# probcomp/PClean

Hardware: AMD Instinct MI355X
Metric: rows/sec per Gibbs sweep on 1M-row synthetic hospital; F1 vs ground truth (higher is better)
Workload: dtype f64

## Files before the change

include/pclean_hip.h:

```cpp
#ifndef PCLEAN_HIP_H
#define PCLEAN_HIP_H

#include <stddef.h>
#include <stdint.h>

#ifdef __cplusplus
extern "C" {
#endif

typedef struct pclean_ctx pclean_ctx;

typedef enum {
  PCLEAN_OK = 0,
  PCLEAN_ERR_ARG = -1,
  PCLEAN_ERR_HIP = -2,
  PCLEAN_ERR_NO_DEVICE = -3,
  PCLEAN_ERR_STATE = -4,
  PCLEAN_ERR_CAPACITY = -5
} pclean_status;

#define PCLEAN_DIST_OSA 0
#define PCLEAN_DIST_DL 1

#define PCLEAN_DENS_ADD_TYPOS 0
// ... 176 lines not shown
int pclean_get_moved(pclean_ctx* ctx, int32_t block_id, int32_t* n_out, int32_t* rows_out, int32_t* choice_out);
int pclean_set_active_rows(pclean_ctx* ctx, int32_t begin, int32_t count);
int pclean_set_cur_stride(pclean_ctx* ctx, int64_t stride);
int pclean_pin_host(pclean_ctx* ctx, void* ptr, size_t bytes);
int pclean_unpin_host(pclean_ctx* ctx, void* ptr);
int pclean_sweep_latent(pclean_ctx* ctx, const pclean_infer_config* cfg, uint64_t seed, uint32_t sweep_idx,
                        int32_t block_id, int32_t n_roots, const int32_t* roots, int32_t n_items,
                        const int32_t* keys, const int32_t* ev_off, const int32_t* ev_rows, const int32_t* ev_ctx,
                        const int32_t* excl, int32_t* chosen, int32_t* vals);
#define PCLEAN_EV_MAX_STEPS 4
int pclean_build_evidence(pclean_ctx* ctx, int32_t cur_block, int32_t n_steps, const int32_t* step_table,
                          const int32_t* step_col, int32_t n_target_rows, int32_t n_src, const int32_t* src_block,
                          const int32_t* src_table, const int32_t* src_col, int32_t* off_out);
int pclean_get_evidence(pclean_ctx* ctx, int32_t begin, int32_t n, int32_t* rows_out, int32_t* ctx_out);
int pclean_sweep_latent_resident(pclean_ctx* ctx, const pclean_infer_config* cfg, uint64_t seed, uint32_t sweep_idx,
                                 int32_t block_id, int32_t n_roots, const int32_t* roots, int32_t n_items,
                                 const int32_t* keys, const int32_t* ev_off, int32_t ev_begin, const int32_t* excl,
                                 int32_t* chosen, int32_t* vals);
int pclean_stats_device_ptr(pclean_ctx* ctx, int32_t table_id, void** dptr, int64_t* n);
int pclean_get_stats(pclean_ctx* ctx, int32_t table_id, int64_t* out);
int pclean_get_timing(pclean_ctx* ctx, pclean_timing* out);
int pclean_get_root_stats(pclean_ctx* ctx, pclean_root_stats* out);
int pclean_set_timed_block(pclean_ctx* ctx, int32_t block_id);
int pclean_set_profiling(pclean_ctx* ctx, int32_t on);
int pclean_get_profile(pclean_ctx* ctx, int32_t cap, char* names, float* ms, int32_t* launches, int32_t* n_out);

int pclean_argsort_ids(pclean_ctx* ctx, int32_t n, const int32_t* ids, int32_t id_max, int32_t* order_out);

int pclean_comm_unique_id(pclean_ctx* ctx, unsigned char id_out[128]);
int pclean_comm_init(pclean_ctx* ctx, int32_t n_ranks, int32_t rank, const unsigned char id[128]);
int pclean_allreduce_stats(pclean_ctx* ctx, int32_t table_id, int64_t* out);
int pclean_allreduce_stats_fused(pclean_ctx* ctx, int32_t n_tables, const int32_t* table_ids, int32_t local_is_zero,
                                 int64_t* out);
int pclean_comm_destroy(pclean_ctx* ctx);
int pclean_comm_get_stats(pclean_ctx* ctx, int64_t out[8]);

#define PCLEAN_COMMIT_FB_RECORDS 1
#define PCLEAN_COMMIT_FB_DUMMY 2
#define PCLEAN_COMMIT_FB_CAPACITY 4
typedef struct {
  int32_t table_id;
  int32_t n_hw;
  int32_t n_free;
  int32_t cols_changed;
  int32_t created, deleted;
  int64_t total, live, max_count;
} pclean_commit_slot;
typedef struct {
  int32_t fallback;
  int32_t n_changed;
  int32_t n_slots;
  int32_t stats_reduced;
  int32_t n_records[16];
  int32_t n_distinct[16];
  pclean_commit_slot slot[16];
} pclean_commit_summary;
int pclean_prepare(pclean_ctx* ctx, uint32_t ev_blocks);
int pclean_commit_enable(pclean_ctx* ctx, int32_t n_blocks, int32_t* supported);
int pclean_commit_n_slots(pclean_ctx* ctx, int32_t* n_slots, int32_t* table_ids);
int pclean_commit_set_table_state(pclean_ctx* ctx, int32_t table_id, int32_t n_hw, int32_t n_free,
                                  const int32_t* free_stack);
int pclean_commit_device(pclean_ctx* ctx, int32_t n_blocks, uint32_t sweep_idx, pclean_commit_summary* out);
int pclean_commit_device_dist(pclean_ctx* ctx, int32_t n_blocks, uint32_t sweep_idx, int32_t local_empty,
                              int32_t max_local_rows, pclean_commit_summary* out);
int pclean_commit_pull_table(pclean_ctx* ctx, int32_t table_id, int32_t* state8, int32_t* cols, int64_t* counts,
                             uint8_t* live, int32_t* free_stack, int32_t* origin);
int pclean_set_cur(pclean_ctx* ctx, int32_t n_blocks, const int32_t* cur);
int pclean_get_cur(pclean_ctx* ctx, int32_t n_blocks, int32_t* cur);
int pclean_drop_cur(pclean_ctx* ctx);
int pclean_set_sweep_mode(pclean_ctx* ctx, int32_t flags);
int pclean_sweep_fetch(pclean_ctx* ctx);
int pclean_table_shape(pclean_ctx* ctx, int32_t table_id, int32_t* n_rows, int32_t* n_cols);

int pclean_maybe_resample(pclean_ctx* ctx, int32_t n_rows, int32_t n_particles, const double* logw,
                          int32_t retain_first, uint64_t seed, uint32_t sweep, uint32_t block,
                          int32_t* ancestors, double* logml_inc, double* ess);
int pclean_final_choice(pclean_ctx* ctx, int32_t n_rows, int32_t n_particles, const double* logw,
                        int32_t use_mh, int32_t is_csmc, uint64_t seed, uint32_t sweep, int32_t* chosen,
                        double* log_total);

int pclean_debug_force_generic(pclean_ctx* ctx, int32_t on);
int pclean_debug_global_evidence_sort(pclean_ctx* ctx, int32_t on);
int pclean_debug_root_flags(pclean_ctx* ctx, int32_t n_rows, int32_t* out);

int pclean_random_add_typos(pclean_ctx* ctx, int32_t n, const uint32_t* cp, const int64_t* off, int32_t max_typos,
                            uint64_t seed, uint32_t stream, int32_t out_stride, uint32_t* out_cp, int32_t* out_len);
int pclean_random_string_prior(pclean_ctx* ctx, int32_t n, int32_t min_len, int32_t max_len, const double* init_p,
                               const double* trans_p, uint64_t seed, uint32_t stream, int32_t out_stride,
                               uint8_t* out_letters, int32_t* out_len);
int pclean_random_string_prior_at(pclean_ctx* ctx, int32_t n, const uint64_t* seeds, const uint32_t* elems, int32_t min_len,
                                  int32_t max_len, const double* init_p, const double* trans_p, uint32_t stream,
                                  int32_t out_stride, uint8_t* out_letters, int32_t* out_len);
int pclean_random_categorical(pclean_ctx* ctx, int32_t n, int32_t n_options, const double* logp, uint64_t seed,
                              uint32_t stream, int32_t* out);
int pclean_random_normal(pclean_ctx* ctx, int32_t n, const double* mean, double std, double fwd_scale, uint64_t seed,
                         uint32_t stream, double* out);
int pclean_random_maybe_swap(pclean_ctx* ctx, int32_t n, const double* prob, const int32_t* n_options, uint64_t seed,
                             uint32_t stream, int32_t* out);
int pclean_random_time_prior(pclean_ctx* ctx, int32_t n, uint64_t seed, uint32_t stream, int32_t* out);

int pclean_debug_detmath(pclean_ctx* ctx, int32_t n, const double* x, double* exp_out, double* log_out,
                         uint64_t* fixw_out);
int pclean_debug_rand64(pclean_ctx* ctx, int32_t n, uint64_t seed, const uint32_t* rows, uint32_t site,
                        uint32_t particle, uint32_t sweep, uint64_t* out);

#ifdef __cplusplus
}
#endif
#endif
```

pclean_amd/_lib.py:

```python
import ctypes as C
import os

import numpy as np

HERE = os.path.dirname(os.path.abspath(__file__))
LIB_PATH = os.environ.get("PCLEAN_HIP_LIB") or os.path.join(HERE, "libpclean_hip.so")

MAX_CTX = 4
EV_MAX_STEPS = 4
CHOICE_NEW = -1
DIST_OSA, DIST_DL = 0, 1
DENS_ADD_TYPOS, DENS_EQUAL, DENS_MAYBE_SWAP = 0, 1, 2
NODE_FK, NODE_LEAF = 0, 1
DUMMY_STRING_PRIOR, DUMMY_TIME_PRIOR = 1, 2


class PCleanHipError(RuntimeError):
    pass


class Term(C.Structure):
    _fields_ = [("obs_col", C.c_int32), ("cand_col", C.c_int32), ("pair_table", C.c_int32),
                ("dens_kind", C.c_int32), ("max_typos", C.c_int32), ("ctx_slot", C.c_int32),
                ("fn_table", C.c_int32), ("ctx_mode", C.c_int32)]
# ... 119 lines not shown
            if self._io.get("cur_pinned"):
                self.lib.pclean_unpin_host(self.h, C.c_void_p(self._io["cur_pinned"][0]))
            self._pinned, self._io = [], {}
            self.lib.pclean_ctx_destroy(self.h)
            self.h = C.c_void_p()

    def __del__(self):
        try:
            self.close()
        except Exception:
            pass

    def load_strings(self, sym, off):
        sym = np.ascontiguousarray(sym, dtype=np.uint16)
        off = np.ascontiguousarray(off, dtype=np.int64)
        check(self.h, self.lib.pclean_load_strings(self.h, C.c_int32(len(off) - 1), _p(sym, C.c_uint16),
                                                   _p(off, C.c_int64)), "pclean_load_strings")

    def load_columns(self, obs):
        obs = np.ascontiguousarray(obs, dtype=np.int32)
        n_cols, n_rows = obs.shape
        check(self.h, self.lib.pclean_load_columns(self.h, C.c_int32(n_rows), C.c_int32(n_cols), _p(obs, C.c_int32)),
              "pclean_load_columns")

    def build_pair_table(self, table_id, obs_ids, lat_ids, mode=DIST_OSA):
        obs_ids = np.ascontiguousarray(obs_ids, dtype=np.int32)
        lat_ids = np.ascontiguousarray(lat_ids, dtype=np.int32)
        check(self.h, self.lib.pclean_build_pair_table(self.h, C.c_int32(table_id), C.c_int32(len(obs_ids)),
                                                       _p(obs_ids, C.c_int32), C.c_int32(len(lat_ids)),
                                                       _p(lat_ids, C.c_int32), C.c_int32(mode)),
              "pclean_build_pair_table")

    def set_pair_table(self, table_id, table):
        table = np.ascontiguousarray(table, dtype=np.uint8)
        check(self.h, self.lib.pclean_set_pair_table(self.h, C.c_int32(table_id), C.c_int32(table.shape[0]),
                                                     C.c_int32(table.shape[1]), _p(table, C.c_uint8)),
              "pclean_set_pair_table")

    def get_pair_table(self, table_id, n_obs, n_lat):
        out = np.empty((n_obs, n_lat), dtype=np.uint16)
        check(self.h, self.lib.pclean_get_pair_table(self.h, C.c_int32(table_id), _p(out, C.c_uint16)),
              "pclean_get_pair_table")
        return out

    def get_pair_rows(self, table_id, obs_rows, n_lat):
        obs_rows = np.ascontiguousarray(obs_rows, dtype=np.int32)
        out = np.empty((len(obs_rows), n_lat), dtype=np.uint16)
        check(self.h, self.lib.pclean_get_pair_rows(self.h, C.c_int32(table_id), C.c_int32(len(obs_rows)),
                                                    _p(obs_rows, C.c_int32), _p(out, C.c_uint16)),
              "pclean_get_pair_rows")
        return out

    def set_row_offset(self, row_offset):
        check(self.h, self.lib.pclean_set_row_offset(self.h, C.c_int64(row_offset)), "pclean_set_row_offset")

    def get_density_tables(self):
        mr, md, ml = C.c_int32(), C.c_int32(), C.c_int32()
        check(self.h, self.lib.pclean_get_density_tables(self.h, C.byref(mr), C.byref(md), C.byref(ml), None, None),
              "pclean_get_density_tables")
        nb = np.empty((mr.value + 1, md.value + 1), dtype=np.float64)
        logl = np.empty(ml.value + 1, dtype=np.float64)
        check(self.h, self.lib.pclean_get_density_tables(self.h, C.byref(mr), C.byref(md), C.byref(ml),
                                                         _p(nb, C.c_double), _p(logl, C.c_double)),
              "pclean_get_density_tables")
        return mr.value, md.value, ml.value, nb, logl

    def string_prior_scores(self, lm, off, min_len, max_len, init_logp, trans_logp):
        lm = np.ascontiguousarray(lm, dtype=np.uint8)
        off = np.ascontiguousarray(off, dtype=np.int64)
        init_logp = np.ascontiguousarray(init_logp, dtype=np.float64)
        trans_logp = np.ascontiguousarray(trans_logp, dtype=np.float64)
        n = len(off) - 1
        out = np.empty(n, dtype=np.float64)
        check(self.h, self.lib.pclean_string_prior_scores(self.h, C.c_int32(n), _p(lm, C.c_uint8), _p(off, C.c_int64),
                                                          C.c_int32(min_len), C.c_int32(max_len),
                                                          _p(init_logp, C.c_double), _p(trans_logp, C.c_double),
                                                          _p(out, C.c_double)), "pclean_string_prior_scores")
        return out

    def root_flags(self, n_rows):
        out = np.empty(n_rows, dtype=np.int32)
        check(self.h, self.lib.pclean_debug_root_flags(self.h, C.c_int32(n_rows), _p(out, C.c_int32)), "pclean_debug_root_flags")
        return out

    def global_evidence_sort(self, on):
        check(self.h, self.lib.pclean_debug_global_evidence_sort(self.h, C.c_int32(int(on))), "pclean_debug_global_evidence_sort")

    def force_generic(self, on):
        check(self.h, self.lib.pclean_debug_force_generic(self.h, C.c_int32(int(on))), "pclean_debug_force_generic")

    def set_table(self, table_id, cols, counts, strength, discount, n_cols=None):
        counts = np.ascontiguousarray(counts, dtype=np.int64)
        if cols is None:
            n_rows = len(counts)
        else:
            cols = np.ascontiguousarray(cols, dtype=np.int32)
            n_cols, n_rows = cols.shape if cols.ndim == 2 else (0, len(counts))
        check(self.h, self.lib.pclean_set_table(self.h, C.c_int32(table_id), C.c_int32(n_rows), C.c_int32(n_cols),
                                                _p(cols, C.c_int32), _p(counts, C.c_int64), C.c_double(strength),
                                                C.c_double(discount)), "pclean_set_table")

    def set_block_group(self, block_id, group):
        check(self.h, self.lib.pclean_set_block_group(self.h, C.c_int32(block_id), C.c_int32(group)), "pclean_set_block_group")

    def set_lm_tables(self, init_p, trans_p, letter_sym):
        init_p = np.ascontiguousarray(init_p, dtype=np.float64)
        trans_p = np.ascontiguousarray(trans_p, dtype=np.float64)
        letter_sym = np.ascontiguousarray(letter_sym, dtype=np.uint16)
        assert init_p.size == 28 and trans_p.size == 28 * 28 and letter_sym.size == 28
        check(self.h, self.lib.pclean_set_lm_tables(self.h, _p(init_p, C.c_double), _p(trans_p, C.c_double),
                                                    _p(letter_sym, C.c_uint16)), "pclean_set_lm_tables")

    def set_options(self, table_id, values, logp):
        values = np.ascontiguousarray(values, dtype=np.int32)
        logp = np.ascontiguousarray(logp, dtype=np.float64)
        check(self.h, self.lib.pclean_set_options(self.h, C.c_int32(table_id), C.c_int32(len(values)),
                                                  _p(values, C.c_int32), _p(logp, C.c_double)), "pclean_set_options")

    def set_options_cols(self, table_id, cols, logp):
        cols = np.ascontiguousarray(cols, dtype=np.int32)
        logp = np.ascontiguousarray(logp, dtype=np.float64)
        check(self.h, self.lib.pclean_set_options_cols(self.h, C.c_int32(table_id), C.c_int32(cols.shape[1]),
                                                       C.c_int32(cols.shape[0]), _p(cols, C.c_int32),
                                                       _p(logp, C.c_double)), "pclean_set_options_cols")

    def load_numeric_columns(self, x):
        x = np.ascontiguousarray(x, dtype=np.float64)
        check(self.h, self.lib.pclean_load_numeric_columns(self.h, C.c_int32(x.shape[1]), C.c_int32(x.shape[0]),
                                                           _p(x, C.c_double)), "pclean_load_numeric_columns")

    def set_mean_table(self, table_id, mean):
        mean = np.ascontiguousarray(mean, dtype=np.float64).reshape(-1)
        check(self.h, self.lib.pclean_set_mean_table(self.h, C.c_int32(table_id), C.c_int32(len(mean)),
                                                     _p(mean, C.c_double)), "pclean_set_mean_table")

    def set_node_gauss(self, block_id, node_id, g):
        check(self.h, self.lib.pclean_set_node_gauss(self.h, C.c_int32(block_id), C.c_int32(node_id), C.byref(g)),
              "pclean_set_node_gauss")

    def set_cur_locals(self, block_id, locals_):
        if locals_ is None:
            check(self.h, self.lib.pclean_set_cur_locals(self.h, C.c_int32(block_id), None, C.c_int32(0)), "pclean_set_cur_locals")
            return
        a = np.ascontiguousarray(locals_, dtype=np.int32).reshape(-1, 2)
        check(self.h, self.lib.pclean_set_cur_locals(self.h, C.c_int32(block_id), _p(a, C.c_int32), C.c_int32(len(a))),
              "pclean_set_cur_locals")

    def get_locals(self, block_id, n_rows):
        out = np.empty((n_rows, 2), dtype=np.int32)
        check(self.h, self.lib.pclean_get_locals(self.h, C.c_int32(block_id), _p(out, C.c_int32)), "pclean_get_locals")
        return out

    def set_fn_table(self, fn_id, fn):
        fn = np.ascontiguousarray(fn, dtype=np.int32)
        check(self.h, self.lib.pclean_set_fn_table(self.h, C.c_int32(fn_id), C.c_int32(fn.shape[0]),
                                                   C.c_int32(fn.shape[1]), _p(fn, C.c_int32)), "pclean_set_fn_table")

    def set_prob_table(self, p):
        p = np.ascontiguousarray(p, dtype=np.float64)
        check(self.h, self.lib.pclean_set_prob_table(self.h, C.c_int32(len(p)), _p(p, C.c_double)),
              "pclean_set_prob_table")

    def load_score_block(self, block_id, obs_col, pair_table, val_src, key_src, nopt_fn, other_val, prob_fn,
                         prob_a_src, prob_b_src):
        a = [np.ascontiguousarray(x, dtype=np.int32).reshape(-1) for x in
             (obs_col, pair_table, val_src, key_src, nopt_fn, other_val, prob_a_src, prob_b_src)]
# ... 454 lines not shown
```

pclean_amd/csrc/enum.h:

```cpp
#pragma once
#include "ctx.h"

#define PCLEAN_MAX_CHILDREN 16
#define PCLEAN_MAX_TERMS 16

struct TermDev {
  const int32_t* obs_col;
  const int32_t* cand_col;
  const uint8_t* pair;
  const uint16_t* lat_len;
  const int32_t* fn;
  int32_t n_lat, elem_bytes, dens_kind, max_typos, ctx_slot, fn_nb;
  int32_t ctx_mode, pad;
  const int32_t* aux_col;
  int32_t other_val, pad2;
};

struct GaussDev {
  int32_t on, n_dims, n_locals, t_kind;
  const double* x;
  const double* mu;
  int32_t src_kind[4];
  const int32_t* src_ptr[4];
  int32_t src_slot[4], stride[4];
// ... 23 lines not shown
  int32_t nb_stride, pad;
  const double* prob_same;
  const double* prob_diff;
  const double* logn;
};

struct AggDev {
  const uint64_t* key;
  const int32_t* cnt;
  const int32_t* off;
  const int32_t* end;
};

struct ItemsDev {
  int32_t n, pad;
  const int32_t* row;
  const int32_t* ctx;
  const int32_t* excl;
  const int32_t* particle;
  int64_t row_offset;
  const int32_t* out_pos;
  const int32_t* ev_lo;
  const int32_t* ev_hi;
  const int32_t* ev_rows;
  const int32_t* ev_ctx;
  const int32_t* rng_row;
  const int32_t* grp_off;
  const int32_t* members;
  int32_t draw_is, draw_ds;
  const AggDev* agg;
  const int32_t* ev_item;
  const int32_t* sel;
  const unsigned int* sel_n;
  const int32_t* grp_uid;
};

struct ChildrenDev {
  int32_t n, pad;
  const double* arr[PCLEAN_MAX_CHILDREN];
  const int32_t* obs_col[PCLEAN_MAX_CHILDREN];
  int32_t n_obs[PCLEAN_MAX_CHILDREN];
};

struct GateDev {
  int32_t n, pad;
  const double* cache[PCLEAN_MAX_CHILDREN];
  const int32_t* obs_col[PCLEAN_MAX_CHILDREN];
  int32_t n_obs[PCLEAN_MAX_CHILDREN];
  double ub[PCLEAN_MAX_CHILDREN];
};
int pclean_launch_gate(pclean_ctx* ctx, const NodeDev& nd, const ItemsDev& it, const GateDev& gt, int32_t* flag);

struct FastTermDev {
  const uint8_t* comp;
  const uint8_t* clen;
  const uint8_t* cmin;
  const int32_t* obs_col;
  int32_t max_typos, ctx_slot;
  const uint8_t* pair;
  const uint16_t* lat_len;
  const int32_t* cand_col;
  const int32_t* fn;
  int32_t n_lat, fn_nb;
};
struct FastRootDev {
  int32_t n_cand, kpad, n_terms, lmax, dstride;
  int32_t kscan;
  int32_t is_leaf;
  const uint16_t* alive;
  const double* prior_e;
  const double* prior_n;
  const double* logc_m1;
  const int64_t* counts;
  double scal[4];
  int32_t n_pre, pre[3];
  int32_t cstride, atd_stride;
  double inv_c, prior_max_e, prior_max_n;
  const double* atd;
  const uint8_t* zero_row;
  const int32_t* obs_rm;
  FastTermDev terms[PCLEAN_MAX_TERMS];
};

#define ROOT_LZ_CAP 256
struct RootExtra {
  int32_t* lz_k;
  uint64_t* lz_p;
  int32_t* lz_ns;
  const int32_t* eager_rows;
  const uint64_t* g_U;
};
int pclean_launch_root_fast(pclean_ctx* ctx, const FastRootDev& fr, const ItemsDev& it, const ChildrenDev& ch,
                            uint64_t seed, uint32_t sweep, uint32_t site, int n_draws, double* lse_out,
                            int32_t* draws_out, int32_t* overflow_flag, unsigned int* overflow_count,
                            int32_t* desc_scratch, int32_t* overflow_list,
                            unsigned int* scan_stats = nullptr, int n_items = 0, const double* pre_score = nullptr,
                            bool want_worklist = true, unsigned int* wl_stat = nullptr, const int32_t* pre_obs = nullptr,
                            RootExtra* extra = nullptr);
struct LazyDrawArgs {
  int32_t n_pos, n_rows, n_particles, pad;
  const int32_t* members;
  const int32_t* uid;
  const int32_t* item_row;
  const int32_t* slot_item;
  const int32_t* chosen;
  const int32_t* cur_b;
  const int32_t* eager_rows;
  const int32_t* draws_item;
  const int32_t* lz_k;
  const uint64_t* lz_p;
  const int32_t* lz_ns;
  const uint64_t* g_U;
  int32_t* pchoice;
  int64_t row_offset;
  int32_t res_new, pad2;
};
int pclean_launch_lazy_draws(pclean_ctx* ctx, const LazyDrawArgs& a, uint64_t seed, uint32_t sweep, uint32_t site);
int pclean_launch_group_gate(pclean_ctx* ctx, const FastRootDev& fr, const ItemsDev& it, const GateDev& gt, int32_t* flag,
                             double* score_out, int32_t* obs_out);
int pclean_launch_overflow_fast(pclean_ctx* ctx, const FastRootDev& fr, const ItemsDev& it, const ChildrenDev& ch,
                                uint64_t seed, uint32_t sweep, uint32_t site, int n_draws, double* lse_out,
                                int32_t* draws_out, const int32_t* over_list, const unsigned int* over_count);
int pclean_overflow_fast_ok(const FastRootDev& fr, const ItemsDev& it);
int pclean_launch_root_flags(pclean_ctx* ctx, int n_groups, const int32_t* gd, const int32_t* grp_off,
                             const int32_t* members, const int32_t* oflag, int32_t* out);
size_t pclean_fast_desc_words(int n_groups);
int pclean_debug_gauss_ev_probe(pclean_ctx* ctx, int n_items, int P, int n_nodes, const NodeDev* nds, int node, const ItemsDev& it,
                                const int32_t* vals, int n_mean, int n_ev);
int pclean_build_obs_rowmajor(pclean_ctx* ctx, const int32_t* const* obs_cols, int n_terms, int n_rows, int32_t* out);
int pclean_build_compact(pclean_ctx* ctx, const uint8_t* pair, int n_obs, int n_lat, const int32_t* cand_col,
                         const uint16_t* lat_len, int n_cand, int kpad, uint8_t* comp, uint8_t* clen);
int pclean_build_compact_min(pclean_ctx* ctx, const uint8_t* comp, int n_obs, int kpad, int cstride, uint8_t* cmin);
int pclean_update_compact_min(pclean_ctx* ctx, const uint8_t* comp, int n_obs, int kpad, int cstride, const int32_t* rows,
                              int n_rows, uint8_t* cmin);
int pclean_update_compact(pclean_ctx* ctx, const uint8_t* pair, int n_obs, int n_lat, const int32_t* cand_col,
                          const uint16_t* lat_len, const int32_t* rows, int n_rows, int kpad, uint8_t* comp, uint8_t* clen);
int pclean_build_priors(pclean_ctx* ctx, const int64_t* counts, const double* logc_full, int n_cand, int kpad,
                        double logden_e, double logden_n, double* prior_e, double* prior_n, uint16_t* alive);

int pclean_launch_enum(pclean_ctx* ctx, const NodeDev& nd, const ItemsDev& it, const ChildrenDev& ch, uint64_t seed,
                       uint32_t sweep, uint32_t site, int n_draws, double* lse_out, double* scores_out,
                       int32_t* draws_out, double* scores_tmp = nullptr);
size_t pclean_enum_split_scores(const NodeDev& nd, const ItemsDev& it);
int pclean_leaf_coarse_blocks(int n_options);
int pclean_launch_leaf_coarse_build(pclean_ctx* ctx, const NodeDev& nd, const ItemsDev& it, int n_blocks, double* lse_out,
                                    double* m_out, uint64_t* U_out, uint64_t* coarse, int dummy_k, uint64_t* udummy_out);
int pclean_launch_leaf_coarse_draw(pclean_ctx* ctx, const NodeDev& nd, const ItemsDev& it, const int32_t* obs_col, int n_obs,
                                   int n_blocks, const double* lse_c, const double* m_c, const uint64_t* U_c,
                                   const uint64_t* coarse, uint64_t seed, uint32_t sweep, uint32_t site, int n_draws,
                                   double* lse_out, int32_t* draws_out);
int pclean_launch_prior_terms(pclean_ctx* ctx, size_t n_slots, int N, int n_nodes, const NodeDev* nds,
                              const int32_t* n_children, const int32_t* child_begin, const int32_t* children,
                              const int32_t* pchoice, const int32_t* pnewpos, const int32_t* vals, const int32_t* it_ctx,
                              double* w);
int pclean_launch_prior_terms_ev(pclean_ctx* ctx, int n_items, int P, int n_nodes, const NodeDev* nds, const AggDev* const* aggs,
                                 const int32_t* n_children, const int32_t* child_begin, const int32_t* children, int n_roots,
                                 const int32_t* roots, const ItemsDev& it, const int32_t* vals, double* w);
int pclean_launch_ev_leaf(pclean_ctx* ctx, const NodeDev& nd, const ItemsDev& it, const FastRootDev& fr, uint64_t seed,
                          uint32_t sweep, uint32_t site, int n_draws, double* lse_out, int32_t* draws_out,
                          int32_t* overflow_flag, unsigned int* overflow_count, int32_t* overflow_list = nullptr,
                          const ChildrenDev* ch = nullptr, uint32_t* dsum = nullptr);
```

pclean_amd/csrc/eval.hip:

```cpp
#include "sweep_internal.h"

int build_gauss_dev(pclean_ctx* ctx, const pclean_gauss& g, const CandTable* t, GaussDev& d) {
  memset(&d, 0, sizeof d);
  if (g.x_col < 0 || g.x_col >= ctx->n_xcols) return pclean_fail(ctx, PCLEAN_ERR_ARG, "gauss: numeric column out of range");
  const MeanTable& m = ctx->mean[g.mean_table];
  if (!m.valid) return pclean_fail(ctx, PCLEAN_ERR_STATE, "gauss: mean table %d not set", g.mean_table);
  d.on = 1;
  d.n_dims = g.n_dims;
  d.n_locals = g.n_locals;
  d.x = ctx->xnum.p + (size_t)g.x_col * ctx->n_rows + ctx->active_begin;
  d.mu = m.v.p;
  for (int i = 0; i < g.n_dims; ++i) {
    d.src_kind[i] = g.src_kind[i];
    d.src_slot[i] = g.src[i];
    d.stride[i] = g.stride[i];
    d.src_ptr[i] = nullptr;
    if (g.src_kind[i] == PCLEAN_GSRC_CAND) {
      if (!t || g.src[i] < 0 || g.src[i] >= t->n_cols) return pclean_fail(ctx, PCLEAN_ERR_ARG, "gauss: candidate column out of range");
      d.src_ptr[i] = t->cols.p + (size_t)g.src[i] * t->n_rows;
    } else if (g.src_kind[i] == PCLEAN_GSRC_OBS) {
      if (g.src[i] < 0 || g.src[i] >= ctx->n_cols) return pclean_fail(ctx, PCLEAN_ERR_ARG, "gauss: observed column out of range");
      d.src_ptr[i] = ctx->obs.p + (size_t)g.src[i] * ctx->n_rows + ctx->active_begin;
    }
  }
// ... 155 lines not shown
      b.leaf_drawable[node_id] = any ? 1 : 0;
      if (getenv("PCLEAN_DEBUG_DUMMY"))
        fprintf(stderr, "[pclean] block %d node %d: dummy option %d, drawable %d (first observed value %d, weight %llu; missing-value weight %llu)\n",
                block_id, node_id, dummy_k, any ? 1 : 0, first_o, first_o >= 0 ? (unsigned long long)hu[first_o] : 0ull,
                (unsigned long long)hu[U]);
    }
    s->leaf_version[key] = ver;
  }
  *out = cache.p;
  *obs_col = ctx->obs.p + (size_t)tm.obs_col * ctx->n_rows + ctx->active_begin;
  *n_obs = U;
  return PCLEAN_OK;
}

static int prefilter_terms(pclean_ctx* ctx, const Block& b, const pclean_node& n, int32_t pre[3]) {
  int order[PCLEAN_MAX_TERMS];
  const int nt = std::min(n.n_terms, PCLEAN_MAX_TERMS);
  for (int i = 0; i < nt; ++i) order[i] = i;
  auto plain = [&](const pclean_term& tm) {
    return tm.ctx_slot < 0 && tm.dens_kind == PCLEAN_DENS_ADD_TYPOS && tm.pair_table >= 0 && tm.pair_table < PCLEAN_MAX_TABLES &&
           ctx->pair[tm.pair_table].valid;
  };
  std::stable_sort(order, order + nt, [&](int a, int c) {
    const pclean_term& ta = b.terms[n.term_begin + a];
    const pclean_term& tc = b.terms[n.term_begin + c];
    if (plain(ta) != plain(tc)) return plain(ta);
    if (!plain(ta)) return false;
    return ctx->pair[ta.pair_table].max_lat_len > ctx->pair[tc.pair_table].max_lat_len;
  });
  int n_compact = 0;
  for (int i = 0; i < nt; ++i) n_compact += plain(b.terms[n.term_begin + i]) ? 1 : 0;
  const int n_pre = std::min(3, n_compact);
  for (int p = 0; p < 3; ++p) pre[p] = p < n_pre ? order[p] : 0;
  return n_pre;
}

static int cols_union(pclean_ctx* ctx, CandTable& t, uint64_t base, uint64_t col_mask, int* n_out) {
  *n_out = 0;
  if (t.union_n >= 0 && t.union_base == base && t.union_head == t.cols_version && t.union_mask == col_mask) {
    *n_out = t.union_n;
    return 1;
  }
  size_t first = t.delta_log.size();
  for (size_t i = 0; i < t.delta_log.size(); ++i)
    if (t.delta_log[i].base == base) {
      first = i;
      break;
    }
  if (first == t.delta_log.size() || t.delta_log.back().next != t.cols_version) return 0;
  std::vector<uint8_t> mark((size_t)std::max(t.n_rows, 1), 0);
  std::vector<int32_t> rows;
  for (size_t i = first; i < t.delta_log.size(); ++i) {
    if (i > first && t.delta_log[i].base != t.delta_log[i - 1].next) return 0;
    const CandTable::DeltaEntry& e = t.delta_log[i];
    for (size_t q = 0; q < e.rows.size(); ++q) {
      const int32_t r = e.rows[q];
      if ((e.masks[q] & col_mask) && r >= 0 && r < t.n_rows && !mark[r]) {
        mark[r] = 1;
        rows.push_back(r);
      }
    }
    if (rows.size() * 8 > (size_t)t.n_rows) return 0;
  }
  std::sort(rows.begin(), rows.end());
  if (!rows.empty()) {
    const size_t bytes = rows.size() * sizeof(int32_t);
    if (t.union_rows.alloc(rows.size() + rows.size() / 4 + 64)) return pclean_fail(ctx, PCLEAN_ERR_HIP, "device alloc failed");
    if (ctx->ustage.grow(bytes + 256)) return pclean_fail(ctx, PCLEAN_ERR_HIP, "page-locked staging alloc failed");
    ctx->ustage.rewind();
    void* h = ctx->ustage.take(bytes);
    if (!h) return pclean_fail(ctx, PCLEAN_ERR_HIP, "page-locked staging alloc failed");
    memcpy(h, rows.data(), bytes);
    HIPCHK(ctx, hipMemcpyAsync(t.union_rows.p, h, bytes, hipMemcpyHostToDevice, ctx->stream));
    HIPCHK(ctx, hipStreamSynchronize(ctx->stream));
  }
  t.union_base = base;
  t.union_mask = col_mask;
  t.union_head = t.cols_version;
  t.union_n = (int32_t)rows.size();
  *n_out = t.union_n;
  return 1;
}

static int try_fast_root(pclean_ctx* ctx, int block_id, int node_id, FastRootDev& fr, bool ev_mode = false) {
  Block& b = ctx->block[block_id];
  if (node_id >= 64) return 0;
  const pclean_node& n = b.nodes[node_id];
  const CandTable& t = ctx->cand[n.table];
  const bool leaf = n.kind == PCLEAN_NODE_LEAF;
  static const bool no_leaf = getenv("PCLEAN_NO_FAST_LEAF") != nullptr;
  if (!t.valid || t.n_rows < 1024 || n.n_terms < 1 || n.n_terms > PCLEAN_MAX_TERMS || (leaf && no_leaf)) return 0;
  if (leaf != t.is_options) return 0;
  int lmax = 0, dmax = 0;
  for (int i = 0; i < n.n_terms; ++i) {
    const pclean_term& tm = b.terms[n.term_begin + i];
    const PairTable& pt = ctx->pair[tm.pair_table];
    if (!pt.valid || tm.dens_kind != PCLEAN_DENS_ADD_TYPOS || pt.elem_bytes != 1) return 0;
    if (tm.ctx_slot >= 0 && ((!ev_mode && tm.ctx_mode != 0) || !ctx->fn[tm.fn_table].valid)) return 0;
    if (tm.ctx_slot >= 2) return 0;
    lmax = std::max(lmax, pt.max_lat_len);
    dmax = std::max(dmax, std::max(pt.max_lat_len, pt.max_obs_len));
  }
  if (lmax > 255 || dmax > 255) return 0;
  if (leaf && !ev_mode) {
    double best = 0.0;
    for (int i = 0; i < n.n_terms; ++i) {
      const pclean_term& tm = b.terms[n.term_begin + i];
      if (tm.ctx_slot < 0) best = std::max(best, ctx->pair[tm.pair_table].mean_lat_len);
    }
    if (best < 16.0) return 0;
  }
  const int kpad = (t.n_rows + 15) & ~15;
  FastRoot& f = st(ctx)->fast[block_id * 64 + node_id];
  if (f.disabled > 0) {
    --f.disabled;
    return 0;
  }
  if ((int)f.comp.size() != n.n_terms) {
    for (auto& c : f.comp) c.release();
    for (auto& c : f.clen) c.release();
    for (auto& c : f.cblk) c.release();
    f.cblk.assign(n.n_terms, DevBuf<uint8_t>());
    f.comp.assign(n.n_terms, DevBuf<uint8_t>());
    f.clen.assign(n.n_terms, DevBuf<uint8_t>());
    f.ver.assign(n.n_terms, 0);
    f.kpad = kpad;
    f.prior_ver = 0;
  } else if (f.kpad != kpad) {
    f.ver.assign(n.n_terms, 0);
    f.kpad = kpad;
    f.prior_ver = 0;
  }
  auto grow = [](DevBuf<uint8_t>& b, size_t need) -> int {
    need = std::max<size_t>(need, 16);
    return need <= b.n && b.p ? 0 : b.alloc(need + need / 8);
  };
  const int cstride = ((((kpad + 63) >> 6) + 15) & ~15);
  for (int i = 0; i < n.n_terms; ++i) {
    const pclean_term& tm = b.terms[n.term_begin + i];
    const PairTable& pt = ctx->pair[tm.pair_table];
    fr.terms[i] = FastTermDev{};
    fr.terms[i].obs_col = ctx->obs_override ? ctx->obs_override : ctx->obs.p + (size_t)tm.obs_col * ctx->n_rows + ctx->active_begin;
    fr.terms[i].max_typos = tm.max_typos;
    fr.terms[i].ctx_slot = tm.ctx_slot;
    fr.terms[i].pair = (const uint8_t*)pt.d.p;
    fr.terms[i].lat_len = pt.lat_len.p;
    fr.terms[i].cand_col = t.cols.p + (size_t)tm.cand_col * t.n_rows;
    fr.terms[i].n_lat = pt.n_lat;
    if (tm.ctx_slot >= 0) {
      const FnTable& fnt = ctx->fn[tm.fn_table];
      fr.terms[i].fn = fnt.fn.p;
      fr.terms[i].fn_nb = fnt.n_b;
      continue;
    }
    const uint64_t ver = t.cols_version * 1000003ull + pt.version;
    static const bool no_delta = getenv("PCLEAN_NO_COMPACT_DELTA") != nullptr;
    if (f.ver[i] != ver && f.comp[i].p && f.cblk[i].p && !no_delta && t.cols_delta_n >= 0 && t.cols_delta_n * 8 <= t.n_rows &&
        f.ver[i] == t.cols_delta_base * 1000003ull + pt.version) {
      ProfScope psd(ctx, "compact_table_update");
      int rc = PCLEAN_OK;
      if (t.cols_delta_n > 0)
        rc = pclean_update_compact(ctx, pt.d.p, pt.n_obs, pt.n_lat, t.cols.p + (size_t)tm.cand_col * t.n_rows, pt.lat_len.p,
                                     t.cols_delta_rows, t.cols_delta_n, kpad, f.comp[i].p, f.clen[i].p);
      if (rc) return rc;
      if (t.cols_delta_n > 0)
        rc = pclean_update_compact_min(ctx, f.comp[i].p, pt.n_obs, kpad, cstride, t.cols_delta_rows, t.cols_delta_n, f.cblk[i].p);
      if (rc) return rc;
      f.ver[i] = ver;
    }
    static const bool no_chain = getenv("PCLEAN_NO_DELTA_CHAIN") != nullptr;
    if (f.ver[i] != ver && f.comp[i].p && f.cblk[i].p && !no_delta && !no_chain) {
      CandTable& tw = ctx->cand[n.table];
      uint64_t at = 0;
      bool have = false, via_commit = false;
      if (tw.commit_delta_n >= 0 && f.ver[i] == tw.commit_delta_base * 1000003ull + pt.version) {
        at = tw.commit_delta_next;
        have = via_commit = true;
      } else {
        for (const auto& e : tw.delta_log)
          if (f.ver[i] == e.base * 1000003ull + pt.version) {
            at = e.base;
            have = true;
            break;
          }
      }
      int un = 0;
      bool ok = have;
      if (ok && at != tw.cols_version) {
        uint64_t node_mask = 0;
        for (int q = 0; q < n.n_terms; ++q)
          if (b.terms[n.term_begin + q].ctx_slot < 0) node_mask |= 1ull << std::min(b.terms[n.term_begin + q].cand_col, 63);
        const int rcu = cols_union(ctx, tw, at, node_mask, &un);
        if (rcu < 0) return rcu;
        ok = rcu == 1;
      }
      const int64_t total = (int64_t)(via_commit ? tw.commit_delta_n : 0) + un;
      static const bool dbg_chain = getenv("PCLEAN_DEBUG_CHAIN") != nullptr;
      if (dbg_chain && i == 0)
        fprintf(stderr, "[chain] block %d node %d table %d (%d rows): have %d via_commit %d (commit rows %d) log %zu entries, union %s %d rows\n",
                block_id, node_id, (int)n.table, tw.n_rows, (int)have, (int)via_commit, tw.commit_delta_n, tw.delta_log.size(),
                ok ? "ok" : "none", un);
      if (ok && total * 8 <= tw.n_rows) {
        ProfScope psd(ctx, "compact_table_update");
        int rc = PCLEAN_OK;
        const int32_t* colp = tw.cols.p + (size_t)tm.cand_col * tw.n_rows;
        if (via_commit && tw.commit_delta_n > 0) {
          rc = pclean_update_compact(ctx, pt.d.p, pt.n_obs, pt.n_lat, colp, pt.lat_len.p, tw.commit_delta_rows, tw.commit_delta_n, kpad,
                                     f.comp[i].p, f.clen[i].p);
          if (!rc) rc = pclean_update_compact_min(ctx, f.comp[i].p, pt.n_obs, kpad, cstride, tw.commit_delta_rows, tw.commit_delta_n, f.cblk[i].p);
          if (rc) return rc;
        }
        if (un > 0) {
          rc = pclean_update_compact(ctx, pt.d.p, pt.n_obs, pt.n_lat, colp, pt.lat_len.p, tw.union_rows.p, un, kpad, f.comp[i].p, f.clen[i].p);
          if (!rc) rc = pclean_update_compact_min(ctx, f.comp[i].p, pt.n_obs, kpad, cstride, tw.union_rows.p, un, f.cblk[i].p);
          if (rc) return rc;
        }
        f.ver[i] = ver;
      }
    }
    if (f.ver[i] != ver || !f.comp[i].p) {
      ProfScope psd(ctx, "compact_table_rebuild");
      if (grow(f.comp[i], (size_t)pt.n_obs * kpad) || grow(f.clen[i], (size_t)kpad))
        return pclean_fail(ctx, PCLEAN_ERR_HIP, "device alloc failed (compact tables)");
      int rc = pclean_build_compact(ctx, pt.d.p, pt.n_obs, pt.n_lat, t.cols.p + (size_t)tm.cand_col * t.n_rows,
                                    pt.lat_len.p, t.n_rows, kpad, f.comp[i].p, f.clen[i].p);
      if (rc) return rc;
      if (grow(f.cblk[i], (size_t)pt.n_obs * cstride))
        return pclean_fail(ctx, PCLEAN_ERR_HIP, "device alloc failed (compact tables)");
      rc = pclean_build_compact_min(ctx, f.comp[i].p, pt.n_obs, kpad, cstride, f.cblk[i].p);
      if (rc) return rc;
      f.ver[i] = ver;
    }
    fr.terms[i].comp = f.comp[i].p;
    fr.terms[i].clen = f.clen[i].p;
    fr.terms[i].cmin = f.cblk[i].p;
  }
  if ((int)f.zero_row.n < kpad || !f.zero_row.p) {
    if (f.zero_row.alloc((size_t)kpad + 4096)) return pclean_fail(ctx, PCLEAN_ERR_HIP, "device alloc failed");
    HIPCHK(ctx, hipMemsetAsync(f.zero_row.p, 0, f.zero_row.n, ctx->stream));
  }
  if (f.prior_ver != t.version || !f.prior_n.p) {
    if ((!leaf && f.prior_e.alloc(kpad)) || f.prior_n.alloc(kpad) || f.alive.alloc(std::max(kpad >> 4, 1)))
      return pclean_fail(ctx, PCLEAN_ERR_HIP, "device alloc failed");
    int rc = pclean_build_priors(ctx, leaf ? nullptr : t.counts.p, t.logc_full.p, t.n_rows, kpad, t.scal[1], t.scal[0],
                                 leaf ? nullptr : f.prior_e.p, f.prior_n.p, f.alive.p);
    if (rc) return rc;
    f.prior_ver = t.version;
    f.logc_max = t.logc_max;
  }
  {
    fr.n_pre = prefilter_terms(ctx, b, n, fr.pre);
    const int stride = ctx->max_d + 1;
    const uint64_t ckey = ((uint64_t)lmax << 40) | ((uint64_t)dmax << 20) | (uint64_t)stride;
    if (f.cmin_key != ckey) {
      double cm = INFINITY;
      for (int L = 1; L <= lmax; ++L)
        for (int d = 1; d <= dmax; ++d) {
          const int r = (L + 4) / 5;
          double l = ctx->h_nb[(size_t)r * stride + d];
          l -= ctx->h_logl[L] * (double)d;
          l -= 1.629048269010741 * (double)d;
          if (l == l) cm = std::min(cm, -l / (double)d);
        }
      f.cmin = cm;
      f.cmin_key = ckey;
    }
    const double cmin = f.cmin;
    if (!(cmin > 1e-6) || !std::isfinite(cmin)) {
      fr.n_pre = 0;
      fr.inv_c = 0.0;
    } else {
      fr.inv_c = 1.0 / (cmin * (1.0 - 1e-9));
    }
    fr.cstride = cstride;
    fr.prior_max_e = f.logc_max - t.scal[1];
    fr.prior_max_n = f.logc_max - t.scal[0];
  }
  fr.obs_rm = nullptr;
  static const bool no_obs_rm = getenv("PCLEAN_NO_OBS_ROWMAJOR") != nullptr;
  if (!leaf && !ev_mode && !ctx->obs_override && !no_obs_rm && ctx->n_rows >= 4096) {
    const uint64_t key = ctx->obs_version * 1000003ull + (uint64_t)ctx->n_rows + 1ull;
    if (f.obs_rm_key != key || !f.obs_rm.p) {
      if (f.obs_rm.alloc((size_t)ctx->n_rows * PCLEAN_MAX_TERMS)) return pclean_fail(ctx, PCLEAN_ERR_HIP, "device alloc failed");
      const int32_t* cols[PCLEAN_MAX_TERMS] = {};
      for (int i = 0; i < n.n_terms; ++i) cols[i] = ctx->obs.p + (size_t)b.terms[n.term_begin + i].obs_col * ctx->n_rows;
      int rc = pclean_build_obs_rowmajor(ctx, cols, n.n_terms, ctx->n_rows, f.obs_rm.p);
      if (rc) return rc;
      f.obs_rm_key = key;
    }
    fr.obs_rm = f.obs_rm.p + (size_t)ctx->active_begin * PCLEAN_MAX_TERMS;
  }
  fr.n_cand = t.n_rows;
  fr.kpad = kpad;
  {
    static const bool no_kscan = getenv("PCLEAN_NO_KSCAN") != nullptr;
    const int n_used = (t.n_used > 0 && t.n_used <= t.n_rows && !no_kscan) ? t.n_used : t.n_rows;
    fr.kscan = std::min(kpad, (n_used + 63) & ~63);
  }
  fr.n_terms = n.n_terms;
  fr.lmax = lmax;
  fr.dstride = dmax + 1;
  fr.is_leaf = leaf ? 1 : 0;
  fr.atd = ctx->atd.p;
  fr.atd_stride = ctx->max_d + 1;
// ... 30 lines not shown
  double sum = 0.0;
  for (int c = 0; c < n.n_children; ++c) sum += subtree_ub(ctx, b, b.children[n.child_begin + c]);
  return std::max(0.0, sum);
}

__global__ void scatter_f64_kernel(int n, const int32_t* list, const double* src, double* dst) {
  const int j = blockIdx.x * blockDim.x + threadIdx.x;
  if (j < n) dst[list[j]] = src[j];
}
__global__ void sub_items_kernel(int n, const int32_t* list, const int32_t* p_row, const int32_t* p_ctx,
                                 const int32_t* p_excl, const int32_t* p_ev_lo, const int32_t* p_ev_hi,
                                 const int32_t* p_rng, const int32_t* p_origin, int32_t* row, int32_t* ctxv,
                                 int32_t* excl, int32_t* ev_lo, int32_t* ev_hi, int32_t* rng, int32_t* origin) {
  const int j = blockIdx.x * blockDim.x + threadIdx.x;
  if (j >= n) return;
  const int s = list[j];
  row[j] = p_row ? p_row[s] : s;
  excl[j] = p_excl ? p_excl[s] : -1;
  for (int c = 0; c < PCLEAN_MAX_CTX; ++c) ctxv[j * PCLEAN_MAX_CTX + c] = p_ctx ? p_ctx[(size_t)s * PCLEAN_MAX_CTX + c] : 0;
  if (p_ev_lo) {
    ev_lo[j] = p_ev_lo[s];
    ev_hi[j] = p_ev_hi[s];
  }
  if (p_rng) rng[j] = p_rng[s];
  if (origin) origin[j] = p_origin ? p_origin[s] : s;
}

__global__ void group_rep_items_kernel(int n, const int32_t* list, const int32_t* grp_off, const int32_t* members,
                                       const int32_t* p_row, const int32_t* p_ctx, const int32_t* p_excl, int32_t* row,
                                       int32_t* ctxv, int32_t* excl) {
  const int j = blockIdx.x * blockDim.x + threadIdx.x;
  if (j >= n) return;
  const int g = list ? list[j] : j;
  const int s = members[grp_off[g]];
  row[j] = p_row ? p_row[s] : s;
  excl[j] = p_excl ? p_excl[s] : -1;
  for (int c = 0; c < PCLEAN_MAX_CTX; ++c) ctxv[j * PCLEAN_MAX_CTX + c] = p_ctx ? p_ctx[(size_t)s * PCLEAN_MAX_CTX + c] : 0;
}
__global__ void group_scatter_f64_kernel(int n, const int32_t* list, const int32_t* grp_off, const int32_t* members,
                                         const double* src, double* dst) {
  const int j = blockIdx.x * blockDim.x + threadIdx.x;
  if (j >= n) return;
  const int g = list ? list[j] : j;
  const double v = src[j];
  const int hi = grp_off[g + 1];
  for (int mi = grp_off[g]; mi < hi; ++mi) dst[members[mi]] = v;
}

__global__ void member_scatter_f64_kernel(int n_pos, const int32_t* uid, const int32_t* members, const double* src, double* dst) {
  const int mi = blockIdx.x * blockDim.x + threadIdx.x;
  if (mi < n_pos) dst[members[mi]] = src[uid[mi] - 1];
}

int eval_node(pclean_ctx* ctx, int block_id, int node_id, const ItemList& il, const int32_t* excl,
                     uint64_t seed, uint32_t sweep, int n_draws, double* lse_out, int32_t* draws_out,
                     double* scores_out, const double* snew_override, bool time_it) {
  Block& b = ctx->block[block_id];
  const pclean_node& n = b.nodes[node_id];
  SweepState* s = st(ctx);
  const SweepState::LazyReq lazy_req = s->lazy_req;
  s->lazy_req = SweepState::LazyReq();
  s->lazy_out.valid = false;
  static const bool no_lazy = getenv("PCLEAN_NO_LAZY_DRAWS") != nullptr;
  const bool lazy_ok = lazy_req.on && !no_lazy && n_draws > 1 && !il.rng_row && !il.ev_lo;
  static const bool lazy_split = getenv("PCLEAN_LAZY_SPLIT") != nullptr;
  const bool lazy_sure = lazy_ok && (size_t)il.n * ROOT_LZ_CAP * 12 <= ((size_t)4 << 30);
  const int fast_split_m = (lazy_sure && !lazy_split) ? 0 : std::max(4, 256 / std::max(n_draws, 1));
  NodeDev nd;
  int rc = build_node_dev(ctx, b, node_id, nd);
  if (rc) return rc;
  ChildrenDev ch{};
  ItemsDev it{il.n, 0, il.row, il.ctx, excl, n_draws == 1 ? il.particle : nullptr, s->row_offset + ctx->active_begin,
              nullptr, il.ev_lo, il.ev_hi, il.ev_rows, il.ev_ctx, il.rng_row, nullptr, nullptr, il.draw_is, il.draw_ds,
              nullptr, nullptr};
  if (il.ev_lo) {
    rc = ensure_agg(ctx, block_id, node_id, il, &it.agg);
    if (rc) return rc;
    it.ev_item = il.origin;
  }
  FastRootDev fr;
  int fast = 0, fast_ev = 0;
  ItemGroups g_pre;
  bool fast_tried = false, groups_tried = false;
  const double* pre_score = nullptr;
  const int32_t* pre_obs = nullptr;
  if (n.kind == PCLEAN_NODE_FK && ctx->prior_mode) {
    ch.n = 0;
  } else if (n.kind == PCLEAN_NODE_FK) {
    if (snew_override) {
      ch.n = 1;
      ch.arr[0] = snew_override;
      ch.obs_col[0] = nullptr;
    } else {
      if (n.n_children > PCLEAN_MAX_CHILDREN) return pclean_fail(ctx, PCLEAN_ERR_CAPACITY, "too many children");
      ch.n = n.n_children;
      const CandTable& t = ctx->cand[n.table];
      GateDev gt{};
      gt.n = n.n_children;
      int n_open = 0;
      const char* gm = getenv("PCLEAN_GATE_MIN");
      const int gate_min = gm ? atoi(gm) : 2048;
      bool gate = excl && !scores_out && il.n >= gate_min && !getenv("PCLEAN_NO_GATE");
      SweepState::GateStat* gstat = (gate && node_id < 64 && sweep < 0x7ffffff0u && !il.ev_lo && !getenv("PCLEAN_GATE_ALWAYS"))
                                        ? &s->gate_stat[block_id * 64 + node_id] : nullptr;
      if (gstat && gstat->skip > 0) {
        --gstat->skip;
        gate = false;
        gstat = nullptr;
      }
      for (int c = 0; c < n.n_children; ++c) {
        const int cid = b.children[n.child_begin + c];
        const pclean_node& cn = b.nodes[cid];
        if (cn.kind == PCLEAN_NODE_LEAF && cn.cacheable) {
          rc = ensure_leaf_cache(ctx, block_id, cid, &ch.arr[c], &ch.obs_col[c], &ch.n_obs[c]);
          if (rc) return rc;
          gt.cache[c] = ch.arr[c];
          gt.obs_col[c] = ch.obs_col[c];
          gt.n_obs[c] = ch.n_obs[c];
          gt.ub[c] = 0.0;
          if (il.ev_lo) gt.ub[c] = subtree_ub(ctx, b, cid);
        } else {
          ++n_open;
          gt.cache[c] = nullptr;
          gt.ub[c] = subtree_ub(ctx, b, cid);
          if (!(gt.ub[c] < INFINITY)) gate = false;
        }
        if (il.ev_lo && !(gt.ub[c] < INFINITY)) gate = false;
      }
      static const bool no_group_gate = getenv("PCLEAN_NO_GROUP_GATE") != nullptr;
      bool pre_grouped = false;
      if (n_open > 0 && n_draws > 0 && excl && !scores_out && !ctx->force_generic && !nd.g.on && !il.rng_row && !il.ev_lo &&
          !no_group_gate) {
        fast = try_fast_root(ctx, block_id, node_id, fr);
        if (fast < 0) return fast;
        fast_tried = true;
        if (fast) {
          rc = make_item_groups(ctx, block_id, node_id, il, excl, g_pre, fast_split_m);
          if (rc) return rc;
          groups_tried = true;
          pre_grouped = g_pre.n_groups > 0;
        }
      }
      if (pre_grouped) {
        const int ng = g_pre.n_groups;
        ItemsDev itg = it;
        itg.n = ng;
        itg.grp_off = g_pre.grp_off;
        itg.members = g_pre.members;
        int32_t* list_g = nullptr;
        unsigned int n_need = (unsigned int)ng;
        if (gate) {
          ProfScope ps(ctx, "gate_new_branch");
          int32_t* flag = scratch<int32_t>(ctx, ng);
          list_g = scratch<int32_t>(ctx, ng);
          double* sc = scratch<double>(ctx, ng);
          int32_t* ow = scratch<int32_t>(ctx, (size_t)ng * PCLEAN_MAX_TERMS);
          if (!flag || !list_g || !sc || !ow) return pclean_fail(ctx, PCLEAN_ERR_HIP, "scratch alloc failed");
          if (time_it && s->evg0) (void)hipEventRecord(s->evg0, ctx->stream);
          rc = pclean_launch_group_gate(ctx, fr, itg, gt, flag, sc, ow);
          if (rc) return rc;
          if (time_it && s->evg0) {
            (void)hipEventRecord(s->evg1, ctx->stream);
            s->gate_timed = true;
          }
          unsigned int* need_ctr = fresh_counter(ctx);
          if (!need_ctr) return pclean_fail(ctx, PCLEAN_ERR_HIP, "counter bank: device alloc failed");
          hipLaunchKernelGGL(compact_new_kernel, grid1(ng), dim3(256), 0, ctx->stream, (size_t)ng, flag, 1, need_ctr, list_g,
                             nullptr);
          PCLEAN_READ_COUNT(ctx, need_ctr, &n_need);
          pre_score = sc;
          pre_obs = ow;
          if (gstat) {
            gstat->all_need_run = n_need == (unsigned int)ng ? gstat->all_need_run + 1 : 0;
            if (gstat->all_need_run >= 3) {
              gstat->skip = 16;
              gstat->all_need_run = 2;
            }
          }
          if (n_need == (unsigned int)ng) list_g = nullptr;
        }
        ItemList sil;
        const int32_t* sexcl = nullptr;
        if (n_need > 0) {
          int32_t* row2 = scratch<int32_t>(ctx, n_need);
          int32_t* ctx2 = scratch<int32_t>(ctx, (size_t)n_need * PCLEAN_MAX_CTX);
          int32_t* excl2 = scratch<int32_t>(ctx, n_need);
          if (!row2 || !ctx2 || !excl2) return pclean_fail(ctx, PCLEAN_ERR_HIP, "scratch alloc failed");
          hipLaunchKernelGGL(group_rep_items_kernel, grid1(n_need), dim3(256), 0, ctx->stream, (int)n_need, list_g, g_pre.grp_off,
                             g_pre.members, il.row, il.ctx, excl, row2, ctx2, excl2);
          sil = ItemList{(int)n_need, row2, il.ctx ? ctx2 : nullptr, nullptr, nullptr};
          sexcl = excl2;
        }
        for (int c = 0; c < n.n_children; ++c) {
          const int cid = b.children[n.child_begin + c];
          const pclean_node& cn = b.nodes[cid];
          if (cn.kind == PCLEAN_NODE_LEAF && cn.cacheable) continue;
          double* child_lse = scratch<double>(ctx, il.n);
          if (!child_lse) return pclean_fail(ctx, PCLEAN_ERR_HIP, "scratch alloc failed");
          ch.arr[c] = child_lse;
          ch.obs_col[c] = nullptr;
          if (n_need < (unsigned int)ng)
            hipLaunchKernelGGL(fill_f64_kernel, grid1(il.n), dim3(256), 0, ctx->stream, child_lse, (size_t)il.n, -__builtin_inf());
          if (n_need == 0) continue;
          const int32_t* child_excl = nullptr;
          if (cn.kind == PCLEAN_NODE_FK) {
            if (cn.parent_fk_col < 0 || cn.parent_fk_col >= t.n_cols)
              return pclean_fail(ctx, PCLEAN_ERR_ARG, "node %d: parent_fk_col out of range", cid);
            int32_t* ce = scratch<int32_t>(ctx, sil.n);
            if (!ce) return pclean_fail(ctx, PCLEAN_ERR_HIP, "scratch alloc failed");
            hipLaunchKernelGGL(derive_excl_kernel, grid1(sil.n), dim3(256), 0, ctx->stream, sil.n, sexcl, t.counts.p,
                               t.cols.p + (size_t)cn.parent_fk_col * t.n_rows, ce);
            child_excl = ce;
          }
          double* dst = scratch<double>(ctx, sil.n);
          if (!dst) return pclean_fail(ctx, PCLEAN_ERR_HIP, "scratch alloc failed");
          rc = eval_node_lse(ctx, block_id, cid, sil, child_excl, seed, sweep, dst);
          if (rc) return rc;
          if (!list_g && g_pre.uid && fast_split_m == 0)
            hipLaunchKernelGGL(member_scatter_f64_kernel, grid1(il.n), dim3(256), 0, ctx->stream, il.n, g_pre.uid, g_pre.members, dst,
                               child_lse);
          else
            hipLaunchKernelGGL(group_scatter_f64_kernel, grid1(sil.n), dim3(256), 0, ctx->stream, sil.n, list_g, g_pre.grp_off,
                               g_pre.members, dst, child_lse);
        }
      } else {
      int32_t* list = nullptr;
      unsigned int n_need = (unsigned int)il.n;
      if (gate && n_open > 0) {
        ProfScope ps(ctx, "gate_new_branch");
        int32_t* flag = scratch<int32_t>(ctx, il.n);
        list = scratch<int32_t>(ctx, il.n);
        if (!flag || !list) return pclean_fail(ctx, PCLEAN_ERR_HIP, "scratch alloc failed");
        if (s->counter.alloc(4)) return pclean_fail(ctx, PCLEAN_ERR_HIP, "device alloc failed");
        rc = pclean_launch_gate(ctx, nd, it, gt, flag);
        if (rc) return rc;
        unsigned int* need_ctr = fresh_counter(ctx);
        if (!need_ctr) return pclean_fail(ctx, PCLEAN_ERR_HIP, "counter bank: device alloc failed");
        hipLaunchKernelGGL(compact_new_kernel, grid1(il.n), dim3(256), 0, ctx->stream, (size_t)il.n, flag, 1, need_ctr, list,
                           nullptr);
        PCLEAN_READ_COUNT(ctx, need_ctr, &n_need);
        if (gstat) {
          gstat->all_need_run = n_need == (unsigned int)il.n ? gstat->all_need_run + 1 : 0;
// ... 106 lines not shown
        it.grp_off = g.grp_off;
        it.members = g.members;
        if (fast && fast_split_m == 0) it.grp_uid = g.uid;
        ggrp = g;
      }
    }
  }
  const uint32_t site = PCLEAN_SITE_NODE(block_id, node_id);
  if (time_it) {
    pclean_root_stats& rs = ctx->root_stats;
    rs = pclean_root_stats{};
    rs.fast = fast;
    rs.n_items = il.n;
    rs.n_groups = it.n;
    rs.n_cand = nd.n_cand;
    rs.n_terms = n.n_terms;
    rs.n_draws = n_draws;
    rs.pre_scored = pre_score ? 1 : 0;
    if (fast) {
      rs.kpad = fr.kscan;
      rs.cstride = std::min(fr.cstride, (((fr.kscan + 63) >> 6) + 15) & ~15);
      rs.n_pre = fr.n_pre;
      for (int p = 0; p < 3; ++p) rs.pre_obs_col[p] = p < fr.n_pre ? b.terms[n.term_begin + fr.pre[p]].obs_col : -1;
    }
  }
  if (!fast && !fast_ev) {
    ProfScope ps(ctx, n.kind == PCLEAN_NODE_FK ? "enum_fk_generic" : "enum_leaf_generic");
    if (time_it) (void)hipEventRecord(s->ev0, ctx->stream);
    double* sc_tmp = nullptr;
    if (!scores_out) {
      const size_t sc_n = pclean_enum_split_scores(nd, it);
      if (sc_n && !(sc_tmp = scratch<double>(ctx, sc_n))) return pclean_fail(ctx, PCLEAN_ERR_HIP, "scratch alloc failed");
    }
    rc = pclean_launch_enum(ctx, nd, it, ch, seed, sweep, site, n_draws, lse_out, scores_out, draws_out, sc_tmp);
    if (time_it) (void)hipEventRecord(s->ev1, ctx->stream);
    return rc;
  }
  int32_t* oflag = scratch<int32_t>(ctx, il.n);
  if (!oflag || s->counter.alloc(4)) return pclean_fail(ctx, PCLEAN_ERR_HIP, "scratch alloc failed");
  static const bool no_fast_over = getenv("PCLEAN_NO_FAST_OVERFLOW") != nullptr;
  const bool list_mode = fast && !no_fast_over && pclean_overflow_fast_ok(fr, it) && s->over_rec.size() < OVER_SLOTS &&
                         s->over_ctr.p != nullptr;
  static const bool no_ev_list = getenv("PCLEAN_NO_EV_LIST") != nullptr;
  const bool ev_list_mode = fast_ev && !no_ev_list && s->over_rec.size() < OVER_SLOTS && s->over_ctr.p != nullptr;
  unsigned int* over_count = (list_mode || ev_list_mode) ? s->over_ctr.p + s->over_rec.size() : s->counter.p + 1;
  int32_t* over_list = nullptr;
  if (list_mode || ev_list_mode) {
    over_list = scratch<int32_t>(ctx, il.n);
    if (!over_list) return pclean_fail(ctx, PCLEAN_ERR_HIP, "scratch alloc failed");
    s->over_rec.push_back(SweepState::OverRec{block_id, node_id, il.n, time_it, n.kind == PCLEAN_NODE_LEAF, fast_ev ? 64 : 1024});
  } else {
    { const int rcz = dev_zero(ctx, s->counter.p + 1, sizeof(unsigned int)); if (rcz) return rcz; }
  }
  if (!ev_list_mode)
    { const int rcz = dev_zero(ctx, oflag, (size_t)il.n * sizeof(int32_t)); if (rcz) return rcz; }
  if (fast) {
    int32_t* desc = scratch<int32_t>(ctx, pclean_fast_desc_words(it.n));
    if (!desc) return pclean_fail(ctx, PCLEAN_ERR_HIP, "scratch alloc failed");
    ProfScope ps(ctx, (time_it && block_id == 0) ? "root_scan_block0" : (n.kind == PCLEAN_NODE_FK ? "slot_scan" : "option_scan"));
    if (time_it) (void)hipEventRecord(s->ev0, ctx->stream);
    unsigned int* scan_stats = nullptr;
    if (time_it && s->over_ctr.p) {
      scan_stats = s->over_ctr.p + OVER_SLOTS;
      s->scan_stats_used = true;
    }
    FastRoot& fwl = s->fast[block_id * 64 + node_id];
    unsigned int* wl_stat = nullptr;
    if (!fwl.wl_off && node_id < 64 && s->over_rec.size() < OVER_SLOTS && s->over_ctr.p) {
      wl_stat = s->over_ctr.p + s->over_rec.size();
      s->over_rec.push_back(SweepState::OverRec{block_id, node_id, it.n, false, false, -1});
    }
    if (fwl.wl_off > 0) --fwl.wl_off;
    RootExtra ex{};
    bool use_ex = false;
    if (lazy_ok && !it.particle && !it.out_pos &&
        (size_t)it.n * ROOT_LZ_CAP * 12 <= ((size_t)4 << 30)) {
      ex.lz_k = scratch<int32_t>(ctx, (size_t)it.n * ROOT_LZ_CAP);
      ex.lz_p = scratch<uint64_t>(ctx, (size_t)it.n * ROOT_LZ_CAP);
      ex.lz_ns = scratch<int32_t>(ctx, (size_t)it.n);
      if (!ex.lz_k || !ex.lz_p || !ex.lz_ns) return pclean_fail(ctx, PCLEAN_ERR_HIP, "scratch alloc failed");
      ex.eager_rows = lazy_req.eager_rows;
      use_ex = true;
    }
    rc = pclean_launch_root_fast(ctx, fr, it, ch, seed, sweep, site, n_draws, lse_out, draws_out, oflag, over_count, desc,
                                 over_list, scan_stats, il.n, pre_score, wl_stat != nullptr, wl_stat, pre_obs, use_ex ? &ex : nullptr);
    if (!rc && ex.lz_ns) {
      SweepState::LazyOut& lo = s->lazy_out;
      lo.valid = true;
      lo.site = site;
      lo.args = LazyDrawArgs{};
      lo.args.n_pos = il.n;
      lo.args.members = it.grp_off ? it.members : nullptr;
      lo.args.uid = it.grp_off ? ggrp.uid : nullptr;
      lo.args.item_row = il.row;
      lo.args.eager_rows = lazy_req.eager_rows;
      lo.args.draws_item = draws_out;
      lo.args.lz_k = ex.lz_k;
      lo.args.lz_p = ex.lz_p;
      lo.args.lz_ns = ex.lz_ns;
      lo.args.g_U = ex.g_U;
      lo.args.row_offset = it.row_offset;
      lo.args.res_new = fr.is_leaf ? fr.n_cand - 1 : PCLEAN_CHOICE_NEW;
    }
    if (time_it) {
      (void)hipEventRecord(s->ev1, ctx->stream);
      s->dbg_desc = desc;
      s->dbg_grp_off = it.grp_off;
      s->dbg_members = it.members;
      s->dbg_oflag = oflag;
      s->dbg_groups = it.n;
      s->dbg_items = il.n;
    }
    if (!rc && list_mode) {
      ProfScope ps2(ctx, "overflow_rerun");
      ItemsDev itf = it;
      itf.n = il.n;
      itf.grp_off = nullptr;
      itf.members = nullptr;
      const int done = pclean_launch_overflow_fast(ctx, fr, itf, ch, seed, sweep, site, n_draws, lse_out, draws_out, over_list,
                                                   over_count);
      return done < 0 ? done : PCLEAN_OK;
    }
  } else {
    {
      ProfScope ps(ctx, "evidence_option_scan");
      uint32_t* dsum = nullptr;
      static const bool no_split = getenv("PCLEAN_NO_EV_SPLIT") != nullptr;
      if (!no_split && il.n <= 64 && s->lat_max_ev >= 16384 && fr.kpad >= 256 && (size_t)il.n * fr.kpad * 4 <= ((size_t)1 << 28)) {
        dsum = scratch<uint32_t>(ctx, (size_t)il.n * fr.kpad);
        if (!dsum) return pclean_fail(ctx, PCLEAN_ERR_HIP, "scratch alloc failed");
        const int rcz = dev_zero(ctx, dsum, (size_t)il.n * fr.kpad * sizeof(uint32_t));
        if (rcz) return rcz;
      }
      rc = pclean_launch_ev_leaf(ctx, nd, it, fr, seed, sweep, site, n_draws, lse_out, draws_out, oflag, over_count, over_list,
                                 n.kind == PCLEAN_NODE_FK ? &ch : nullptr, dsum);
    }
    if (!rc && ev_list_mode) {
      ProfScope ps2(ctx, "overflow_rerun");
      ItemsDev itr = it;
      itr.sel = over_list;
      itr.sel_n = over_count;
      double* sc_tmp = nullptr;
      const size_t sc_n = pclean_enum_split_scores(nd, itr);
      if (sc_n && !(sc_tmp = scratch<double>(ctx, sc_n))) return pclean_fail(ctx, PCLEAN_ERR_HIP, "scratch alloc failed");
      return pclean_launch_enum(ctx, nd, itr, ch, seed, sweep, site, n_draws, lse_out, nullptr, draws_out, sc_tmp);
    }
  }
  if (rc) return rc;
  unsigned int n_over = 0;
  PCLEAN_READ_COUNT(ctx, s->counter.p + 1, &n_over);
  ctx->timing.reserved += (int32_t)n_over;
  if (time_it) ctx->root_stats.overflow_items = (int32_t)n_over;
  if (n.kind == PCLEAN_NODE_LEAF && il.n >= (il.ev_lo ? 64 : 1024) &&
      (il.ev_lo ? n_over >= (unsigned int)il.n : (size_t)n_over * 4 > (size_t)il.n)) {
    FastRoot& f = s->fast[block_id * 64 + node_id];
    f.disabled = f.backoff;
    f.backoff = std::min(f.backoff * 2, 1 << 20);
  }
  if (n_over && getenv("PCLEAN_DEBUG_OVERFLOW"))
    fprintf(stderr, "[pclean] block %d node %d: %u of %d items re-run by the generic kernel\n", block_id, node_id, n_over,
            il.n);
  if (n_over) {
    ProfScope ps(ctx, "overflow_rerun");
    int32_t* list = scratch<int32_t>(ctx, n_over);
    int32_t* row2 = scratch<int32_t>(ctx, n_over);
    int32_t* excl2 = scratch<int32_t>(ctx, n_over);
    int32_t* ctx2 = scratch<int32_t>(ctx, (size_t)n_over * PCLEAN_MAX_CTX);
    int32_t* part2 = scratch<int32_t>(ctx, n_over);
// ... 334 lines not shown
  const bool first = split_m > 0 ? pos == piece * split_m : pos == 0;
  const int at = off0 + pos;
  members[at] = i;
  uid[at] = g0 + piece + 1;
  if (head) head[at] = first ? 1 : 0;
  if (first) grp_off[g0 + piece] = at;
}
__global__ void hg_unique_kernel(int n, const uint64_t* __restrict__ incl, const int32_t* __restrict__ rep,
                                 const int32_t* __restrict__ slot_of, const int32_t* __restrict__ row,
                                 const int32_t* __restrict__ ctxv, const int32_t* __restrict__ excl,
                                 int32_t* __restrict__ uid_of_item, int32_t* __restrict__ row2, int32_t* __restrict__ ctx2,
                                 int32_t* __restrict__ excl2) {
  const int i = blockIdx.x * blockDim.x + threadIdx.x;
  if (i >= n) return;
  const int sl = slot_of[i];
  const int u = (int)incl[sl] - 1;
  uid_of_item[i] = u;
  if (rep[sl] - 1 == i) {
    row2[u] = row ? row[i] : i;
    if (ctxv)
      for (int s = 0; s < PCLEAN_MAX_CTX; ++s) ctx2[(size_t)u * PCLEAN_MAX_CTX + s] = ctxv[(size_t)i * PCLEAN_MAX_CTX + s];
    if (excl) excl2[u] = excl[i];
  }
}
static int make_item_groups_hash(pclean_ctx* ctx, const ItemList& il, const int32_t* excl, const KeyColsDev& kc, int split_m,
                                 bool want_members, ItemGroups& g) {
  const int n = il.n;
  uint32_t cap = 1024;
  while (cap < 2u * (uint32_t)n) cap <<= 1;
  int32_t* rep = scratch<int32_t>(ctx, (size_t)cap * 2);
  uint64_t* incl = scratch<uint64_t>(ctx, cap);
  int32_t* slot_of = scratch<int32_t>(ctx, n);
  int32_t* pos_of = want_members ? scratch<int32_t>(ctx, n) : nullptr;
  size_t tmp_scan = 0, tmp_scan2 = 0;
  hipcub::TransformInputIterator<uint64_t, HgClaimed, const int32_t*> in_claimed(rep, HgClaimed());
  hipcub::TransformInputIterator<uint64_t, HgPacked, const unsigned int*> in_packed((const unsigned int*)(rep + cap), HgPacked{split_m});
  HIPCHK(ctx, hipcub::DeviceScan::InclusiveSum(nullptr, tmp_scan, in_claimed, incl, (int)cap, ctx->stream));
  HIPCHK(ctx, hipcub::DeviceScan::InclusiveSum(nullptr, tmp_scan2, in_packed, incl, (int)cap, ctx->stream));
  unsigned char* tmp = scratch<unsigned char>(ctx, std::max<size_t>(std::max(tmp_scan, tmp_scan2), 16));
  if (!rep || !incl || !slot_of || (want_members && !pos_of) || !tmp) return pclean_fail(ctx, PCLEAN_ERR_HIP, "scratch alloc failed");
  uint32_t wbits = HG_WBITS;
  while ((1u << wbits) > cap) --wbits;
  HashGroupDev hg{rep, want_members ? (unsigned int*)(rep + cap) : nullptr, cap - 1, split_m, wbits};
  { const int rcz = dev_zero(ctx, rep, (size_t)cap * (want_members ? 2 : 1) * sizeof(int32_t)); if (rcz) return rcz; }
  hipLaunchKernelGGL(hg_insert_kernel, grid1(n), dim3(256), 0, ctx->stream, n, kc, il.row, il.ctx, excl, hg, slot_of, pos_of);
  int32_t n_unique = 0;
  if (want_members) {
    HIPCHK(ctx, hipcub::DeviceScan::InclusiveSum(tmp, tmp_scan2, in_packed, incl, (int)cap, ctx->stream));
    PCLEAN_READ_COUNT(ctx, reinterpret_cast<const uint32_t*>(incl + (cap - 1)) + 1, &n_unique);
  } else {
    HIPCHK(ctx, hipcub::DeviceScan::InclusiveSum(tmp, tmp_scan, in_claimed, incl, (int)cap, ctx->stream));
    PCLEAN_READ_COUNT(ctx, reinterpret_cast<const uint32_t*>(incl + (cap - 1)), &n_unique);
  }
  if (n_unique <= 0 || (double)n_unique > 0.75 * n) return PCLEAN_OK;
  g.n_groups = n_unique;
  g.hg_incl = incl;
  g.hg_rep = rep;
  g.hg_slot_of = slot_of;
  if (!want_members) return PCLEAN_OK;
  int32_t* members = scratch<int32_t>(ctx, n);
  int32_t* uid = scratch<int32_t>(ctx, n);
  int32_t* grp_off = scratch<int32_t>(ctx, (size_t)n_unique + 1);
  if (!members || !uid || !grp_off) return pclean_fail(ctx, PCLEAN_ERR_HIP, "scratch alloc failed");
  hipLaunchKernelGGL(hg_fill_kernel, grid1(n), dim3(256), 0, ctx->stream, n, cap, incl, hg.cnt, slot_of, pos_of, split_m, members,
                     (int32_t*)nullptr, uid, grp_off);
  g.grp_off = grp_off;
  g.members = members;
  g.head = nullptr;
  g.uid = uid;
  return PCLEAN_OK;
}

#define STATIC_ORDER_WINDOWS 8
__global__ void static_key_kernel(int n, const int32_t* __restrict__ tuple_id, const uint32_t* __restrict__ pre_hash,
                                  uint64_t* __restrict__ key, int32_t* __restrict__ idx) {
  const int i = blockIdx.x * blockDim.x + threadIdx.x;
  if (i >= n) return;
  key[i] = ((uint64_t)pre_hash[i] << 32) | (uint32_t)tuple_id[i];
  idx[i] = i;
}
__global__ void static_tid_kernel(int n, const uint64_t* __restrict__ key_s, int32_t* __restrict__ tid) {
  const int j = blockIdx.x * blockDim.x + threadIdx.x;
  if (j < n) tid[j] = (int32_t)(uint32_t)key_s[j];
}
static int ensure_static_order(pclean_ctx* ctx, int block_id, int node_id, int n, const SweepState::TupleIds::StaticOrder** out) {
  typedef SweepState::TupleIds::StaticOrder StaticOrder;
  *out = nullptr;
  SweepState::TupleIds& t = st(ctx)->tuple_ids[block_id * 64 + node_id];
  const int begin = ctx->active_begin;
  if (!t.id.p || !t.pre.p || n <= 0 || (size_t)begin + (size_t)n > t.id.n) return PCLEAN_OK;
  for (const StaticOrder& w : t.windows)
    if (w.begin == begin && w.n == n) {
      *out = &w;
      return PCLEAN_OK;
    }
  for (;;) {
    size_t held = 0, smallest = 0;
    for (size_t k = 0; k < t.windows.size(); ++k) {
      held += (size_t)t.windows[k].n;
      if (t.windows[k].n < t.windows[smallest].n) smallest = k;
    }
    if (t.windows.size() < STATIC_ORDER_WINDOWS && held + (size_t)n <= 2 * (size_t)ctx->n_rows) break;
    if (t.windows.empty() || t.windows[smallest].n >= n) {
      static const bool trace = getenv("PCLEAN_TRACE_SYNC") != nullptr;
      if (trace) fprintf(stderr, "[pclean static groups] block %d node %d rows %d+%d: window not cached, hash table\n", block_id, node_id, begin, n);
      return PCLEAN_OK;
    }
    t.windows[smallest].release();
    t.windows.erase(t.windows.begin() + smallest);
  }
  StaticOrder w;
  w.begin = begin;
  w.n = n;
  DevBuf<uint64_t> key, key_s;
  DevBuf<int32_t> idx;
  DevBuf<unsigned char> tmp;
  int32_t* h_tid = nullptr;
  int32_t* h_off = nullptr;
  auto cleanup = [&]() {
    key.release(); key_s.release(); idx.release(); tmp.release();
    if (h_tid) (void)hipHostFree(h_tid);
    if (h_off) (void)hipHostFree(h_off);
  };
  auto fail = [&](const char* what) {
    cleanup();
    w.release();
    return pclean_fail(ctx, PCLEAN_ERR_HIP, "%s", what);
  };
  if (key.alloc(n) || key_s.alloc(n) || idx.alloc(n) || w.order.alloc(n) || w.tid.alloc(n)) return fail("device alloc failed");
  hipLaunchKernelGGL(static_key_kernel, grid1(n), dim3(256), 0, ctx->stream, n, t.id.p + begin, t.pre.p + begin, key.p, idx.p);
  size_t tmp_sort = 0;
  if (hipcub::DeviceRadixSort::SortPairs(nullptr, tmp_sort, key.p, key_s.p, idx.p, w.order.p, n, 0, 64, ctx->stream) != hipSuccess ||
      tmp.alloc(std::max<size_t>(tmp_sort, 16)) ||
      hipcub::DeviceRadixSort::SortPairs(tmp.p, tmp_sort, key.p, key_s.p, idx.p, w.order.p, n, 0, 64, ctx->stream) != hipSuccess)
    return fail("static order: sort failed");
  hipLaunchKernelGGL(static_tid_kernel, grid1(n), dim3(256), 0, ctx->stream, n, key_s.p, w.tid.p);
  if (hipHostMalloc((void**)&h_tid, (size_t)n * sizeof(int32_t)) != hipSuccess) { h_tid = nullptr; return fail("host alloc failed"); }
  if (hipHostMalloc((void**)&h_off, ((size_t)n + 1) * sizeof(int32_t)) != hipSuccess) { h_off = nullptr; return fail("host alloc failed"); }
  if (hipMemcpyAsync(h_tid, w.tid.p, (size_t)n * sizeof(int32_t), hipMemcpyDeviceToHost, ctx->stream) != hipSuccess ||
      hipStreamSynchronize(ctx->stream) != hipSuccess)
    return fail("static order: read-back failed");
  int n_off = 0, start = 0;
  h_off[n_off++] = 0;
  for (int sb = 0; sb < n;) {
    int se = sb + 1;
    while (se < n && h_tid[se] == h_tid[sb]) ++se;
    if (se - start > 64) {
      if (sb > start) h_off[n_off++] = start = sb;
      while (se - start > 64) h_off[n_off++] = start = start + 64;
    }
    sb = se;
  }
  h_off[n_off++] = n;
  w.n_tiles = n_off - 1;
  if (w.tile_off.alloc(n_off)) return fail("device alloc failed");
  if (hipMemcpyAsync(w.tile_off.p, h_off, (size_t)n_off * sizeof(int32_t), hipMemcpyHostToDevice, ctx->stream) != hipSuccess ||
      hipStreamSynchronize(ctx->stream) != hipSuccess)
    return fail("static order: upload failed");
  cleanup();
  t.windows.push_back(w);
  *out = &t.windows.back();
  return PCLEAN_OK;
}
__global__ __launch_bounds__(256) void sg_class_kernel(int n_tiles, const int32_t* __restrict__ tile_off,
                                                       const int32_t* __restrict__ order, const int32_t* __restrict__ tid_sorted,
                                                       const int32_t* __restrict__ excl, int split_m,
                                                       int32_t* __restrict__ members, int32_t* __restrict__ loc,
                                                       int32_t* __restrict__ tile_cnt) {
  const int tile = blockIdx.x * 4 + (threadIdx.x >> 6);
  const int lane = threadIdx.x & 63;
  if (tile >= n_tiles) return;
  const int t0 = tile_off[tile], len = tile_off[tile + 1] - t0;
  const bool on = lane < len;
  int i = 0, kt = 0, ke = 0;
  if (on) {
    i = order[t0 + lane];
    kt = tid_sorted[t0 + lane];
    ke = excl[i];
  }
  int pos_acc = 0, piece_acc = 0, my_at = 0, my_loc = 0;
  for (unsigned long long pend = __ballot(on); pend;) {
    const int ld = __builtin_ctzll(pend);
    const int lt = __builtin_amdgcn_readlane(kt, ld), le = __builtin_amdgcn_readlane(ke, ld);
    const unsigned long long cls = __ballot(on && kt == lt && ke == le) & pend;
    const int c = __popcll(cls);
    const int pieces = split_m > 0 ? max(c / split_m, 1) : 1;
    if ((cls >> lane) & 1ull) {
      const int r = __popcll(cls & ((1ull << lane) - 1ull));
      const int piece = split_m > 0 ? min(r / split_m, pieces - 1) : 0;
      const bool first = split_m > 0 ? r == piece * split_m : r == 0;
      my_at = pos_acc + r;
      my_loc = ((piece_acc + piece) << 1) | (first ? 1 : 0);
    }
    pos_acc += c;
    piece_acc += pieces;
    pend &= ~cls;
  }
  if (on) {
    members[t0 + my_at] = i;
    loc[t0 + my_at] = my_loc;
  }
  if (lane == 0) tile_cnt[tile] = piece_acc;
}
__global__ __launch_bounds__(256) void sg_fill_kernel(int n, int n_tiles, const int32_t* __restrict__ tile_off,
                                                      const int32_t* __restrict__ loc, const int32_t* __restrict__ tile_cnt,
                                                      const int32_t* __restrict__ incl, int32_t* __restrict__ uid,
                                                      int32_t* __restrict__ grp_off) {
  const int tile = blockIdx.x * 4 + (threadIdx.x >> 6);
  const int lane = threadIdx.x & 63;
  if (tile >= n_tiles) return;
  const int t0 = tile_off[tile], len = tile_off[tile + 1] - t0;
  const int base = incl[tile] - tile_cnt[tile];
  if (lane < len) {
    const int v = loc[t0 + lane], grp = base + (v >> 1);
    uid[t0 + lane] = grp + 1;
    if (v & 1) grp_off[grp] = t0 + lane;
  }
  if (tile == 0 && lane == 0) grp_off[incl[n_tiles - 1]] = n;
}
static int make_item_groups_static(pclean_ctx* ctx, const SweepState::TupleIds::StaticOrder& so, const ItemList& il,
                                   const int32_t* excl, int split_m, ItemGroups& g) {
  const int n = il.n, nt = so.n_tiles;
  int32_t* members = scratch<int32_t>(ctx, n);
  int32_t* loc = scratch<int32_t>(ctx, n);
  int32_t* tile_cnt = scratch<int32_t>(ctx, nt);
  int32_t* incl = scratch<int32_t>(ctx, nt);
  size_t tmp_scan = 0;
  HIPCHK(ctx, hipcub::DeviceScan::InclusiveSum(nullptr, tmp_scan, tile_cnt, incl, nt, ctx->stream));
  unsigned char* tmp = scratch<unsigned char>(ctx, std::max<size_t>(tmp_scan, 16));
  if (!members || !loc || !tile_cnt || !incl || !tmp) return pclean_fail(ctx, PCLEAN_ERR_HIP, "scratch alloc failed");
  hipLaunchKernelGGL(sg_class_kernel, grid1(nt, 4), dim3(256), 0, ctx->stream, nt, so.tile_off.p, so.order.p, so.tid.p, excl,
                     split_m, members, loc, tile_cnt);
  HIPCHK(ctx, hipcub::DeviceScan::InclusiveSum(tmp, tmp_scan, tile_cnt, incl, nt, ctx->stream));
  int32_t n_unique = 0;
  PCLEAN_READ_COUNT(ctx, incl + (nt - 1), &n_unique);
  if (n_unique <= 0 || (double)n_unique > 0.75 * n) return PCLEAN_OK;
  int32_t* uid = scratch<int32_t>(ctx, n);
  int32_t* grp_off = scratch<int32_t>(ctx, (size_t)n_unique + 1);
  if (!uid || !grp_off) return pclean_fail(ctx, PCLEAN_ERR_HIP, "scratch alloc failed");
  hipLaunchKernelGGL(sg_fill_kernel, grid1(nt, 4), dim3(256), 0, ctx->stream, n, nt, so.tile_off.p, loc, tile_cnt, incl, uid, grp_off);
  g.n_groups = n_unique;
  g.grp_off = grp_off;
  g.members = members;
  g.head = nullptr;
  g.uid = uid;
  return PCLEAN_OK;
}

static int make_item_groups(pclean_ctx* ctx, int block_id, int node_id, const ItemList& il, const int32_t* excl,
                            ItemGroups& g, int split_m, bool want_members) {
  Block& b = ctx->block[block_id];
  std::set<int> cols;
  bool use_ctx = false;
  static const bool disabled = getenv("PCLEAN_NO_DEDUP") != nullptr;
  g = ItemGroups();
  if (ctx->prior_mode) {
    if (disabled || il.n < 4096 || il.ev_lo) return PCLEAN_OK;
  } else if (disabled || il.n < 4096 || il.ev_lo || !subtree_key(ctx, b, node_id, cols, use_ctx) || cols.size() > 32) {
    return PCLEAN_OK;
  }
  const int n = il.n;
  KeyColsDev kc{};
  kc.use_ctx = use_ctx ? 1 : 0;
  for (int c : cols) {
    if (c < 0 || c >= ctx->n_cols) return pclean_fail(ctx, PCLEAN_ERR_ARG, "term column out of range");
    kc.col[kc.n_cols++] = ctx->obs.p + (size_t)c * ctx->n_rows + ctx->active_begin;
  }
  {
    const pclean_node& nn = b.nodes[node_id];
    int32_t pre[3];
    kc.n_pre = (nn.n_terms <= PCLEAN_MAX_TERMS && !ctx->prior_mode) ? prefilter_terms(ctx, b, nn, pre) : 0;
    for (int q = 0; q < kc.n_pre; ++q) {
      const int c = b.terms[nn.term_begin + pre[q]].obs_col;
      kc.pre_col[q] = ctx->obs.p + (size_t)c * ctx->n_rows + ctx->active_begin;
    }
  }
  static const bool no_tuple_ids = getenv("PCLEAN_NO_TUPLE_IDS") != nullptr;
  if (!ctx->prior_mode && !ctx->obs_override && !cols.empty() && node_id < 64 && !no_tuple_ids) {
    int32_t pre_cols[3] = {-1, -1, -1};
    const pclean_node& nn2 = b.nodes[node_id];
    int32_t pre2[3];
    const int np2 = kc.n_pre > 0 ? prefilter_terms(ctx, b, nn2, pre2) : 0;
    for (int q = 0; q < np2; ++q) pre_cols[q] = b.terms[nn2.term_begin + pre2[q]].obs_col;
    int rc = ensure_tuple_ids(ctx, block_id, node_id, cols, pre_cols, np2, &kc.tuple_id, &kc.pre_hash);
    if (rc) return rc;
    if (np2 == 0) kc.pre_hash = nullptr;
  }
  static const bool sort_groups = getenv("PCLEAN_SORT_GROUPS") != nullptr;
  static const bool no_static = getenv("PCLEAN_NO_STATIC_GROUPS") != nullptr;
  if (want_members && excl && !il.row && (!kc.use_ctx || !il.ctx) && kc.tuple_id && !sort_groups && !no_static) {
    const SweepState::TupleIds::StaticOrder* so = nullptr;
    int rc = ensure_static_order(ctx, block_id, node_id, n, &so);
    if (rc) return rc;
    if (so) return make_item_groups_static(ctx, *so, il, excl, split_m, g);
  }
  if (!sort_groups) return make_item_groups_hash(ctx, il, excl, kc, split_m, want_members, g);
  uint64_t* key = scratch<uint64_t>(ctx, n);
  uint64_t* key_s = scratch<uint64_t>(ctx, n);
  int32_t* idx = scratch<int32_t>(ctx, n);
  int32_t* idx_s = scratch<int32_t>(ctx, n);
  int32_t* head = scratch<int32_t>(ctx, n);
  int32_t* uid = scratch<int32_t>(ctx, n);
  if (!key || !key_s || !idx || !idx_s || !head || !uid) return pclean_fail(ctx, PCLEAN_ERR_HIP, "scratch alloc failed");
  size_t tmp_sort = 0, tmp_scan = 0;
  int key_bits = 32, low_bits = 24;
  bool k32 = true;
  if (excl) {
    const int kmax = ctx->cand[b.nodes[node_id].table].n_rows + 2;
    int rb = 1;
    while ((1ll << rb) < kmax) ++rb;
    static const bool force64 = getenv("PCLEAN_SORT_KEY64") != nullptr;
    k32 = rb <= 16 && !force64;
    low_bits = k32 ? 32 - rb : 24;
    key_bits = low_bits + rb;
  }
  uint32_t* key32 = (uint32_t*)key;
  uint32_t* key32_s = (uint32_t*)key_s;
  if (k32) {
    hipLaunchKernelGGL(item_key_kernel<uint32_t>, grid1(n), dim3(256), 0, ctx->stream, n, kc, il.row, il.ctx, excl, low_bits,
                       key32, idx);
    HIPCHK(ctx, pclean_sort_pairs<uint32_t>(nullptr, tmp_sort, key32, key32_s, idx, idx_s, n, key_bits, ctx->stream));
  } else {
    hipLaunchKernelGGL(item_key_kernel<uint64_t>, grid1(n), dim3(256), 0, ctx->stream, n, kc, il.row, il.ctx, excl, low_bits,
// ... 341 lines not shown
```

pclean_amd/csrc/root_wave.hip:

```cpp
#include <algorithm>
#include <cstdlib>
#include <cstring>
#include <cstdio>

#include "../../include/pclean_detmath.h"
#include "../../include/pclean_philox.h"
#include "enum.h"

#define ADD_TYPOS_IMPOSSIBLE (-1e5)
#define FIX_CUTOFF 28.5
#define PRE_CLAMP 42
#define CUT_ALL 126u
#define WAVE_SURV_CAP 256
#ifndef WAVE_RB
#define WAVE_RB 1
#endif
#ifndef WAVE_TC
#define WAVE_TC 6
#endif
#ifndef WAVE_CHUNK
#define WAVE_CHUNK 4
#endif
#ifndef WAVE_MIN_WAVES
#define WAVE_MIN_WAVES 5
// ... 107 lines not shown
  return PCLEAN_OK;
}
int pclean_build_compact_min(pclean_ctx* ctx, const uint8_t* comp, int n_obs, int kpad, int cstride, uint8_t* cmin) {
  for (int o0 = 0; o0 < n_obs; o0 += 65535) {
    const int no = std::min(65535, n_obs - o0);
    hipLaunchKernelGGL(compact_min_kernel, dim3((cstride + 63) / 64, no), dim3(64), 0, ctx->stream,
                       comp + (size_t)o0 * kpad, no, kpad, cstride, cmin + (size_t)o0 * cstride);
  }
  HIPCHK(ctx, hipGetLastError());
  return PCLEAN_OK;
}
__global__ void compact_min_rows_kernel(const uint8_t* __restrict__ comp, int kpad, int cstride, const int32_t* __restrict__ rows,
                                        int n_rows, uint8_t* __restrict__ cmin) {
  const int j = blockIdx.x * blockDim.x + threadIdx.x;
  const int o = blockIdx.y;
  if (j >= n_rows) return;
  const int kb = rows[j] >> 6;
  uint32_t m = 255u;
  const int q0 = kb * 4, nq = kpad >> 4;
  for (int q = q0; q < q0 + 4 && q < nq; ++q) {
    const uint4 c = reinterpret_cast<const uint4*>(comp + (size_t)o * kpad)[q];
    const uint32_t cw[4] = {c.x, c.y, c.z, c.w};
#pragma unroll
    for (int w = 0; w < 4; ++w)
#pragma unroll
      for (int e = 0; e < 4; ++e) m = min(m, (cw[w] >> (8 * e)) & 0xffu);
  }
  cmin[(size_t)o * cstride + kb] = (uint8_t)m;
}
int pclean_update_compact_min(pclean_ctx* ctx, const uint8_t* comp, int n_obs, int kpad, int cstride, const int32_t* rows,
                              int n_rows, uint8_t* cmin) {
  if (n_rows <= 0) return PCLEAN_OK;
  static const bool no_rows = getenv("PCLEAN_NO_COMPACT_MIN_ROWS") != nullptr;
  if (no_rows || (size_t)n_rows * 64 * 2 > (size_t)kpad) return pclean_build_compact_min(ctx, comp, n_obs, kpad, cstride, cmin);
  for (int o0 = 0; o0 < n_obs; o0 += 65535) {
    const int no = std::min(65535, n_obs - o0);
    hipLaunchKernelGGL(compact_min_rows_kernel, dim3((n_rows + 63) / 64, no), dim3(64), 0, ctx->stream, comp + (size_t)o0 * kpad,
                       kpad, cstride, rows, n_rows, cmin + (size_t)o0 * cstride);
  }
  HIPCHK(ctx, hipGetLastError());
  return PCLEAN_OK;
}
int pclean_build_priors(pclean_ctx* ctx, const int64_t* counts, const double* logc_full, int n_cand, int kpad,
                        double logden_e, double logden_n, double* prior_e, double* prior_n, uint16_t* alive) {
  static const bool unfused = getenv("PCLEAN_NO_FUSED_PRIORS") != nullptr;
  hipLaunchKernelGGL(priors_kernel, dim3((kpad + 255) / 256), dim3(256), 0, ctx->stream, counts, logc_full, n_cand,
                     kpad, logden_e, logden_n, prior_e, prior_n, unfused ? (uint16_t*)nullptr : alive);
  if (unfused) hipLaunchKernelGGL(alive_kernel, dim3(((kpad >> 4) + 255) / 256), dim3(256), 0, ctx->stream, prior_n, kpad, alive);
  HIPCHK(ctx, hipGetLastError());
  return PCLEAN_OK;
}

__device__ __forceinline__ double wave_max64(double v) {
  for (int o = 32; o > 0; o >>= 1) v = fmax(v, __shfl_xor(v, o, 64));
  return v;
}

__device__ __forceinline__ double wave_term_dens(const FastRootDev& fr, const FastTermDev& tm, int of, int ctx0, int ctx1,
                                                 int k) {
  int d, L;
  if (tm.ctx_slot < 0) {
    d = tm.comp[(size_t)of * fr.kpad + k];
    L = tm.clen[k];
    if (d == PRE_CLAMP) d = tm.pair[(size_t)of * tm.n_lat + tm.cand_col[k]];
  } else {
    const int c = tm.ctx_slot == 0 ? ctx0 : ctx1;
    const int val = tm.fn[(size_t)c * tm.fn_nb + tm.cand_col[k]];
    d = tm.pair[(size_t)of * tm.n_lat + val];
    L = tm.lat_len[val];
  }
  return (tm.max_typos >= 0 && d > tm.max_typos) ? ADD_TYPOS_IMPOSSIBLE : fr.atd[(size_t)L * fr.atd_stride + d];
}

__device__ __forceinline__ double fast_exact_score(const FastRootDev& fr, const int* o, int ctx0, int ctx1, int k,
                                                   double pr) {
  double b = pr;
  for (int f = 0; f < fr.n_terms; ++f) {
    if (o[f] < 0) continue;
    b += wave_term_dens(fr, fr.terms[f], o[f], ctx0, ctx1, k);
  }
  return b;
}

__device__ __forceinline__ double fast_exact_score_mlp(const FastRootDev& fr, const int* o, int ctx0, int ctx1, int k, double pr) {
  int d[PCLEAN_MAX_TERMS], L[PCLEAN_MAX_TERMS];
  bool sat = false;
#pragma unroll
  for (int f = 0; f < PCLEAN_MAX_TERMS; ++f) {
    const bool plain = f < fr.n_terms && fr.terms[f].ctx_slot < 0;
    const uint8_t* crow = (plain && o[f] >= 0) ? fr.terms[f].comp + (size_t)o[f] * fr.kpad : fr.zero_row;
    const uint8_t* cl = plain ? fr.terms[f].clen : fr.zero_row;
    d[f] = crow[k];
    L[f] = cl[k];
  }
#pragma unroll
  for (int f = 0; f < PCLEAN_MAX_TERMS; ++f) sat |= d[f] == PRE_CLAMP;
  if (sat) {
#pragma unroll
    for (int f = 0; f < PCLEAN_MAX_TERMS; ++f)
      if (d[f] == PRE_CLAMP) d[f] = fr.terms[f].pair[(size_t)o[f] * fr.terms[f].n_lat + fr.terms[f].cand_col[k]];
  }
  double l[PCLEAN_MAX_TERMS];
#pragma unroll
  for (int f = 0; f < PCLEAN_MAX_TERMS; ++f) {
    const int mt = f < fr.n_terms ? fr.terms[f].max_typos : -1;
    l[f] = fr.atd[(size_t)L[f] * fr.atd_stride + ((mt >= 0 && d[f] > mt) ? 0 : d[f])];
  }
  double b = pr;
#pragma unroll
  for (int f = 0; f < PCLEAN_MAX_TERMS; ++f) {
    if (f < fr.n_terms) {
      if (fr.terms[f].ctx_slot >= 0) {
        if (o[f] >= 0) b += wave_term_dens(fr, fr.terms[f], o[f], ctx0, ctx1, k);
      } else {
        const int mt = fr.terms[f].max_typos;
        const double lf = (mt >= 0 && d[f] > mt) ? ADD_TYPOS_IMPOSSIBLE : l[f];
        if (o[f] >= 0) b += lf;
      }
    }
  }
  return b;
}

__device__ __forceinline__ void load_row_obs(const FastRootDev& fr, int row, int* o) {
  static_assert(PCLEAN_MAX_TERMS == 16, "four 16-byte loads");
  if (fr.obs_rm) {
    const int4* po = reinterpret_cast<const int4*>(fr.obs_rm + (size_t)row * PCLEAN_MAX_TERMS);
#pragma unroll
    for (int q = 0; q < 4; ++q) {
      const int4 v = po[q];
      o[4 * q] = v.x;
      o[4 * q + 1] = v.y;
      o[4 * q + 2] = v.z;
      o[4 * q + 3] = v.w;
    }
  } else {
    for (int f = 0; f < PCLEAN_MAX_TERMS; ++f) o[f] = f < fr.n_terms ? fr.terms[f].obs_col[row] : -1;
  }
}
struct ObsColsDev {
  const int32_t* col[PCLEAN_MAX_TERMS];
};
__global__ void obs_rowmajor_kernel(ObsColsDev oc, int n_terms, int n_rows, int32_t* __restrict__ out) {
  const size_t i = (size_t)blockIdx.x * blockDim.x + threadIdx.x;
  if (i >= (size_t)n_rows * PCLEAN_MAX_TERMS) return;
  const int row = (int)(i / PCLEAN_MAX_TERMS), f = (int)(i % PCLEAN_MAX_TERMS);
  out[i] = f < n_terms ? oc.col[f][row] : -1;
}
int pclean_build_obs_rowmajor(pclean_ctx* ctx, const int32_t* const* obs_cols, int n_terms, int n_rows, int32_t* out) {
  if (n_rows <= 0) return PCLEAN_OK;
  ObsColsDev oc{};
  for (int f = 0; f < n_terms && f < PCLEAN_MAX_TERMS; ++f) oc.col[f] = obs_cols[f];
  const size_t n = (size_t)n_rows * PCLEAN_MAX_TERMS;
  hipLaunchKernelGGL(obs_rowmajor_kernel, dim3((unsigned)((n + 255) / 256)), dim3(256), 0, ctx->stream, oc, n_terms, n_rows, out);
  HIPCHK(ctx, hipGetLastError());
  return PCLEAN_OK;
}

__global__ void group_desc_kernel(const FastRootDev fr, const ItemsDev it, const ChildrenDev ch, int n_groups,
                                  int32_t* __restrict__ gd, unsigned int* __restrict__ chunk_ctr, double* __restrict__ g_m,
                                  uint64_t* __restrict__ g_U, int32_t* __restrict__ g_res,
                                  unsigned int* __restrict__ scan_stats, const double* __restrict__ pre_score,
                                  const int32_t* __restrict__ pre_obs) {
  const int g = blockIdx.x * blockDim.x + threadIdx.x;
  if (g < 8) chunk_ctr[g * WAVE_CTR_STRIDE] = 0u;
  if (g >= 8 && g < 8 + WL_SEGS) chunk_ctr[WL_SEG_CTR(g - 8)] = 0u;
  if (g == 8 + WL_SEGS) chunk_ctr[WAVE_WORK_CTR] = 0u;
  unsigned int st_blocks = 0, st_resolved = 0;
  if (g < n_groups) {
  const int m_lo = it.grp_off ? it.grp_off[g] : g, m_hi = it.grp_off ? it.grp_off[g + 1] : g + 1;
  const int t = it.grp_off ? it.members[m_lo] : g;
  const int row = it.row ? it.row[t] : t;
  const int excl = it.excl ? it.excl[t] : -1;
  const int ctx0 = it.ctx ? it.ctx[(size_t)t * PCLEAN_MAX_CTX] : 0;
  const int ctx1 = it.ctx ? it.ctx[(size_t)t * PCLEAN_MAX_CTX + 1] : 0;
  int o[PCLEAN_MAX_TERMS];
  if (pre_obs) {
    static_assert(PCLEAN_MAX_TERMS == 16, "four 16-byte loads");
    const int4* po = reinterpret_cast<const int4*>(pre_obs + (size_t)g * PCLEAN_MAX_TERMS);
#pragma unroll
    for (int q = 0; q < 4; ++q) {
      const int4 v = po[q];
      o[4 * q] = v.x;
      o[4 * q + 1] = v.y;
      o[4 * q + 2] = v.z;
      o[4 * q + 3] = v.w;
    }
  } else {
    load_row_obs(fr, row, o);
  }
  const bool deleted = excl >= 0 && fr.counts && fr.counts[excl] <= 1;
  double bound = -__builtin_inf(), score_cur = 0.0;
  bool have_cur = false;
  if (excl >= 0 && !deleted && fr.logc_m1) {
    score_cur = pre_score ? pre_score[g] : fast_exact_score_mlp(fr, o, ctx0, ctx1, excl, fr.logc_m1[excl] - fr.scal[1]);
    have_cur = true;
    bound = score_cur - 1.0;
  }
  double sn = -__builtin_inf();
  if (!fr.is_leaf) {
    const double logden = excl >= 0 ? fr.scal[1] : fr.scal[0];
    double snew = 0.0;
    for (int c = 0; c < ch.n; ++c) {
      size_t idx = (size_t)(it.out_pos ? it.out_pos[t] : t);
      if (ch.obs_col[c]) {
        const int oc = ch.obs_col[c][row];
        idx = oc < 0 ? (size_t)ch.n_obs[c] : (size_t)oc;
      }
      snew += ch.arr[c][idx];
    }
    sn = ((deleted ? fr.scal[3] : fr.scal[2]) - logden) + snew;
  }
  bound = fmax(bound, sn);
  uint32_t cut = CUT_ALL, cut_max = CUT_ALL, refine = 0;
  if (fr.n_pre > 0) {
    const double pmax = excl >= 0 ? fr.prior_max_e : fr.prior_max_n;
    if (bound > -__builtin_inf()) {
      const double x = (pmax - bound + FIX_CUTOFF) * fr.inv_c;
      if (x >= 0.0 && x < (double)(CUT_ALL - 2u)) cut_max = (uint32_t)x + 2u;
    }
    if (cut_max < WAVE_DCUT_OK) {
      cut = cut_max;
    } else {
      cut = WAVE_GUESS;
      refine = 1;
    }
  }
  bool resolved = false;
  int res_val = 0;
  double res_m = 0.0;
  if (g_res && have_cur && !refine && fr.n_pre == 3 && fr.cstride > 0 && !fr.is_leaf) {
    const double hi = fmax(score_cur, sn), lo = fmin(score_cur, sn);
    if (hi > -__builtin_inf() && score_cur != sn && !(lo - hi >= -28.5)) {
      const uint8_t *r[3], *mn[3];
      for (int p = 0; p < 3; ++p) {
        const int op = o[fr.pre[p]];
        r[p] = op >= 0 ? fr.terms[fr.pre[p]].comp + (size_t)op * fr.kpad : fr.zero_row;
        mn[p] = op >= 0 ? fr.terms[fr.pre[p]].cmin + (size_t)op * fr.cstride : fr.zero_row;
      }
      const int nquads = fr.kscan >> 4, kblk = (fr.kscan + 63) >> 6;
      bool has_excl = false, other = false;
      for (int kb0 = 0; kb0 < kblk && !other; kb0 += 16) {
        const uint4 a = *reinterpret_cast<const uint4*>(mn[0] + kb0), b = *reinterpret_cast<const uint4*>(mn[1] + kb0),
                    c = *reinterpret_cast<const uint4*>(mn[2] + kb0);
        const uint32_t aw[4] = {a.x, a.y, a.z, a.w}, bw[4] = {b.x, b.y, b.z, b.w}, cw[4] = {c.x, c.y, c.z, c.w};
        for (int e = 0; e < 16 && !other; ++e) {
          const int kb = kb0 + e;
          if (kb >= kblk) break;
          const uint32_t sh = 8u * (e & 3);
          if (((aw[e >> 2] >> sh) & 0xffu) + ((bw[e >> 2] >> sh) & 0xffu) + ((cw[e >> 2] >> sh) & 0xffu) > cut) continue;
          ++st_blocks;
          for (int q = kb * 4; q < kb * 4 + 4 && q < nquads && !other; ++q) {
            const uint4 fa = reinterpret_cast<const uint4*>(r[0])[q], fb = reinterpret_cast<const uint4*>(r[1])[q],
                        fc = reinterpret_cast<const uint4*>(r[2])[q];
            const uint32_t al = fr.alive[q];
            const uint32_t xa[4] = {fa.x, fa.y, fa.z, fa.w}, xb[4] = {fb.x, fb.y, fb.z, fb.w}, xc[4] = {fc.x, fc.y, fc.z, fc.w};
            for (int i = 0; i < 16; ++i) {
              const uint32_t s2 = 8u * (i & 3);
              const uint32_t dsum = ((xa[i >> 2] >> s2) & 0xffu) + ((xb[i >> 2] >> s2) & 0xffu) + ((xc[i >> 2] >> s2) & 0xffu);
              if (dsum <= cut && ((al >> i) & 1u)) {
                if (q * 16 + i == excl)
                  has_excl = true;
                else
                  other = true;
              }
            }
          }
        }
      }
      if (has_excl && !other) {
        resolved = true;
        res_m = hi;
        res_val = sn > score_cur ? PCLEAN_CHOICE_NEW : excl;
      }
    }
  }
  int32_t* d = gd + (size_t)g * GD_STRIDE;
  d[0] = m_lo;
  d[1] = m_hi;
  d[2] = t;
  d[3] = row;
  d[4] = excl;
  d[5] = ctx0;
  d[6] = ctx1;
  d[7] = (deleted ? 1 : 0) | (refine ? 2 : 0) | (have_cur ? 4 : 0) | (resolved ? 8 : 0);
  d[8] = __double2loint(bound);
  d[9] = __double2hiint(bound);
  for (int f = 0; f < PCLEAN_MAX_TERMS; ++f) d[10 + f] = o[f];
  d[26] = __double2loint(sn);
  d[27] = __double2hiint(sn);
  d[28] = (int32_t)cut;
  d[29] = (int32_t)cut_max;
  d[30] = __double2loint(score_cur);
  d[31] = __double2hiint(score_cur);
  if (g_res) g_res[g] = resolved ? res_val : WAVE_RES_UNRESOLVED;
  if (resolved) {
    g_m[g] = res_m;
    g_U[g] = PCLEAN_FIX_ONE;
    st_resolved = 1u;
  }
  }
  if (scan_stats) {
    for (int sh = 32; sh > 0; sh >>= 1) {
      st_blocks += __shfl_xor(st_blocks, sh, 64);
      st_resolved += __shfl_xor(st_resolved, sh, 64);
    }
    if ((threadIdx.x & 63) == 0 && (st_blocks | st_resolved)) {
      unsigned int* sl = scan_stats + (size_t)(((blockIdx.x * blockDim.x + threadIdx.x) >> 6) & 63) * 32;
      atomicAdd(&sl[1], st_blocks);
      atomicAdd(&sl[3], st_resolved);
    }
  }
}

__global__ void group_gate_kernel(const FastRootDev fr, const ItemsDev it, const GateDev gt, int n_groups,
                                  int32_t* __restrict__ flag, double* __restrict__ score_out,
                                  int32_t* __restrict__ obs_out) {
  const int g = blockIdx.x * blockDim.x + threadIdx.x;
  if (g >= n_groups) return;
  const int t = it.grp_off ? it.members[it.grp_off[g]] : g;
  const int row = it.row ? it.row[t] : t;
  const int excl = it.excl ? it.excl[t] : -1;
  const int ctx0 = it.ctx ? it.ctx[(size_t)t * PCLEAN_MAX_CTX] : 0;
  const int ctx1 = it.ctx ? it.ctx[(size_t)t * PCLEAN_MAX_CTX + 1] : 0;
  const bool deleted = excl >= 0 && fr.counts && fr.counts[excl] <= 1;
  bool need = true;
  double sc = 0.0;
  int o[PCLEAN_MAX_TERMS];
  load_row_obs(fr, row, o);
  {
    int4* po = reinterpret_cast<int4*>(obs_out + (size_t)g * PCLEAN_MAX_TERMS);
#pragma unroll
    for (int q = 0; q < 4; ++q) po[q] = make_int4(o[4 * q], o[4 * q + 1], o[4 * q + 2], o[4 * q + 3]);
  }
  if (excl >= 0 && !deleted && fr.logc_m1) {
    sc = fast_exact_score_mlp(fr, o, ctx0, ctx1, excl, fr.logc_m1[excl] - fr.scal[1]);
    double ub = fr.scal[2] - fr.scal[1];
    for (int c = 0; c < gt.n; ++c) {
      if (gt.cache[c]) {
        const int oc = gt.obs_col[c][row];
        ub += gt.cache[c][oc < 0 ? gt.n_obs[c] : oc];
      } else {
        ub += gt.ub[c];
      }
    }
    need = !(ub + 1e-6 < sc - FIX_CUTOFF);
  }
  flag[g] = need ? PCLEAN_CHOICE_NEW : 0;
  score_out[g] = sc;
}
int pclean_launch_group_gate(pclean_ctx* ctx, const FastRootDev& fr, const ItemsDev& it, const GateDev& gt, int32_t* flag,
                             double* score_out, int32_t* obs_out) {
  if (it.n <= 0) return PCLEAN_OK;
  hipLaunchKernelGGL(group_gate_kernel, dim3((it.n + 255) / 256), dim3(256), 0, ctx->stream, fr, it, gt, it.n, flag, score_out,
                     obs_out);
  HIPCHK(ctx, hipGetLastError());
  return PCLEAN_OK;
}

__global__ void resolved_draws_kernel(int n_items, int n_groups, const int32_t* __restrict__ grp_off,
                                      const int32_t* __restrict__ members, const int32_t* __restrict__ out_pos,
                                      const int32_t* __restrict__ g_res, int n_draws, int draw_is, int draw_ds,
                                      int32_t* __restrict__ draws_out) {
  const int mi = blockIdx.x * blockDim.x + threadIdx.x;
  if (mi >= n_items) return;
  int g = mi, tm = mi;
  if (grp_off) {
    int lo = 0, hi = n_groups - 1;
    while (lo < hi) {
      const int mid = (lo + hi + 1) >> 1;
      if (grp_off[mid] <= mi)
        lo = mid;
      else
        hi = mid - 1;
    }
    g = lo;
    tm = members[mi];
  }
  const int r = g_res[g];
  if (r == WAVE_RES_UNRESOLVED) return;
  int32_t* dst = draws_out + (size_t)(out_pos ? out_pos[tm] : tm) * draw_is;
  for (int j = 0; j < n_draws; ++j) dst[(size_t)j * draw_ds] = r;
}

struct WaveItems {
  const int32_t* members;
  const int32_t* row;
  const int32_t* rng_row;
  const int32_t* particle;
  const int32_t* out_pos;
  int64_t row_offset;
  int32_t draw_is, draw_ds;
};

#define SETTLE_L 16
#define SETTLE_MAX_BLOCKS 4
struct SettleArgs {
  const uint8_t* comp[3];
  const uint8_t* cmin[3];
  int32_t pre[3];
  int32_t kpad, kscan, cstride;
  const uint16_t* alive;
  const uint8_t* zero_row;
};
__global__ __launch_bounds__(256) void group_settle_kernel(const SettleArgs sa, const WaveItems wi, int n_groups, int n_draws,
                                                           int32_t* __restrict__ gd, double* __restrict__ g_m,
                                                           uint64_t* __restrict__ g_U, int32_t* __restrict__ draws_out,
                                                           unsigned int* __restrict__ scan_stats,
                                                           int32_t* __restrict__ worklist, unsigned int* __restrict__ work_n,
                                                           int seg_cap, int32_t* __restrict__ lz_ns, int32_t* __restrict__ lz_k,
                                                           uint64_t* __restrict__ lz_p, const int32_t* __restrict__ eager_rows) {
  const int tid = blockIdx.x * blockDim.x + threadIdx.x;
  const int g = tid / SETTLE_L, l = tid % SETTLE_L;
  const int lane = threadIdx.x & 63, base = lane & ~(SETTLE_L - 1);
  const unsigned long long gmask = ((1ull << SETTLE_L) - 1ull) << base;
  int32_t* d = gd + (size_t)(g < n_groups ? g : 0) * GD_STRIDE;
  const int w0 = g < n_groups ? d[l] : 0, w1 = g < n_groups ? d[16 + l] : 0;
  auto word = [&](int w) { return __shfl(w < 16 ? w0 : w1, base + (w & 15), 64); };
  const int flags = word(7), excl = word(4);
  const double sn = __hiloint2double(word(27), word(26)), score_cur = __hiloint2double(word(31), word(30));
  const double hi = fmax(score_cur, sn), lo = fmin(score_cur, sn);
  const uint32_t cut = (uint32_t)word(28);
  int op[3];
#pragma unroll
  for (int p = 0; p < 3; ++p) op[p] = sa.pre[p] >= 0 ? word(sa.pre[p] >= 0 ? sa.pre[p] : 0) : -1;
  const bool eligible = g < n_groups && (flags & 4) && !(flags & 2) && !(flags & 8) && hi > -__builtin_inf() &&
                        score_cur != sn && !(lo - hi >= -28.5);
  const uint8_t *r[3], *mn[3];
#pragma unroll
  for (int p = 0; p < 3; ++p) {
    r[p] = op[p] >= 0 ? sa.comp[p] + (size_t)op[p] * sa.kpad : sa.zero_row;
    mn[p] = op[p] >= 0 ? sa.cmin[p] + (size_t)op[p] * sa.cstride : sa.zero_row;
  }
  const int kblk = (sa.kscan + 63) >> 6;
  unsigned int st_blocks = 0;
  bool has_excl = false, other = false;
  uint32_t pass = 0;
  int kb_base = 0;
// ... 977 lines not shown
      const uint64_t x = pclean_mulhi64(pclean_rand64(seed, rng_row, site, pid, sweep), U);
      int a = 0, b = nc - 1;
      while (a < b) {
        const int mid = (a + b) >> 1;
        if (u[mid] > x)
          b = mid;
        else
          a = mid + 1;
      }
      res = (fk && a == n) ? PCLEAN_CHOICE_NEW : a;
    }
    draws_out[(size_t)to * draw_is + (size_t)j * draw_ds] = res;
  }
  }
}

static size_t overflow_lds_bytes(const FastRootDev& fr) {
  const int nc = fr.n_cand + (fr.is_leaf ? 0 : 1);
  return (size_t)((nc + 1) & ~1) * 8 + (32 + 64) * 8;
}
int pclean_overflow_fast_ok(const FastRootDev& fr, const ItemsDev& it) {
  return overflow_lds_bytes(fr) <= 160 * 1024 && !it.ev_lo;
}
int pclean_launch_overflow_fast(pclean_ctx* ctx, const FastRootDev& fr, const ItemsDev& it, const ChildrenDev& ch,
                                uint64_t seed, uint32_t sweep, uint32_t site, int n_draws, double* lse_out,
                                int32_t* draws_out, const int32_t* over_list, const unsigned int* over_count) {
  if (it.n <= 0) return 1;
  const size_t lds = overflow_lds_bytes(fr);
  if (lds > 160 * 1024 || it.grp_off || it.ev_lo) return 0;
  static bool attr_set = false;
  if (!attr_set) {
    HIPCHK(ctx, hipFuncSetAttribute((const void*)overflow_lds_kernel, hipFuncAttributeMaxDynamicSharedMemorySize, 160 * 1024));
    attr_set = true;
  }
  const int grid = over_list ? std::min(it.n, 256) : it.n;
  hipLaunchKernelGGL(overflow_lds_kernel, dim3(grid), dim3(OVF_T), lds, ctx->stream, fr, it, ch, seed, sweep, site, n_draws,
                     lse_out, draws_out, over_list, over_count);
  HIPCHK(ctx, hipGetLastError());
  return 1;
}

__global__ void root_flags_kernel(int n_groups, const int32_t* __restrict__ gd, const int32_t* __restrict__ grp_off,
                                  const int32_t* __restrict__ members, const int32_t* __restrict__ oflag,
                                  int32_t* __restrict__ out) {
  const int g = blockIdx.x * blockDim.x + threadIdx.x;
  if (g >= n_groups) return;
  const int refine = (gd[(size_t)g * GD_STRIDE + 7] & 2) ? 2 : 0;
  const int lo = grp_off ? grp_off[g] : g, hi = grp_off ? grp_off[g + 1] : g + 1;
  for (int mi = lo; mi < hi; ++mi) {
    const int t = grp_off ? members[mi] : g;
    out[t] = refine | (oflag[t] != 0 ? 1 : 0);
  }
}
int pclean_launch_root_flags(pclean_ctx* ctx, int n_groups, const int32_t* gd, const int32_t* grp_off,
                             const int32_t* members, const int32_t* oflag, int32_t* out) {
  hipLaunchKernelGGL(root_flags_kernel, dim3((n_groups + 255) / 256), dim3(256), 0, ctx->stream, n_groups, gd, grp_off,
                     members, oflag, out);
  HIPCHK(ctx, hipGetLastError());
  return PCLEAN_OK;
}

typedef void (*wave_kernel_t)(const FastRootDev, const WaveItems, uint64_t, uint32_t, uint32_t, int, int, int, const int32_t*,
                              unsigned int*, double*, uint64_t*, int32_t*, int32_t*, unsigned int*, int32_t*, unsigned int*,
                              const int32_t*, int32_t*, uint64_t*, int32_t*, const int32_t*, int);

static wave_kernel_t pick_kernel(int n_terms) {
  if (n_terms <= 2) return fk_root_wave_kernel<2, WAVE_SURV_CAP, 4>;
  if (n_terms <= 4) return fk_root_wave_kernel<4, WAVE_SURV_CAP, 4>;
  if (n_terms <= 8) return fk_root_wave_kernel<8, WAVE_SURV_CAP, 4>;
  if (n_terms <= 12) return fk_root_wave_kernel<12, WAVE_SURV_CAP, 4>;
  return fk_root_wave_kernel<16, WAVE_SURV_CAP, 4>;
}

size_t pclean_fast_desc_words(int n_groups) {
  const size_t ng = (size_t)std::max(n_groups, 1);
  return ng * GD_STRIDE + 8 * WAVE_CTR_STRIDE + ng * 4 + ng + ng + (ng + 16 * (WL_SEGS + 1) + 64);
}

int pclean_launch_root_fast(pclean_ctx* ctx, const FastRootDev& fr, const ItemsDev& it, const ChildrenDev& ch,
                            uint64_t seed, uint32_t sweep, uint32_t site, int n_draws, double* lse_out,
                            int32_t* draws_out, int32_t* overflow_flag, unsigned int* overflow_count,
                            int32_t* desc_scratch, int32_t* overflow_list, unsigned int* scan_stats, int n_items,
                            const double* pre_score, bool want_worklist, unsigned int* wl_stat, const int32_t* pre_obs,
                            RootExtra* extra) {
  if (it.n <= 0) return PCLEAN_OK;
  const size_t ng = (size_t)it.n;
  unsigned int* chunk_ctr = reinterpret_cast<unsigned int*>(desc_scratch + ng * GD_STRIDE);
  double* g_m = reinterpret_cast<double*>(desc_scratch + ng * GD_STRIDE + 8 * WAVE_CTR_STRIDE);
  uint64_t* g_U = reinterpret_cast<uint64_t*>(g_m + ng);
  int32_t* g_res = reinterpret_cast<int32_t*>(g_U + ng);
  int32_t* worklist = g_res + ng;
  static const bool want_resolve = getenv("PCLEAN_RESOLVE_GROUPS") != nullptr;
  const bool resolve = n_draws > 0 && want_resolve && (!it.grp_off || n_items > 0);
  const bool lazy = extra && extra->lz_ns && n_draws > 0 && !resolve;
  hipLaunchKernelGGL(group_desc_kernel, dim3((it.n + 255) / 256), dim3(256), 0, ctx->stream, fr, it, ch, it.n,
                     desc_scratch, chunk_ctr, g_m, g_U, resolve ? g_res : nullptr, scan_stats, pre_score, pre_obs);
  if (extra) extra->g_U = g_U;
  static const bool no_settle = getenv("PCLEAN_NO_SETTLE") != nullptr;
  const bool settle = !no_settle && !resolve && n_draws > 0 && !fr.is_leaf && fr.n_pre >= 1 && fr.n_pre <= 3 && fr.cstride > 0 &&
                      it.excl != nullptr && it.n >= 4096;
  const int wpg = 4;
  wave_kernel_t kern = pick_kernel(fr.n_terms);
  static const bool no_dense = getenv("PCLEAN_NO_DENSE_SCAN") != nullptr;
  static int resident[17] = {0};
  const int variant = fr.n_terms <= 2 ? 2 : fr.n_terms <= 4 ? 4 : fr.n_terms <= 8 ? 8 : fr.n_terms <= 12 ? 12 : 16;
  int& res = resident[variant];
  if (!res) {
    int per_cu = 0, n_cu = 256;
    if (hipOccupancyMaxActiveBlocksPerMultiprocessor(&per_cu, (const void*)kern, 64 * wpg, 0) != hipSuccess || per_cu <= 0) per_cu = 4;
    hipDeviceProp_t prop;
    if (hipGetDeviceProperties(&prop, ctx->device) == hipSuccess && prop.multiProcessorCount > 0) n_cu = prop.multiProcessorCount;
    per_cu = std::min(per_cu, 8);
    res = n_cu * per_cu;
  }
  int wgs = res;
  if (const char* e = getenv("PCLEAN_WAVE_WGS")) wgs = std::max(1, atoi(e));
  int chunk = std::max(1, std::min(WAVE_CHUNK, it.n / std::max(res * wpg, 1)));
  if (const char* e = getenv("PCLEAN_WAVE_CHUNK")) chunk = std::max(1, atoi(e));
  wgs = std::min(wgs, (it.n + wpg * chunk - 1) / (wpg * chunk));
  wgs = (wgs + 7) & ~7;
  WaveItems wi{it.grp_off ? it.members : nullptr, it.row, it.rng_row, it.particle, it.out_pos, it.row_offset, it.draw_is,
               it.draw_ds};
  bool use_worklist = false;
  if (settle) {
    WaveItems ws = wi;
    ws.draw_is = it.draw_is ? it.draw_is : n_draws;
    ws.draw_ds = it.draw_ds ? it.draw_ds : 1;
    SettleArgs sa{};
    for (int p = 0; p < 3; ++p) {
      const bool on = p < fr.n_pre && fr.terms[fr.pre[p]].comp && fr.terms[fr.pre[p]].cmin;
      sa.comp[p] = on ? fr.terms[fr.pre[p]].comp : fr.zero_row;
      sa.cmin[p] = on ? fr.terms[fr.pre[p]].cmin : fr.zero_row;
      sa.pre[p] = on ? 10 + fr.pre[p] : -1;
    }
    sa.kpad = fr.kpad;
    sa.kscan = fr.kscan;
    sa.cstride = fr.cstride;
    sa.alive = fr.alive;
    sa.zero_row = fr.zero_row;
    const size_t n_thr = (size_t)it.n * SETTLE_L;
    static const bool no_worklist = getenv("PCLEAN_NO_WORKLIST") != nullptr;
    use_worklist = !no_worklist && want_worklist;
    const unsigned int n_wg = (unsigned int)((n_thr + 255) / 256);
    const int seg_cap = (int)((n_wg / WL_SEGS + 1) * 16);
    int32_t* seg_list = worklist + ng;
    hipLaunchKernelGGL(group_settle_kernel, dim3(n_wg), dim3(256), 0, ctx->stream, sa, ws, it.n, n_draws, desc_scratch, g_m, g_U,
                       draws_out, scan_stats, use_worklist ? seg_list : nullptr, chunk_ctr, seg_cap, lazy ? extra->lz_ns : nullptr,
                       lazy ? extra->lz_k : nullptr, lazy ? extra->lz_p : nullptr, lazy ? extra->eager_rows : nullptr);
    if (use_worklist)
      hipLaunchKernelGGL(worklist_pack_kernel, dim3(1), dim3(1024), 0, ctx->stream, seg_list, seg_cap, chunk_ctr, worklist, wl_stat);
  }
  hipLaunchKernelGGL(kern, dim3(wgs), dim3(64 * wpg), 0, ctx->stream, fr, wi, seed, sweep, site, n_draws, it.n, chunk, desc_scratch,
                     chunk_ctr, g_m, g_U, draws_out, overflow_flag, overflow_count, overflow_list, scan_stats,
                     use_worklist ? worklist : nullptr, lazy ? extra->lz_k : nullptr, lazy ? extra->lz_p : nullptr,
                     lazy ? extra->lz_ns : nullptr, lazy ? extra->eager_rows : nullptr, no_dense ? 0 : 1);
#ifdef WAVE_PHASE_CLOCK
  if (it.n > 100000) {
    unsigned long long h[16];
    (void)hipStreamSynchronize(ctx->stream);
    (void)hipMemcpyFromSymbol(h, HIP_SYMBOL(g_wave_clk), sizeof h);
    const char* nm[7] = {"handout+desc", "decode", "scan", "exact", "weights", "draws+out", "tail"};
    double tot = 0;
    for (int i = 0; i < 6; ++i) tot += (double)h[i];
    fprintf(stderr, "[wave clk] groups %d terms %d waves %llu (grid %d WGs): ", it.n, fr.n_terms, h[8], wgs);
    for (int i = 0; i < 6; ++i) fprintf(stderr, "%s %.1f%% ", nm[i], 100.0 * (double)h[i] / tot);
    fprintf(stderr, "| cycles/group %.0f, groups seen %llu; full scans %llu, cached scans %llu, decided groups %llu, survivors scored %llu; two-level scans %llu, passing blocks %llu; chunk %d, lazy %d\n",
            tot / (double)h[7], h[7], h[9], h[10], h[12], h[11], h[13], h[14], chunk, lazy ? 1 : 0);
    memset(h, 0, sizeof h);
    (void)hipMemcpyToSymbol(HIP_SYMBOL(g_wave_clk), h, sizeof h);
  }
#endif
  if (resolve) {
    const int n_mem_all = it.grp_off ? n_items : it.n;
    hipLaunchKernelGGL(resolved_draws_kernel, dim3((n_mem_all + 255) / 256), dim3(256), 0, ctx->stream, n_mem_all, it.n,
                       it.grp_off, it.members, it.out_pos, g_res, n_draws, it.draw_is ? it.draw_is : n_draws,
                       it.draw_ds ? it.draw_ds : 1, draws_out);
  }
  if (lse_out && it.grp_off && it.grp_uid && n_items > 0)
    hipLaunchKernelGGL(member_lse_kernel, dim3((n_items + 255) / 256), dim3(256), 0, ctx->stream, n_items, it.grp_uid, it.members,
// ... 48 lines not shown
```

pclean_amd/csrc/sweep.hip:

```cpp
#include "sweep_internal.h"

int g_pclean_sync_count = 0;

__global__ void publish_count_kernel(const unsigned int* __restrict__ src, volatile unsigned int* __restrict__ dst, unsigned int seq) {
  dst[0] = *src;
  __threadfence_system();
  dst[1] = seq;
}
int read_count(pclean_ctx* ctx, const void* dev, void* out, const char* func, int line) {
  SweepState* s = st(ctx);
  static const bool no_poll = getenv("PCLEAN_NO_POLL") != nullptr;
  static const bool trace = getenv("PCLEAN_TRACE_SYNC") != nullptr;
  if (trace) fprintf(stderr, "[pclean sync %d] %s:%d (count)\n", ++g_pclean_sync_count, func, line);
  if (!no_poll && !s->h_poll) {
    if (hipHostMalloc((void**)&s->h_poll, 64, hipHostMallocMapped | hipHostMallocCoherent) != hipSuccess) s->h_poll = nullptr;
    if (s->h_poll) {
      s->h_poll[0] = s->h_poll[1] = 0;
      if (hipHostGetDevicePointer((void**)&s->d_poll, (void*)s->h_poll, 0) != hipSuccess) {
        (void)hipHostFree((void*)s->h_poll);
        s->h_poll = nullptr;
      }
    }
  }
  if (no_poll || !s->h_poll) {
// ... 837 lines not shown
  const int slot = new_slots[j];
  const int row = slot % N, particle = slot / N;
  const int32_t* v = vals + (size_t)j * n_nodes;
  double corr = 0.0;
  bool any = false;
  for (int li = 0; li < dp.n_leaves; ++li) {
    const DummyLeafDev& lf = dp.leaf[li];
    const int k = v[lf.node];
    if (k < 0 || lf.opt_vals[k] != lf.dummy_val) continue;
    any = true;
    double c = -lf.opt_logp[k];
    if (lf.kind == PCLEAN_DUMMY_STRING_PRIOR) {
      uint16_t drawn[DUMMY_MAX_LEN + 1];
      int L = -1;
      for (int ti = 0; ti < lf.n_terms; ++ti) {
        const DummyTermDev& tm = lf.t[ti];
        const int o = tm.obs_col[row];
        if (o < 0) continue;
        if (L < 0) {
          const uint64_t key = pclean_dummy_seed(seed, PCLEAN_SITE_NODE(dp.site_block, lf.node), (uint32_t)particle, sweep);
          L = dummy_draw_string(key, (uint32_t)((int64_t)row + row_offset), lf.min_len, lf.max_len, dp.lm_init, dp.lm_trans,
                                dp.letter_sym, drawn);
        }
        const int sid = tm.obs_ids[o];
        const uint16_t* os = dp.sym + dp.off[sid];
        const int ol = (int)(dp.off[sid + 1] - dp.off[sid]);
        if (ol > DUMMY_MAX_LEN) {
          dp.dp_ctr[1] = 1u;
          continue;
        }
        int16_t* H = dp.dp + (size_t)jl * dp.slot_cells + tm.dp_off;
        const int d = dummy_distance(tm.dist_mode, os, ol, drawn, L, H);
        double l;
        if (tm.max_typos >= 0 && d > tm.max_typos) {
          l = -1e5;
        } else {
          l = dp.nb[(size_t)((L + 4) / 5) * dp.nb_stride + d];
          l -= dp.logl[L] * (double)d;
          l -= 1.629048269010741 * (double)d;
        }
        const size_t pi = (size_t)o * tm.n_lat + lf.dummy_val;
        const int dph = tm.elem_bytes == 1 ? (int)tm.pair[pi] : (int)((const uint16_t*)tm.pair)[pi];
        double lph;
        if (tm.max_typos >= 0 && dph > tm.max_typos) {
          lph = -1e5;
        } else {
          const int Lp = tm.lat_len[lf.dummy_val];
          lph = dp.nb[(size_t)((Lp + 4) / 5) * dp.nb_stride + dph];
          lph -= dp.logl[Lp] * (double)dph;
          lph -= 1.629048269010741 * (double)dph;
        }
        c += l - lph;
      }
    }
    corr += c;
  }
  if (any) w[slot] += corr;
}


void pclean_sweep_state_free(pclean_ctx* ctx) {
  if (!ctx->sweep_state) return;
  SweepState* s = (SweepState*)ctx->sweep_state;
  for (auto& b : s->pool) b.release();
  for (auto& r : s->run) {
    r.pchoice.release(); r.pnewpos.release(); r.draws.release(); r.moved_flag.release(); r.new_flag.release();
    r.moved_list.release(); r.new_list.release(); r.new_slots.release();
    r.locals.release(); r.it_ctx.release(); r.choice.release(); r.chosen_newpos.release(); r.vals.release();
    r.lse.release(); r.plan_kind.release(); r.plan_nrows.release(); r.plan_cmb.release(); r.plan_colmap.release();
    r.plan_cols.release();
  }
  s->did.release(); s->cur.release(); s->chosen.release(); s->ancestors.release(); s->csmc_flag.release(); s->w.release();
  s->log_total.release(); s->logml_inc.release(); s->logml_acc.release(); s->logml.release(); s->counter.release();
  s->arr_ptrs.release();
  for (auto& kv : s->leaf_iota) kv.second.release();
  for (auto& f : s->fast) {
    for (auto& c : f.comp) c.release();
    for (auto& c : f.clen) c.release();
    for (auto& c : f.cblk) c.release();
    f.prior_e.release();
    f.prior_n.release();
    f.alive.release();
    f.zero_row.release();
  }
  s->tail_counts.release();
  for (auto& kv : s->tuple_ids) kv.second.release();
  for (auto& kv : s->memo) {
    kv.second.keys.release();
    kv.second.vals.release();
    kv.second.count.release();
  }
  if (s->h_counts) (void)hipHostFree(s->h_counts);
  if (s->h_over) (void)hipHostFree(s->h_over);
  for (int k = 0; k < SweepState::MAX_SIDE; ++k) {
    if (s->side[k]) (void)hipStreamDestroy(s->side[k]);
    if (s->side_join[k]) (void)hipEventDestroy(s->side_join[k]);
    if (s->side_mid[k]) (void)hipEventDestroy(s->side_mid[k]);
  }
  if (s->side_fork) (void)hipEventDestroy(s->side_fork);
  if (s->h_poll) (void)hipHostFree((void*)s->h_poll);
  s->dummy_dp.release();
  s->dummy_ctr.release();
  s->over_ctr.release();
  for (auto& b : s->more_banks) b.release();
  for (auto e : s->prof_ev) (void)hipEventDestroy(e);
  if (s->ev0) (void)hipEventDestroy(s->ev0);
  if (s->ev1) (void)hipEventDestroy(s->ev1);
  if (s->pre_stream) (void)hipStreamDestroy(s->pre_stream);
  if (s->pre_fork) (void)hipEventDestroy(s->pre_fork);
  if (s->pre_join) (void)hipEventDestroy(s->pre_join);
  if (s->evg0) (void)hipEventDestroy(s->evg0);
  if (s->evg1) (void)hipEventDestroy(s->evg1);
  if (s->evs) (void)hipEventDestroy(s->evs);
  if (s->eve) (void)hipEventDestroy(s->eve);
  delete s;
  ctx->sweep_state = nullptr;
}

int begin_call(pclean_ctx* ctx) {
  SweepState* s = st(ctx);
  s->pool_used = 0;
  s->dbg_desc = nullptr;
  s->dummy_used = false;
  ctx->prior_mode = false;
  s->over_rec.clear();
  if (s->over_ctr.alloc(OVER_SLOTS + STAT_WORDS + CTR_BANK)) return pclean_fail(ctx, PCLEAN_ERR_HIP, "device alloc failed");
  { const int rcz = dev_zero(ctx, s->over_ctr.p, (OVER_SLOTS + STAT_WORDS + CTR_BANK) * sizeof(unsigned int)); if (rcz) return rcz; }
  s->bank_used = 0;
  s->scan_stats_used = false;
  return PCLEAN_OK;
}
__global__ void dev_zero_kernel(uint4* __restrict__ p16, size_t n16, unsigned char* __restrict__ tail, int n_tail) {
  const size_t stride = (size_t)gridDim.x * blockDim.x;
  for (size_t i = (size_t)blockIdx.x * blockDim.x + threadIdx.x; i < n16; i += stride) p16[i] = make_uint4(0u, 0u, 0u, 0u);
  if (blockIdx.x == 0 && (int)threadIdx.x < n_tail) tail[threadIdx.x] = 0;
}
int dev_zero(pclean_ctx* ctx, void* p, size_t bytes) {
  static const bool off = getenv("PCLEAN_NO_ZERO_KERNEL") != nullptr;
  if (bytes == 0) return PCLEAN_OK;
  unsigned char* b = static_cast<unsigned char*>(p);
  const size_t head = (16 - ((uintptr_t)b & 15)) & 15;
  if (!off && bytes <= 256) {
    hipLaunchKernelGGL(dev_zero_kernel, dim3(1), dim3(256), 0, ctx->stream, (uint4*)nullptr, (size_t)0, b, (int)bytes);
    return PCLEAN_OK;
  }
  if (off || head > 0) {
    HIPCHK(ctx, hipMemsetAsync(p, 0, bytes, ctx->stream));
    return PCLEAN_OK;
  }
  const size_t n16 = bytes >> 4;
  const int n_tail = (int)(bytes & 15);
  const unsigned int blocks = (unsigned int)std::min<size_t>(std::max<size_t>((n16 + 255) / 256, 1), 4096);
  hipLaunchKernelGGL(dev_zero_kernel, dim3(blocks), dim3(256), 0, ctx->stream, reinterpret_cast<uint4*>(b), n16, b + (n16 << 4), n_tail);
  return PCLEAN_OK;
}
__global__ void publish_regions_kernel(const SweepState::PubRegions pr) {
  const int r = blockIdx.x;
  const uint32_t* __restrict__ src = pr.src[r];
  uint32_t* __restrict__ dst = pr.dst[r];
  for (uint32_t i = threadIdx.x; i < pr.words[r]; i += blockDim.x) dst[i] = src[i];
}
int d2h_small(pclean_ctx* ctx, void* host, const void* dev, size_t bytes, void* host_base) {
  SweepState* s = st(ctx);
  static const bool off = getenv("PCLEAN_NO_PUBLISH_REGIONS") != nullptr;
  if (bytes == 0) return PCLEAN_OK;
  void* mapped = nullptr;
// ... 73 lines not shown
}
int finish_call(pclean_ctx* ctx) {
  if (st(ctx)->over_rec.empty() && !st(ctx)->scan_stats_used) return PCLEAN_OK;
  int rc = queue_over_copy(ctx);
  if (!rc) rc = d2h_flush(ctx);
  if (rc) return rc;
  PCLEAN_SYNC(ctx);
  apply_over_stats(ctx);
  return PCLEAN_OK;
}


int prof_phase_id(SweepState* s, const char* name) {
  for (size_t i = 0; i < s->prof_names.size(); ++i)
    if (s->prof_names[i] == name) return (int)i;
  s->prof_names.push_back(name);
  s->prof_ms.push_back(0.f);
  s->prof_launches.push_back(0);
  return (int)s->prof_names.size() - 1;
}
void prof_collect(pclean_ctx* ctx) {
  SweepState* s = st(ctx);
  (void)hipStreamSynchronize(ctx->stream);
  for (size_t r = 0; r < s->prof_used; ++r) {
    float ms = 0.f;
    if (hipEventElapsedTime(&ms, s->prof_ev[2 * r], s->prof_ev[2 * r + 1]) == hipSuccess) {
      s->prof_ms[s->prof_phase[r]] += ms;
      s->prof_launches[s->prof_phase[r]] += 1;
    }
  }
  s->prof_used = 0;
}

extern "C" int pclean_set_profiling(pclean_ctx* ctx, int32_t on) {
  if (!ctx) return PCLEAN_ERR_ARG;
  SweepState* s = st(ctx);
  s->prof_on = on != 0;
  s->prof_used = 0;
  std::fill(s->prof_ms.begin(), s->prof_ms.end(), 0.f);
  std::fill(s->prof_launches.begin(), s->prof_launches.end(), 0);
  return PCLEAN_OK;
}
extern "C" int pclean_get_profile(pclean_ctx* ctx, int32_t cap, char* names, float* ms, int32_t* launches,
                                  int32_t* n_out) {
  if (!ctx || !n_out || cap < 0) return PCLEAN_ERR_ARG;
  SweepState* s = st(ctx);
  *n_out = (int32_t)s->prof_names.size();
  for (int i = 0; i < cap && i < *n_out; ++i) {
    if (names) {
      strncpy(names + (size_t)i * 32, s->prof_names[i].c_str(), 31);
      names[(size_t)i * 32 + 31] = 0;
    }
    if (ms) ms[i] = s->prof_ms[i];
    if (launches) launches[i] = s->prof_launches[i];
  }
  return PCLEAN_OK;
}


extern "C" int pclean_set_active_rows(pclean_ctx* ctx, int32_t begin, int32_t count) {
  if (!ctx || begin < 0 || count < -1 || (count >= 0 && (int64_t)begin + count > ctx->n_rows))
    return pclean_fail(ctx, PCLEAN_ERR_ARG, "pclean_set_active_rows: window outside the loaded rows");
  ctx->active_begin = count < 0 ? 0 : begin;
  ctx->active_count = count;
  return PCLEAN_OK;
}


extern "C" int pclean_debug_root_flags(pclean_ctx* ctx, int32_t n_rows, int32_t* out) {
  if (!ctx || !out || n_rows <= 0) return pclean_fail(ctx, PCLEAN_ERR_ARG, "pclean_debug_root_flags: bad arguments");
  SweepState* s = st(ctx);
  if (!s->dbg_desc || s->dbg_items != n_rows)
    return pclean_fail(ctx, PCLEAN_ERR_STATE, "pclean_debug_root_flags: the last call was not a pclean_sweep of %d rows "
                                              "through the compact-table root kernel", n_rows);
  HIPCHK(ctx, hipSetDevice(ctx->device));
  DevBuf<int32_t> d;
  if (d.alloc(n_rows)) return pclean_fail(ctx, PCLEAN_ERR_HIP, "device alloc failed");
  int rc = pclean_launch_root_flags(ctx, s->dbg_groups, s->dbg_desc, s->dbg_grp_off, s->dbg_members, s->dbg_oflag, d.p);
  hipError_t e = rc ? hipSuccess : hipMemcpyAsync(out, d.p, (size_t)n_rows * 4, hipMemcpyDeviceToHost, ctx->stream);
  if (e == hipSuccess) e = hipStreamSynchronize(ctx->stream);
  d.release();
  if (rc) return rc;
  if (e != hipSuccess) return pclean_fail(ctx, PCLEAN_ERR_HIP, "pclean_debug_root_flags: %s", hipGetErrorString(e));
  return PCLEAN_OK;
}

extern "C" int pclean_debug_global_evidence_sort(pclean_ctx* ctx, int32_t on) {
  if (!ctx) return PCLEAN_ERR_ARG;
  ctx->no_item_agg = on != 0;
  return PCLEAN_OK;
}

extern "C" int pclean_debug_force_generic(pclean_ctx* ctx, int32_t on) {
  if (!ctx) return PCLEAN_ERR_ARG;
  ctx->force_generic = on != 0;
  return PCLEAN_OK;
}

extern "C" int pclean_set_row_offset(pclean_ctx* ctx, int64_t row_offset) {
  if (!ctx || row_offset < 0) return pclean_fail(ctx, PCLEAN_ERR_ARG, "bad row offset");
  st(ctx)->row_offset = row_offset;
  return PCLEAN_OK;
}

extern "C" int pclean_score_node(pclean_ctx* ctx, int32_t block_id, int32_t node_id, int32_t n_items,
                                 const int32_t* rows, const int32_t* ctxv, const int32_t* excl, const double* snew,
                                 uint64_t seed, uint32_t sweep, int32_t n_draws, double* lse, double* scores,
                                 int32_t* draws) {
  if (!ctx || block_id < 0 || block_id >= PCLEAN_MAX_BLOCKS || !ctx->block[block_id].valid || n_items <= 0 || !rows ||
      n_draws < 0 || (n_draws > 0 && !draws))
    return pclean_fail(ctx, PCLEAN_ERR_ARG, "pclean_score_node: bad arguments");
  Block& b = ctx->block[block_id];
  if (node_id < 0 || node_id >= (int)b.nodes.size()) return pclean_fail(ctx, PCLEAN_ERR_ARG, "bad node id");
  HIPCHK(ctx, hipSetDevice(ctx->device));
  {
    const int rcb = begin_call(ctx);
    if (rcb) return rcb;
  }
  const pclean_node& n = b.nodes[node_id];
  const CandTable& t = ctx->cand[n.table];
  const int nc = t.n_rows + (n.kind == PCLEAN_NODE_FK ? 1 : 0);
  int32_t* d_rows = scratch<int32_t>(ctx, n_items);
  int32_t* d_ctx = ctxv ? scratch<int32_t>(ctx, (size_t)n_items * PCLEAN_MAX_CTX) : nullptr;
  int32_t* d_excl = excl ? scratch<int32_t>(ctx, n_items) : nullptr;
  double* d_snew = snew ? scratch<double>(ctx, n_items) : nullptr;
  double* d_lse = scratch<double>(ctx, n_items);
  double* d_scores = scores ? scratch<double>(ctx, (size_t)n_items * nc) : nullptr;
  int32_t* d_draws = n_draws ? scratch<int32_t>(ctx, (size_t)n_items * n_draws) : nullptr;
  if (!d_rows || !d_lse || (ctxv && !d_ctx) || (excl && !d_excl) || (snew && !d_snew) || (scores && !d_scores) ||
      (n_draws && !d_draws))
    return pclean_fail(ctx, PCLEAN_ERR_HIP, "scratch alloc failed");
  HIPCHK(ctx, hipMemcpyAsync(d_rows, rows, n_items * 4, hipMemcpyHostToDevice, ctx->stream));
  if (ctxv) HIPCHK(ctx, hipMemcpyAsync(d_ctx, ctxv, (size_t)n_items * PCLEAN_MAX_CTX * 4, hipMemcpyHostToDevice, ctx->stream));
  if (excl) HIPCHK(ctx, hipMemcpyAsync(d_excl, excl, n_items * 4, hipMemcpyHostToDevice, ctx->stream));
  if (snew) HIPCHK(ctx, hipMemcpyAsync(d_snew, snew, n_items * 8, hipMemcpyHostToDevice, ctx->stream));
  ItemList il{n_items, d_rows, d_ctx, nullptr, nullptr};
  int rc = eval_node(ctx, block_id, node_id, il, d_excl, seed, sweep, n_draws, d_lse, d_draws, d_scores,
                     (n.kind == PCLEAN_NODE_FK && snew) ? d_snew : nullptr, false);
  if (rc) return rc;
  if (lse) HIPCHK(ctx, hipMemcpyAsync(lse, d_lse, n_items * 8, hipMemcpyDeviceToHost, ctx->stream));
  if (scores) HIPCHK(ctx, hipMemcpyAsync(scores, d_scores, (size_t)n_items * nc * 8, hipMemcpyDeviceToHost, ctx->stream));
  if (n_draws) HIPCHK(ctx, hipMemcpyAsync(draws, d_draws, (size_t)n_items * n_draws * 4, hipMemcpyDeviceToHost, ctx->stream));
  PCLEAN_SYNC(ctx);
  return finish_call(ctx);
}


static int block_dummy_drawable(pclean_ctx* ctx, int bi, bool* out, bool* by_row = nullptr) {
  Block& b = ctx->block[bi];
  *out = false;
  if (by_row) *by_row = true;
  for (int node = 0; node < (int)b.nodes.size(); ++node) {
    const pclean_node& n = b.nodes[node];
    if (n.kind != PCLEAN_NODE_LEAF || n.dummy_value == 0) continue;
    if (!n.cacheable || (node < (int)b.node_gauss.size() && b.node_gauss[node] >= 0)) {
      *out = true;
      if (by_row) *by_row = false;
      return PCLEAN_OK;
    }
    const double* cache;
    const int32_t* ocol;
    int n_obs;
    int rc = ensure_leaf_cache(ctx, bi, node, &cache, &ocol, &n_obs);
    if (rc) return rc;
    if (b.leaf_drawable[node] != 0) {
      static const bool dbg = getenv("PCLEAN_DEBUG_DUMMY") != nullptr;
// ... 1205 lines not shown
```

pclean_amd/csrc/sweep_internal.h:

```cpp
#pragma once
#include <algorithm>
#include <cmath>
#include <map>
#include <set>

#include <hipcub/hipcub.hpp>
#include <rocprim/rocprim.hpp>

#include "../../include/pclean_detmath.h"
#include "../../include/pclean_philox.h"
#include "dummy_dev.h"
#include "enum.h"
#include "gauss_dev.h"
#include "sweep_state.h"

extern int g_pclean_sync_count;
int read_count(pclean_ctx* ctx, const void* dev, void* out, const char* func, int line);
#define PCLEAN_READ_COUNT(ctx, dev, out)                                  \
  do {                                                                    \
    const int rc_ = read_count(ctx, (dev), (out), __func__, __LINE__);    \
    if (rc_) return rc_;                                                  \
  } while (0)

#define PCLEAN_SYNC(ctx)                                                                                   \
  do {                                                                                                     \
    static const bool trace_ = getenv("PCLEAN_TRACE_SYNC") != nullptr;                                     \
    if (trace_) fprintf(stderr, "[pclean sync %d] %s:%d\n", ++g_pclean_sync_count, __func__, __LINE__);          \
    HIPCHK(ctx, hipStreamSynchronize(ctx->stream));                                                        \
  } while (0)

static inline dim3 grid1(size_t n, int bs = 256) { return dim3((unsigned)((n + bs - 1) / bs)); }

struct ItemList {
  int n = 0;
  const int32_t* row = nullptr;
  const int32_t* ctx = nullptr;
  const int32_t* particle = nullptr;
  const int32_t* origin = nullptr;
  const int32_t* ev_lo = nullptr;
  const int32_t* ev_hi = nullptr;
  const int32_t* ev_rows = nullptr;
  const int32_t* ev_ctx = nullptr;
  const int32_t* rng_row = nullptr;
  int draw_is = 0, draw_ds = 0;
};
struct ItemGroups {
  int n_groups = 0;
  const int32_t* grp_off = nullptr;
  const int32_t* members = nullptr;
  const int32_t* head = nullptr;
  const int32_t* uid = nullptr;
  const uint64_t* hg_incl = nullptr;
  const int32_t* hg_rep = nullptr;
  const int32_t* hg_slot_of = nullptr;
};

template <typename T>
static T* scratch(pclean_ctx* ctx, size_t count) {
  SweepState* s = st(ctx);
  if (s->pool_used == s->pool.size()) s->pool.emplace_back();
  DevBuf<unsigned char>& b = s->pool[s->pool_used++];
  const size_t need = std::max<size_t>(count * sizeof(T), 16);
  if (need > b.n && b.alloc(std::max(need, b.n + b.n / 2))) {
    if (b.alloc(need)) return nullptr;
  }
  return (T*)b.p;
}

static unsigned int* fresh_counter(pclean_ctx* ctx) {
  SweepState* s = st(ctx);
  if (!s->over_ctr.p) return nullptr;
  unsigned int* bank = s->over_ctr.p + OVER_SLOTS + STAT_WORDS;
  static const int first = [] {
    const char* e = getenv("PCLEAN_CTR_BANK");
    return e ? std::max(1, std::min(atoi(e), CTR_BANK)) : CTR_BANK;
  }();
  if (s->bank_used < first) return bank + s->bank_used++;
  const int idx = s->bank_used - first, b = idx / CTR_BANK, o = idx % CTR_BANK;
  while ((int)s->more_banks.size() <= b) s->more_banks.emplace_back();
  if (s->more_banks[b].alloc(CTR_BANK)) return nullptr;
  if (o == 0 && hipMemsetAsync(s->more_banks[b].p, 0, CTR_BANK * sizeof(unsigned int), ctx->stream) != hipSuccess) return nullptr;
  ++s->bank_used;
  return s->more_banks[b].p + o;
}

int prof_phase_id(SweepState* s, const char* name);
struct ProfScope {
  pclean_ctx* ctx;
  SweepState* s;
  size_t rec = (size_t)-1;
  ProfScope(pclean_ctx* c, const char* name) : ctx(c), s(st(c)) {
    if (!s->prof_on) return;
    rec = s->prof_used++;
    while (s->prof_ev.size() < 2 * (rec + 1)) {
      hipEvent_t e;
      if (hipEventCreate(&e) != hipSuccess) {
        rec = (size_t)-1;
        --s->prof_used;
        return;
      }
      s->prof_ev.push_back(e);
    }
    if (s->prof_phase.size() <= rec) s->prof_phase.resize(rec + 1);
    s->prof_phase[rec] = prof_phase_id(s, name);
    (void)hipEventRecord(s->prof_ev[2 * rec], ctx->stream);
  }
  ~ProfScope() {
    if (rec != (size_t)-1) (void)hipEventRecord(s->prof_ev[2 * rec + 1], ctx->stream);
  }
};

#define MAXP 64

template <int PMAX>
struct FixW {
  double m;
  uint64_t U;
  uint64_t u[PMAX];
};
template <int PMAX>
__device__ __forceinline__ void fix_weights(const double* w, size_t sp, int P, FixW<PMAX>& f) {
  f.m = -__builtin_inf();
  f.U = 0;
#pragma unroll
  for (int p = 0; p < PMAX; ++p)
    if (p < P) f.m = fmax(f.m, w[(size_t)p * sp]);
#pragma unroll
  for (int p = 0; p < PMAX; ++p) {
    f.u[p] = (p < P && f.m != -__builtin_inf()) ? pclean_fixw(w[(size_t)p * sp] - f.m) : 0ull;
    f.U += f.u[p];
  }
}
template <int PMAX>
__device__ __forceinline__ int fix_pick(const FixW<PMAX>& f, int P, uint64_t R) {
  if (f.U == 0) return P - 1;
  const uint64_t x = pclean_mulhi64(R, f.U);
  uint64_t acc = 0;
// ... 130 lines not shown
```

pclean_amd/csrc/sweep_state.h:

```cpp
#pragma once
#include <functional>
#include <map>
#include <string>
#include <deque>
#include <vector>

#include "ctx.h"
#include "enum.h"

struct PlanDev {
  int32_t n_nodes;
  const int32_t* kind;
  const int32_t* const* cols;
  const int32_t* n_rows;
  const int32_t* colmap_begin;
  const int32_t* colmap;
};


struct BlockRun {
  DevBuf<int32_t> pchoice, pnewpos, draws, it_ctx, choice, chosen_newpos, vals, locals, moved_flag, new_flag, moved_list,
      new_list, new_slots;
  DevBuf<double> lse;
  int n_new = 0;
  int locals_rows = 0;
  DevBuf<int32_t> plocals;
  bool plocals_on = false;
  size_t it_ctx_np = 0;
  int it_ctx_used = -1;
  bool lazy_new = false;
  int ctx_extra_cap = 0;
  DevBuf<int32_t> plan_kind, plan_nrows, plan_cmb, plan_colmap;
  DevBuf<const int32_t*> plan_cols;
  PlanDev plan{};
  bool plan_ready = false;
  std::vector<int32_t> plan_sig_nrows, plan_sig_kind, plan_sig_cmb;
  std::vector<const int32_t*> plan_sig_cols;
  size_t plan_sig_colmap = 0;
  uint64_t plan_sig_block = 0;
};

struct FastRoot {
  std::vector<DevBuf<uint8_t>> comp, clen, cblk;
  std::vector<uint64_t> ver;
  DevBuf<double> prior_e, prior_n;
  DevBuf<uint16_t> alive;
  DevBuf<uint8_t> zero_row;
  int disabled = 0;
  int backoff = 64;
  uint64_t cmin_key = 0;
  double cmin = 0.0;
  uint64_t prior_ver = 0;
  int kpad = 0;
  double logc_max = 0.0;
  int wl_off = 0;
  DevBuf<int32_t> obs_rm;
  uint64_t obs_rm_key = 0;
};

struct SweepState {
  FastRoot fast[PCLEAN_MAX_BLOCKS * 64];
  std::vector<DevBuf<unsigned char>> pool;
  size_t pool_used = 0;
  BlockRun run[PCLEAN_MAX_BLOCKS];
  DevBuf<int32_t> cur, chosen, ancestors, csmc_flag, did;
  const int32_t* last_cur_base = nullptr;
  size_t last_cur_ld = 0;
  int last_N = 0, last_blocks = 0;
  bool last_dev_cur = false, last_hot_timed = false;
  volatile unsigned int* h_poll = nullptr;
  unsigned int* d_poll = nullptr;
  unsigned int poll_seq = 0;
  bool outputs_pending = false;
  bool lists_on_host = false;
  DevBuf<double> w, log_total, logml_inc, logml_acc, logml;
  DevBuf<unsigned int> counter;
  DevBuf<int32_t*> arr_ptrs;
  std::map<int, DevBuf<int32_t>> leaf_iota;
  std::map<int, uint64_t> leaf_version;
  int64_t row_offset = 0;
  hipEvent_t ev0 = nullptr, ev1 = nullptr, evs = nullptr, eve = nullptr;
  hipEvent_t evg0 = nullptr, evg1 = nullptr;
  hipStream_t pre_stream = nullptr;
  std::function<int()> on_first_wait;
  hipEvent_t pre_fork = nullptr, pre_join = nullptr;
  bool gate_timed = false;
  struct LeafMemo {
    DevBuf<uint64_t> keys;
    DevBuf<double> vals;
    DevBuf<unsigned int> count;
    uint64_t ver = 0;
    int cap = 0;
  };
  std::map<int, LeafMemo> memo;
  struct TupleIds {
    DevBuf<int32_t> id;
    DevBuf<uint32_t> pre;
    uint64_t sig = 0;
    struct StaticOrder {
      int begin = 0, n = 0, n_tiles = 0;
      DevBuf<int32_t> order, tid, tile_off;
      void release() { order.release(); tid.release(); tile_off.release(); }
    };
    std::vector<StaticOrder> windows;
    void release() {
      id.release();
      pre.release();
      for (auto& w : windows) w.release();
      windows.clear();
    }
  };
  std::map<int, TupleIds> tuple_ids;
  struct GateStat { int all_need_run = 0, skip = 0; };
  std::map<int, GateStat> gate_stat;
  struct DummyRows { DevBuf<int32_t> flag; uint64_t sig = 0; int n = 0, n_flagged = 0; };
  std::map<int, DummyRows> dummy_rows;
  const int32_t* lat_off = nullptr;
  const int32_t* lat_item_of_pos = nullptr;
  int lat_items = 0, lat_ev = 0, lat_max_ev = 0;
  std::map<int, const AggDev*> lat_agg;
  DevBuf<int32_t> tail_counts;
  int32_t* h_counts = nullptr;
  bool prof_on = false;
  std::vector<hipEvent_t> prof_ev;
  std::vector<int> prof_phase;
  size_t prof_used = 0;
  std::vector<std::string> prof_names;
  std::vector<float> prof_ms;
  std::vector<int32_t> prof_launches;
  bool scan_stats_used = false;
  int bank_used = 0;
  DevBuf<unsigned int> over_ctr;
  std::deque<DevBuf<unsigned int>> more_banks;
  struct PubRegions { const uint32_t* src[12]; uint32_t* dst[12]; uint32_t words[12]; int n; } pub = {};
  std::map<void*, void*> pub_map;
  struct OverRec { int block, node, n_items; bool time_it, leaf; int min_items; };
  std::vector<OverRec> over_rec;
  static const int MAX_SIDE = 8;
  hipStream_t side[MAX_SIDE] = {};
  hipEvent_t side_fork = nullptr, side_join[MAX_SIDE] = {}, side_mid[MAX_SIDE] = {};
  int n_side = -1;
  unsigned int* h_over = nullptr;
  DevBuf<int16_t> dummy_dp;
  DevBuf<unsigned int> dummy_ctr;
  bool dummy_used = false;
  struct LazyReq { bool on = false; const int32_t* eager_rows = nullptr; } lazy_req;
  struct LazyOut { bool valid = false; LazyDrawArgs args{}; uint32_t site = 0; } lazy_out;
  const int32_t* dbg_desc = nullptr;
  const int32_t* dbg_grp_off = nullptr;
  const int32_t* dbg_members = nullptr;
  const int32_t* dbg_oflag = nullptr;
  int dbg_groups = 0, dbg_items = 0;
};

#define OVER_SLOTS 256
#define STAT_WORDS (64 * 32)
#define CTR_BANK 2048
static SweepState* st(pclean_ctx* ctx) {
  if (!ctx->sweep_state) ctx->sweep_state = new SweepState();
  return (SweepState*)ctx->sweep_state;
}


int pclean_sweep_finish_queue(pclean_ctx* ctx);
int d2h_small(pclean_ctx* ctx, void* host, const void* dev, size_t bytes, void* host_base = nullptr);
int d2h_flush(pclean_ctx* ctx);
int dev_zero(pclean_ctx* ctx, void* p, size_t bytes);
int pclean_sweep_finish_synced(pclean_ctx* ctx);
int pclean_sweep_fetch_lists(pclean_ctx* ctx);
```

Before: 405.0 million.

## Cache per-run gate distances across sweeps with generation-tagged invalidation

Adds a per-run cache of per-term byte distances for the exact candidate score in the group gate and descriptor kernels. Entries are keyed by a candidate generation counter, which is bumped for every row whose compact table changes, plus an epoch that invalidates everything on rebuilds. Observation tuples are precomputed per static run so the kernels load them from a compact array instead of gathering per row. The aim is to skip recomputing string distances for unchanged candidates across Gibbs sweeps. In exchange it adds bump kernels, per-run metadata and cache memory, and stats atomics, and stale-cache bugs could affect correctness.

```diff
diff --git a/include/pclean_hip.h b/include/pclean_hip.h
--- a/include/pclean_hip.h
+++ b/include/pclean_hip.h
@@ -282,6 +282,7 @@
 int pclean_debug_force_generic(pclean_ctx* ctx, int32_t on);
 int pclean_debug_global_evidence_sort(pclean_ctx* ctx, int32_t on);
 int pclean_debug_root_flags(pclean_ctx* ctx, int32_t n_rows, int32_t* out);
+int pclean_debug_gate_cache(pclean_ctx* ctx, int32_t block_id, int32_t node_id, uint32_t* out);
 
 int pclean_random_add_typos(pclean_ctx* ctx, int32_t n, const uint32_t* cp, const int64_t* off, int32_t max_typos,
                             uint64_t seed, uint32_t stream, int32_t out_stride, uint32_t* out_cp, int32_t* out_len);
diff --git a/pclean_amd/_lib.py b/pclean_amd/_lib.py
--- a/pclean_amd/_lib.py
+++ b/pclean_amd/_lib.py
@@ -225,6 +225,12 @@
         out = np.empty(n_rows, dtype=np.int32)
         check(self.h, self.lib.pclean_debug_root_flags(self.h, C.c_int32(n_rows), _p(out, C.c_int32)), "pclean_debug_root_flags")
         return out
+
+    def gate_cache_stats(self, block_id, node_id=0):
+        out = np.zeros(4, dtype=np.uint32)
+        check(self.h, self.lib.pclean_debug_gate_cache(self.h, C.c_int32(block_id), C.c_int32(node_id), _p(out, C.c_uint32)),
+              "pclean_debug_gate_cache")
+        return tuple(int(v) for v in out)
 
     def global_evidence_sort(self, on):
         check(self.h, self.lib.pclean_debug_global_evidence_sort(self.h, C.c_int32(int(on))), "pclean_debug_global_evidence_sort")
diff --git a/pclean_amd/csrc/enum.h b/pclean_amd/csrc/enum.h
--- a/pclean_amd/csrc/enum.h
+++ b/pclean_amd/csrc/enum.h
@@ -129,6 +129,22 @@
   FastTermDev terms[PCLEAN_MAX_TERMS];
 };
 
+struct GateCacheEntry {
+  int32_t k;
+  uint32_t gen, epoch, pad;
+  uint8_t d[PCLEAN_MAX_TERMS];
+};
+struct GateCacheDev {
+  const int32_t* grp_run;
+  const int32_t* run_obs;
+  GateCacheEntry* entry;
+  const uint32_t* cand_gen;
+  uint32_t epoch;
+  int32_t verify;
+  unsigned int* stats;
+  unsigned int* stats_clear;
+};
+
 #define ROOT_LZ_CAP 256
 struct RootExtra {
   int32_t* lz_k;
@@ -143,7 +159,7 @@
                             int32_t* desc_scratch, int32_t* overflow_list,
                             unsigned int* scan_stats = nullptr, int n_items = 0, const double* pre_score = nullptr,
                             bool want_worklist = true, unsigned int* wl_stat = nullptr, const int32_t* pre_obs = nullptr,
-                            RootExtra* extra = nullptr);
+                            RootExtra* extra = nullptr, const GateCacheDev* gc = nullptr);
 struct LazyDrawArgs {
   int32_t n_pos, n_rows, n_particles, pad;
   const int32_t* members;
@@ -164,7 +180,7 @@
 };
 int pclean_launch_lazy_draws(pclean_ctx* ctx, const LazyDrawArgs& a, uint64_t seed, uint32_t sweep, uint32_t site);
 int pclean_launch_group_gate(pclean_ctx* ctx, const FastRootDev& fr, const ItemsDev& it, const GateDev& gt, int32_t* flag,
-                             double* score_out, int32_t* obs_out);
+                             double* score_out, int32_t* obs_out, const GateCacheDev* gc = nullptr);
 int pclean_launch_overflow_fast(pclean_ctx* ctx, const FastRootDev& fr, const ItemsDev& it, const ChildrenDev& ch,
                                 uint64_t seed, uint32_t sweep, uint32_t site, int n_draws, double* lse_out,
                                 int32_t* draws_out, const int32_t* over_list, const unsigned int* over_count);
diff --git a/pclean_amd/csrc/eval.hip b/pclean_amd/csrc/eval.hip
--- a/pclean_amd/csrc/eval.hip
+++ b/pclean_amd/csrc/eval.hip
@@ -261,6 +261,11 @@
   return 1;
 }
 
+__global__ void cand_gen_bump_kernel(const int32_t* __restrict__ rows, int n, uint32_t* __restrict__ cand_gen) {
+  const int j = blockIdx.x * blockDim.x + threadIdx.x;
+  if (j < n) atomicAdd(&cand_gen[rows[j]], 1u);
+}
+
 static int try_fast_root(pclean_ctx* ctx, int block_id, int node_id, FastRootDev& fr, bool ev_mode = false) {
   Block& b = ctx->block[block_id];
   if (node_id >= 64) return 0;
@@ -310,6 +315,28 @@
     f.kpad = kpad;
     f.prior_ver = 0;
   }
+  if (!leaf) {
+    const uint64_t gkey = (((uint64_t)kpad * 1000003ull + b.version) * 1000003ull + ctx->obs_version) * 1000003ull + (uint64_t)n.n_terms;
+    if (f.gc_key != gkey) {
+      f.gc_key = gkey;
+      ++f.gc_epoch;
+    }
+    if ((int)f.cand_gen.n < kpad || !f.cand_gen.p) {
+      if (f.cand_gen.alloc((size_t)kpad + kpad / 8 + 64)) return pclean_fail(ctx, PCLEAN_ERR_HIP, "device alloc failed");
+      HIPCHK(ctx, hipMemsetAsync(f.cand_gen.p, 0, f.cand_gen.n * sizeof(uint32_t), ctx->stream));
+      ++f.gc_epoch;
+    }
+  }
+  const int32_t* bumped[4] = {nullptr, nullptr, nullptr, nullptr};
+  int n_bumped = 0;
+  bool epoch_bumped = false;
+  auto bump_gen = [&](const int32_t* rows, int n_rows) {
+    if (leaf || n_rows <= 0 || !f.cand_gen.p) return;
+    for (int q = 0; q < n_bumped; ++q)
+      if (bumped[q] == rows) return;
+    if (n_bumped < 4) bumped[n_bumped++] = rows;
+    hipLaunchKernelGGL(cand_gen_bump_kernel, dim3((n_rows + 255) / 256), dim3(256), 0, ctx->stream, rows, n_rows, f.cand_gen.p);
+  };
   auto grow = [](DevBuf<uint8_t>& b, size_t need) -> int {
     need = std::max<size_t>(need, 16);
     return need <= b.n && b.p ? 0 : b.alloc(need + need / 8);
@@ -338,9 +365,11 @@
         f.ver[i] == t.cols_delta_base * 1000003ull + pt.version) {
       ProfScope psd(ctx, "compact_table_update");
       int rc = PCLEAN_OK;
-      if (t.cols_delta_n > 0)
+      if (t.cols_delta_n > 0) {
+        bump_gen(t.cols_delta_rows, t.cols_delta_n);
         rc = pclean_update_compact(ctx, pt.d.p, pt.n_obs, pt.n_lat, t.cols.p + (size_t)tm.cand_col * t.n_rows, pt.lat_len.p,
                                      t.cols_delta_rows, t.cols_delta_n, kpad, f.comp[i].p, f.clen[i].p);
+      }
       if (rc) return rc;
       if (t.cols_delta_n > 0)
         rc = pclean_update_compact_min(ctx, f.comp[i].p, pt.n_obs, kpad, cstride, t.cols_delta_rows, t.cols_delta_n, f.cblk[i].p);
@@ -384,12 +413,14 @@
         int rc = PCLEAN_OK;
         const int32_t* colp = tw.cols.p + (size_t)tm.cand_col * tw.n_rows;
         if (via_commit && tw.commit_delta_n > 0) {
+          bump_gen(tw.commit_delta_rows, tw.commit_delta_n);
           rc = pclean_update_compact(ctx, pt.d.p, pt.n_obs, pt.n_lat, colp, pt.lat_len.p, tw.commit_delta_rows, tw.commit_delta_n, kpad,
                                      f.comp[i].p, f.clen[i].p);
           if (!rc) rc = pclean_update_compact_min(ctx, f.comp[i].p, pt.n_obs, kpad, cstride, tw.commit_delta_rows, tw.commit_delta_n, f.cblk[i].p);
           if (rc) return rc;
         }
         if (un > 0) {
+          bump_gen(tw.union_rows.p, un);
           rc = pclean_update_compact(ctx, pt.d.p, pt.n_obs, pt.n_lat, colp, pt.lat_len.p, tw.union_rows.p, un, kpad, f.comp[i].p, f.clen[i].p);
           if (!rc) rc = pclean_update_compact_min(ctx, f.comp[i].p, pt.n_obs, kpad, cstride, tw.union_rows.p, un, f.cblk[i].p);
           if (rc) return rc;
@@ -399,6 +430,10 @@
     }
     if (f.ver[i] != ver || !f.comp[i].p) {
       ProfScope psd(ctx, "compact_table_rebuild");
+      if (!epoch_bumped) {
+        ++f.gc_epoch;
+        epoch_bumped = true;
+      }
       if (grow(f.comp[i], (size_t)pt.n_obs * kpad) || grow(f.clen[i], (size_t)kpad))
         return pclean_fail(ctx, PCLEAN_ERR_HIP, "device alloc failed (compact tables)");
       int rc = pclean_build_compact(ctx, pt.d.p, pt.n_obs, pt.n_lat, t.cols.p + (size_t)tm.cand_col * t.n_rows,
@@ -595,6 +630,30 @@
   int fast = 0, fast_ev = 0;
   ItemGroups g_pre;
   bool fast_tried = false, groups_tried = false;
+  auto make_gate_cache = [&](const ItemGroups& gr, GateCacheDev& gc) -> int {
+    gc = GateCacheDev{};
+    if (!gr.grp_run || node_id >= 64) return PCLEAN_OK;
+    FastRoot& f = s->fast[block_id * 64 + node_id];
+    if (!f.cand_gen.p) return PCLEAN_OK;
+    if (!f.gc_stats.p) {
+      if (f.gc_stats.alloc(8)) return pclean_fail(ctx, PCLEAN_ERR_HIP, "device alloc failed");
+      HIPCHK(ctx, hipMemsetAsync(f.gc_stats.p, 0, 8 * sizeof(unsigned int), ctx->stream));
+    }
+    if (f.gc_sweep != sweep) {
+      f.gc_sweep = sweep;
+      f.gc_slot ^= 1;
+    }
+    static const bool verify = getenv("PCLEAN_GATE_CACHE_VERIFY") != nullptr;
+    gc.grp_run = gr.grp_run;
+    gc.run_obs = gr.run_obs;
+    gc.entry = gr.run_entry;
+    gc.cand_gen = f.cand_gen.p;
+    gc.epoch = f.gc_epoch;
+    gc.verify = verify ? 1 : 0;
+    gc.stats = f.gc_stats.p + 4 * f.gc_slot;
+    gc.stats_clear = f.gc_stats.p + 4 * (f.gc_slot ^ 1);
+    return PCLEAN_OK;
+  };
   const double* pre_score = nullptr;
   const int32_t* pre_obs = nullptr;
   if (n.kind == PCLEAN_NODE_FK && ctx->prior_mode) {
@@ -667,10 +726,13 @@
           int32_t* flag = scratch<int32_t>(ctx, ng);
           list_g = scratch<int32_t>(ctx, ng);
           double* sc = scratch<double>(ctx, ng);
-          int32_t* ow = scratch<int32_t>(ctx, (size_t)ng * PCLEAN_MAX_TERMS);
-          if (!flag || !list_g || !sc || !ow) return pclean_fail(ctx, PCLEAN_ERR_HIP, "scratch alloc failed");
+          GateCacheDev gc;
+          rc = make_gate_cache(g_pre, gc);
+          if (rc) return rc;
+          int32_t* ow = gc.grp_run ? nullptr : scratch<int32_t>(ctx, (size_t)ng * PCLEAN_MAX_TERMS);
+          if (!flag || !list_g || !sc || (!gc.grp_run && !ow)) return pclean_fail(ctx, PCLEAN_ERR_HIP, "scratch alloc failed");
           if (time_it && s->evg0) (void)hipEventRecord(s->evg0, ctx->stream);
-          rc = pclean_launch_group_gate(ctx, fr, itg, gt, flag, sc, ow);
+          rc = pclean_launch_group_gate(ctx, fr, itg, gt, flag, sc, ow, &gc);
           if (rc) return rc;
           if (time_it && s->evg0) {
             (void)hipEventRecord(s->evg1, ctx->stream);
@@ -943,8 +1005,12 @@
       ex.eager_rows = lazy_req.eager_rows;
       use_ex = true;
     }
+    GateCacheDev gc;
+    rc = make_gate_cache(ggrp, gc);
+    if (rc) return rc;
     rc = pclean_launch_root_fast(ctx, fr, it, ch, seed, sweep, site, n_draws, lse_out, draws_out, oflag, over_count, desc,
-                                 over_list, scan_stats, il.n, pre_score, wl_stat != nullptr, wl_stat, pre_obs, use_ex ? &ex : nullptr);
+                                 over_list, scan_stats, il.n, pre_score, wl_stat != nullptr, wl_stat, pre_obs, use_ex ? &ex : nullptr,
+                                 &gc);
     if (!rc && ex.lz_ns) {
       SweepState::LazyOut& lo = s->lazy_out;
       lo.valid = true;
@@ -1445,6 +1511,18 @@
 __global__ void static_tid_kernel(int n, const uint64_t* __restrict__ key_s, int32_t* __restrict__ tid) {
   const int j = blockIdx.x * blockDim.x + threadIdx.x;
   if (j < n) tid[j] = (int32_t)(uint32_t)key_s[j];
+}
+struct RunObsCols {
+  const int32_t* col[PCLEAN_MAX_TERMS];
+};
+__global__ void static_run_obs_kernel(int n, const int32_t* __restrict__ order, const int32_t* __restrict__ run_id, RunObsCols oc,
+                                      int n_terms, int32_t* __restrict__ run_obs) {
+  const int p = blockIdx.x * blockDim.x + threadIdx.x;
+  if (p >= n) return;
+  const int run = run_id[p];
+  if (p > 0 && run_id[p - 1] == run) return;
+  const int row = order[p];
+  for (int f = 0; f < PCLEAN_MAX_TERMS; ++f) run_obs[(size_t)run * PCLEAN_MAX_TERMS + f] = f < n_terms ? oc.col[f][row] : -1;
 }
 static int ensure_static_order(pclean_ctx* ctx, int block_id, int node_id, int n, const SweepState::TupleIds::StaticOrder** out) {
   typedef SweepState::TupleIds::StaticOrder StaticOrder;
@@ -1520,6 +1598,31 @@
   if (hipMemcpyAsync(w.tile_off.p, h_off, (size_t)n_off * sizeof(int32_t), hipMemcpyHostToDevice, ctx->stream) != hipSuccess ||
       hipStreamSynchronize(ctx->stream) != hipSuccess)
     return fail("static order: upload failed");
+  {
+    Block& b = ctx->block[block_id];
+    const pclean_node& nd = b.nodes[node_id];
+    if (nd.n_terms >= 1 && nd.n_terms <= PCLEAN_MAX_TERMS) {
+      int run = -1, tile = 0, prev = 0;
+      for (int p = 0; p < n; ++p) {
+        while (p >= h_off[tile + 1]) ++tile;
+        const int cur = h_tid[p];
+        if (p == h_off[tile] || cur != prev) ++run;
+        prev = cur;
+        h_tid[p] = run;
+      }
+      w.n_runs = run + 1;
+      RunObsCols oc{};
+      for (int f = 0; f < nd.n_terms; ++f) oc.col[f] = ctx->obs.p + (size_t)b.terms[nd.term_begin + f].obs_col * ctx->n_rows + begin;
+      if (w.run_id.alloc(n) || w.run_obs.alloc((size_t)w.n_runs * PCLEAN_MAX_TERMS) || w.cache.alloc(w.n_runs))
+        return fail("device alloc failed");
+      if (hipMemcpyAsync(w.run_id.p, h_tid, (size_t)n * sizeof(int32_t), hipMemcpyHostToDevice, ctx->stream) != hipSuccess ||
+          hipMemsetAsync(w.cache.p, 0xff, (size_t)w.n_runs * sizeof(GateCacheEntry), ctx->stream) != hipSuccess)
+        return fail("static order: upload failed");
+      hipLaunchKernelGGL(static_run_obs_kernel, grid1(n), dim3(256), 0, ctx->stream, n, w.order.p, w.run_id.p, oc, nd.n_terms,
+                         w.run_obs.p);
+      if (hipStreamSynchronize(ctx->stream) != hipSuccess) return fail("static order: upload failed");
+    }
+  }
   cleanup();
   t.windows.push_back(w);
   *out = &t.windows.back();
@@ -1529,7 +1632,8 @@
                                                        const int32_t* __restrict__ order, const int32_t* __restrict__ tid_sorted,
                                                        const int32_t* __restrict__ excl, int split_m,
                                                        int32_t* __restrict__ members, int32_t* __restrict__ loc,
-                                                       int32_t* __restrict__ tile_cnt) {
+                                                       int32_t* __restrict__ tile_cnt, const int32_t* __restrict__ run_id,
+                                                       int32_t* __restrict__ rinfo) {
   const int tile = blockIdx.x * 4 + (threadIdx.x >> 6);
   const int lane = threadIdx.x & 63;
   if (tile >= n_tiles) return;
@@ -1541,6 +1645,10 @@
     kt = tid_sorted[t0 + lane];
     ke = excl[i];
   }
+  const int kt_prev = __shfl_up(kt, 1, 64);
+  const bool run_first = on && (lane == 0 || kt != kt_prev);
+  const int rid = (run_id && on) ? run_id[t0 + lane] : 0;
+  int my_run = 0;
   int pos_acc = 0, piece_acc = 0, my_at = 0, my_loc = 0;
   for (unsigned long long pend = __ballot(on); pend;) {
     const int ld = __builtin_ctzll(pend);
@@ -1554,6 +1662,7 @@
       const bool first = split_m > 0 ? r == piece * split_m : r == 0;
       my_at = pos_acc + r;
       my_loc = ((piece_acc + piece) << 1) | (first ? 1 : 0);
+      my_run = (rid << 1) | ((r == 0 && run_first) ? 1 : 0);
     }
     pos_acc += c;
     piece_acc += pieces;
@@ -1562,13 +1671,15 @@
   if (on) {
     members[t0 + my_at] = i;
     loc[t0 + my_at] = my_loc;
+    if (rinfo) rinfo[t0 + my_at] = my_run;
   }
   if (lane == 0) tile_cnt[tile] = piece_acc;
 }
 __global__ __launch_bounds__(256) void sg_fill_kernel(int n, int n_tiles, const int32_t* __restrict__ tile_off,
                                                       const int32_t* __restrict__ loc, const int32_t* __restrict__ tile_cnt,
                                                       const int32_t* __restrict__ incl, int32_t* __restrict__ uid,
-                                                      int32_t* __restrict__ grp_off) {
+                                                      int32_t* __restrict__ grp_off, const int32_t* __restrict__ rinfo,
+                                                      int32_t* __restrict__ grp_run) {
   const int tile = blockIdx.x * 4 + (threadIdx.x >> 6);
   const int lane = threadIdx.x & 63;
   if (tile >= n_tiles) return;
@@ -1577,7 +1688,10 @@
   if (lane < len) {
     const int v = loc[t0 + lane], grp = base + (v >> 1);
     uid[t0 + lane] = grp + 1;
-    if (v & 1) grp_off[grp] = t0 + lane;
+    if (v & 1) {
+      grp_off[grp] = t0 + lane;
+      if (grp_run) grp_run[grp] = rinfo[t0 + lane];
+    }
   }
   if (tile == 0 && lane == 0) grp_off[incl[n_tiles - 1]] = n;
 }
@@ -1591,17 +1705,25 @@
   size_t tmp_scan = 0;
   HIPCHK(ctx, hipcub::DeviceScan::InclusiveSum(nullptr, tmp_scan, tile_cnt, incl, nt, ctx->stream));
   unsigned char* tmp = scratch<unsigned char>(ctx, std::max<size_t>(tmp_scan, 16));
-  if (!members || !loc || !tile_cnt || !incl || !tmp) return pclean_fail(ctx, PCLEAN_ERR_HIP, "scratch alloc failed");
+  static const bool no_gate_cache = getenv("PCLEAN_NO_GATE_CACHE") != nullptr;
+  const bool runs = !no_gate_cache && so.run_id.p && so.run_obs.p && so.cache.p;
+  int32_t* rinfo = runs ? scratch<int32_t>(ctx, n) : nullptr;
+  if (!members || !loc || !tile_cnt || !incl || !tmp || (runs && !rinfo)) return pclean_fail(ctx, PCLEAN_ERR_HIP, "scratch alloc failed");
   hipLaunchKernelGGL(sg_class_kernel, grid1(nt, 4), dim3(256), 0, ctx->stream, nt, so.tile_off.p, so.order.p, so.tid.p, excl,
-                     split_m, members, loc, tile_cnt);
+                     split_m, members, loc, tile_cnt, runs ? so.run_id.p : (const int32_t*)nullptr, rinfo);
   HIPCHK(ctx, hipcub::DeviceScan::InclusiveSum(tmp, tmp_scan, tile_cnt, incl, nt, ctx->stream));
   int32_t n_unique = 0;
   PCLEAN_READ_COUNT(ctx, incl + (nt - 1), &n_unique);
   if (n_unique <= 0 || (double)n_unique > 0.75 * n) return PCLEAN_OK;
   int32_t* uid = scratch<int32_t>(ctx, n);
   int32_t* grp_off = scratch<int32_t>(ctx, (size_t)n_unique + 1);
-  if (!uid || !grp_off) return pclean_fail(ctx, PCLEAN_ERR_HIP, "scratch alloc failed");
-  hipLaunchKernelGGL(sg_fill_kernel, grid1(nt, 4), dim3(256), 0, ctx->stream, n, nt, so.tile_off.p, loc, tile_cnt, incl, uid, grp_off);
+  int32_t* grp_run = runs ? scratch<int32_t>(ctx, (size_t)n_unique) : nullptr;
+  if (!uid || !grp_off || (runs && !grp_run)) return pclean_fail(ctx, PCLEAN_ERR_HIP, "scratch alloc failed");
+  hipLaunchKernelGGL(sg_fill_kernel, grid1(nt, 4), dim3(256), 0, ctx->stream, n, nt, so.tile_off.p, loc, tile_cnt, incl, uid, grp_off,
+                     (const int32_t*)rinfo, grp_run);
+  g.grp_run = grp_run;
+  g.run_obs = runs ? so.run_obs.p : nullptr;
+  g.run_entry = runs ? so.cache.p : nullptr;
   g.n_groups = n_unique;
   g.grp_off = grp_off;
   g.members = members;
diff --git a/pclean_amd/csrc/root_wave.hip b/pclean_amd/csrc/root_wave.hip
--- a/pclean_amd/csrc/root_wave.hip
+++ b/pclean_amd/csrc/root_wave.hip
@@ -213,15 +213,22 @@
   return b;
 }
 
-__device__ __forceinline__ double fast_exact_score_mlp(const FastRootDev& fr, const int* o, int ctx0, int ctx1, int k, double pr) {
-  int d[PCLEAN_MAX_TERMS], L[PCLEAN_MAX_TERMS];
-  bool sat = false;
+__device__ __forceinline__ void fast_gather_bytes(const FastRootDev& fr, const int* o, int k, int* d) {
 #pragma unroll
   for (int f = 0; f < PCLEAN_MAX_TERMS; ++f) {
     const bool plain = f < fr.n_terms && fr.terms[f].ctx_slot < 0;
     const uint8_t* crow = (plain && o[f] >= 0) ? fr.terms[f].comp + (size_t)o[f] * fr.kpad : fr.zero_row;
+    d[f] = crow[k];
+  }
+}
+__device__ __forceinline__ double fast_score_from_bytes(const FastRootDev& fr, const int* o, int ctx0, int ctx1, int k, double pr,
+                                                        int* d) {
+  int L[PCLEAN_MAX_TERMS];
+  bool sat = false;
+#pragma unroll
+  for (int f = 0; f < PCLEAN_MAX_TERMS; ++f) {
+    const bool plain = f < fr.n_terms && fr.terms[f].ctx_slot < 0;
     const uint8_t* cl = plain ? fr.terms[f].clen : fr.zero_row;
-    d[f] = crow[k];
     L[f] = cl[k];
   }
 #pragma unroll
@@ -252,6 +259,70 @@
   }
   return b;
 }
+__device__ __forceinline__ double fast_exact_score_mlp(const FastRootDev& fr, const int* o, int ctx0, int ctx1, int k, double pr) {
+  int d[PCLEAN_MAX_TERMS];
+  fast_gather_bytes(fr, o, k, d);
+  return fast_score_from_bytes(fr, o, ctx0, ctx1, k, pr, d);
+}
+__device__ __forceinline__ double fast_exact_score_cached(const FastRootDev& fr, const GateCacheDev& gc, int run_info, const int* o,
+                                                          int ctx0, int ctx1, int k, double pr, unsigned int* cnt) {
+  static_assert(sizeof(GateCacheEntry) == 32 && PCLEAN_MAX_TERMS == 16, "two 16-byte words per entry");
+  int d[PCLEAN_MAX_TERMS];
+  bool hit = false;
+  uint4* e = reinterpret_cast<uint4*>(gc.entry + (run_info >> 1));
+  if (run_info & 1) {
+    const uint4 h = e[0];
+    const uint32_t gen = gc.cand_gen[k];
+    const bool same_k = (int)h.x == k;
+    hit = same_k && h.y == gen && h.z == gc.epoch;
+    if (hit) {
+      const uint4 b = e[1];
+      const uint32_t bw[4] = {b.x, b.y, b.z, b.w};
+#pragma unroll
+      for (int f = 0; f < PCLEAN_MAX_TERMS; ++f) d[f] = (int)((bw[f >> 2] >> (8 * (f & 3))) & 0xffu);
+      if (gc.verify) {
+        int d2[PCLEAN_MAX_TERMS];
+        fast_gather_bytes(fr, o, k, d2);
+        bool diff = false;
+#pragma unroll
+        for (int f = 0; f < PCLEAN_MAX_TERMS; ++f) diff |= d2[f] != d[f];
+        cnt[3] += diff ? 1u : 0u;
+      }
+    } else {
+      fast_gather_bytes(fr, o, k, d);
+      uint32_t bw[4] = {0u, 0u, 0u, 0u};
+#pragma unroll
+      for (int f = 0; f < PCLEAN_MAX_TERMS; ++f) bw[f >> 2] |= (uint32_t)d[f] << (8 * (f & 3));
+      e[0] = make_uint4((uint32_t)k, gen, gc.epoch, 0u);
+      e[1] = make_uint4(bw[0], bw[1], bw[2], bw[3]);
+      cnt[2] += same_k ? 1u : 0u;
+    }
+  } else {
+    fast_gather_bytes(fr, o, k, d);
+  }
+  cnt[0] += hit ? 1u : 0u;
+  cnt[1] += hit ? 0u : 1u;
+  return fast_score_from_bytes(fr, o, ctx0, ctx1, k, pr, d);
+}
+__device__ __forceinline__ void load_run_obs(const GateCacheDev& gc, int run, int* o) {
+  const int4* po = reinterpret_cast<const int4*>(gc.run_obs + (size_t)run * PCLEAN_MAX_TERMS);
+#pragma unroll
+  for (int q = 0; q < 4; ++q) {
+    const int4 v = po[q];
+    o[4 * q] = v.x;
+    o[4 * q + 1] = v.y;
+    o[4 * q + 2] = v.z;
+    o[4 * q + 3] = v.w;
+  }
+}
+__device__ __forceinline__ void gate_cache_count(const GateCacheDev& gc, unsigned int* cnt) {
+#pragma unroll
+  for (int c = 0; c < 4; ++c) {
+    unsigned int v = cnt[c];
+    for (int sh = 32; sh > 0; sh >>= 1) v += __shfl_xor(v, sh, 64);
+    if ((threadIdx.x & 63) == 0 && v) atomicAdd(&gc.stats[c], v);
+  }
+}
 
 __device__ __forceinline__ void load_row_obs(const FastRootDev& fr, int row, int* o) {
   static_assert(PCLEAN_MAX_TERMS == 16, "four 16-byte loads");
@@ -292,8 +363,9 @@
                                   int32_t* __restrict__ gd, unsigned int* __restrict__ chunk_ctr, double* __restrict__ g_m,
                                   uint64_t* __restrict__ g_U, int32_t* __restrict__ g_res,
                                   unsigned int* __restrict__ scan_stats, const double* __restrict__ pre_score,
-                                  const int32_t* __restrict__ pre_obs) {
+                                  const int32_t* __restrict__ pre_obs, const GateCacheDev gc) {
   const int g = blockIdx.x * blockDim.x + threadIdx.x;
+  if (gc.grp_run && g < 4) gc.stats_clear[g] = 0u;
   if (g < 8) chunk_ctr[g * WAVE_CTR_STRIDE] = 0u;
   if (g >= 8 && g < 8 + WL_SEGS) chunk_ctr[WL_SEG_CTR(g - 8)] = 0u;
   if (g == 8 + WL_SEGS) chunk_ctr[WAVE_WORK_CTR] = 0u;
@@ -306,7 +378,10 @@
   const int ctx0 = it.ctx ? it.ctx[(size_t)t * PCLEAN_MAX_CTX] : 0;
   const int ctx1 = it.ctx ? it.ctx[(size_t)t * PCLEAN_MAX_CTX + 1] : 0;
   int o[PCLEAN_MAX_TERMS];
-  if (pre_obs) {
+  const int run_info = gc.grp_run ? gc.grp_run[g] : 0;
+  if (gc.grp_run) {
+    load_run_obs(gc, run_info >> 1, o);
+  } else if (pre_obs) {
     static_assert(PCLEAN_MAX_TERMS == 16, "four 16-byte loads");
     const int4* po = reinterpret_cast<const int4*>(pre_obs + (size_t)g * PCLEAN_MAX_TERMS);
 #pragma unroll
@@ -446,9 +521,11 @@
 
 __global__ void group_gate_kernel(const FastRootDev fr, const ItemsDev it, const GateDev gt, int n_groups,
                                   int32_t* __restrict__ flag, double* __restrict__ score_out,
-                                  int32_t* __restrict__ obs_out) {
+                                  int32_t* __restrict__ obs_out, const GateCacheDev gc) {
   const int g = blockIdx.x * blockDim.x + threadIdx.x;
-  if (g >= n_groups) return;
+  unsigned int gc_cnt[4] = {0u, 0u, 0u, 0u};
+  if (gc.grp_run && g < 4) gc.stats_clear[g] = 0u;
+  if (g < n_groups) {
   const int t = it.grp_off ? it.members[it.grp_off[g]] : g;
   const int row = it.row ? it.row[t] : t;
   const int excl = it.excl ? it.excl[t] : -1;
@@ -458,14 +535,17 @@
   bool need = true;
   double sc = 0.0;
   int o[PCLEAN_MAX_TERMS];
-  load_row_obs(fr, row, o);
-  {
+  const int run_info = gc.grp_run ? gc.grp_run[g] : 0;
+  if (gc.grp_run) {
+    load_run_obs(gc, run_info >> 1, o);
+  } else {
+    load_row_obs(fr, row, o);
     int4* po = reinterpret_cast<int4*>(obs_out + (size_t)g * PCLEAN_MAX_TERMS);
 #pragma unroll
     for (int q = 0; q < 4; ++q) po[q] = make_int4(o[4 * q], o[4 * q + 1], o[4 * q + 2], o[4 * q + 3]);
   }
   if (excl >= 0 && !deleted && fr.logc_m1) {
-    sc = fast_exact_score_mlp(fr, o, ctx0, ctx1, excl, fr.logc_m1[excl] - fr.scal[1]);
+    sc = fast_exact_score_cached(fr, gc, run_info, o, ctx0, ctx1, excl, fr.logc_m1[excl] - fr.scal[1], gc_cnt);
     double ub = fr.scal[2] - fr.scal[1];
     for (int c = 0; c < gt.n; ++c) {
       if (gt.cache[c]) {
@@ -479,12 +559,14 @@
   }
   flag[g] = need ? PCLEAN_CHOICE_NEW : 0;
   score_out[g] = sc;
+  }
+  if (gc.grp_run) gate_cache_count(gc, gc_cnt);
 }
 int pclean_launch_group_gate(pclean_ctx* ctx, const FastRootDev& fr, const ItemsDev& it, const GateDev& gt, int32_t* flag,
-                             double* score_out, int32_t* obs_out) {
+                             double* score_out, int32_t* obs_out, const GateCacheDev* gc) {
   if (it.n <= 0) return PCLEAN_OK;
   hipLaunchKernelGGL(group_gate_kernel, dim3((it.n + 255) / 256), dim3(256), 0, ctx->stream, fr, it, gt, it.n, flag, score_out,
-                     obs_out);
+                     obs_out, gc ? *gc : GateCacheDev{});
   HIPCHK(ctx, hipGetLastError());
   return PCLEAN_OK;
 }
@@ -1628,7 +1710,7 @@
                             int32_t* draws_out, int32_t* overflow_flag, unsigned int* overflow_count,
                             int32_t* desc_scratch, int32_t* overflow_list, unsigned int* scan_stats, int n_items,
                             const double* pre_score, bool want_worklist, unsigned int* wl_stat, const int32_t* pre_obs,
-                            RootExtra* extra) {
+                            RootExtra* extra, const GateCacheDev* gc) {
   if (it.n <= 0) return PCLEAN_OK;
   const size_t ng = (size_t)it.n;
   unsigned int* chunk_ctr = reinterpret_cast<unsigned int*>(desc_scratch + ng * GD_STRIDE);
@@ -1640,7 +1722,8 @@
   const bool resolve = n_draws > 0 && want_resolve && (!it.grp_off || n_items > 0);
   const bool lazy = extra && extra->lz_ns && n_draws > 0 && !resolve;
   hipLaunchKernelGGL(group_desc_kernel, dim3((it.n + 255) / 256), dim3(256), 0, ctx->stream, fr, it, ch, it.n,
-                     desc_scratch, chunk_ctr, g_m, g_U, resolve ? g_res : nullptr, scan_stats, pre_score, pre_obs);
+                     desc_scratch, chunk_ctr, g_m, g_U, resolve ? g_res : nullptr, scan_stats, pre_score, pre_obs,
+                     gc ? *gc : GateCacheDev{});
   if (extra) extra->g_U = g_U;
   static const bool no_settle = getenv("PCLEAN_NO_SETTLE") != nullptr;
   const bool settle = !no_settle && !resolve && n_draws > 0 && !fr.is_leaf && fr.n_pre >= 1 && fr.n_pre <= 3 && fr.cstride > 0 &&
diff --git a/pclean_amd/csrc/sweep.hip b/pclean_amd/csrc/sweep.hip
--- a/pclean_amd/csrc/sweep.hip
+++ b/pclean_amd/csrc/sweep.hip
@@ -943,6 +943,9 @@
     f.prior_n.release();
     f.alive.release();
     f.zero_row.release();
+    f.obs_rm.release();
+    f.cand_gen.release();
+    f.gc_stats.release();
   }
   s->tail_counts.release();
   for (auto& kv : s->tuple_ids) kv.second.release();
@@ -1182,6 +1185,18 @@
   d.release();
   if (rc) return rc;
   if (e != hipSuccess) return pclean_fail(ctx, PCLEAN_ERR_HIP, "pclean_debug_root_flags: %s", hipGetErrorString(e));
+  return PCLEAN_OK;
+}
+
+extern "C" int pclean_debug_gate_cache(pclean_ctx* ctx, int32_t block_id, int32_t node_id, uint32_t* out) {
+  if (!ctx || !out || block_id < 0 || block_id >= PCLEAN_MAX_BLOCKS || node_id < 0 || node_id >= 64)
+    return pclean_fail(ctx, PCLEAN_ERR_ARG, "pclean_debug_gate_cache: bad arguments");
+  for (int c = 0; c < 4; ++c) out[c] = 0u;
+  const FastRoot& f = st(ctx)->fast[block_id * 64 + node_id];
+  if (!f.gc_stats.p) return PCLEAN_OK;
+  HIPCHK(ctx, hipSetDevice(ctx->device));
+  HIPCHK(ctx, hipStreamSynchronize(ctx->stream));
+  HIPCHK(ctx, hipMemcpy(out, f.gc_stats.p + 4 * f.gc_slot, 4 * sizeof(uint32_t), hipMemcpyDeviceToHost));
   return PCLEAN_OK;
 }
 
diff --git a/pclean_amd/csrc/sweep_internal.h b/pclean_amd/csrc/sweep_internal.h
--- a/pclean_amd/csrc/sweep_internal.h
+++ b/pclean_amd/csrc/sweep_internal.h
@@ -53,6 +53,9 @@
   const uint64_t* hg_incl = nullptr;
   const int32_t* hg_rep = nullptr;
   const int32_t* hg_slot_of = nullptr;
+  const int32_t* grp_run = nullptr;
+  const int32_t* run_obs = nullptr;
+  GateCacheEntry* run_entry = nullptr;
 };
 
 template <typename T>
diff --git a/pclean_amd/csrc/sweep_state.h b/pclean_amd/csrc/sweep_state.h
--- a/pclean_amd/csrc/sweep_state.h
+++ b/pclean_amd/csrc/sweep_state.h
@@ -56,6 +56,12 @@
   int wl_off = 0;
   DevBuf<int32_t> obs_rm;
   uint64_t obs_rm_key = 0;
+  DevBuf<uint32_t> cand_gen;
+  uint32_t gc_epoch = 1;
+  uint64_t gc_key = 0;
+  DevBuf<unsigned int> gc_stats;
+  int gc_slot = 0;
+  uint32_t gc_sweep = 0xffffffffu;
 };
 
 struct SweepState {
@@ -100,7 +106,10 @@
     struct StaticOrder {
       int begin = 0, n = 0, n_tiles = 0;
       DevBuf<int32_t> order, tid, tile_off;
-      void release() { order.release(); tid.release(); tile_off.release(); }
+      int n_runs = 0;
+      DevBuf<int32_t> run_id, run_obs;
+      DevBuf<GateCacheEntry> cache;
+      void release() { order.release(); tid.release(); tile_off.release(); run_id.release(); run_obs.release(); cache.release(); }
     };
     std::vector<StaticOrder> windows;
     void release() {
```

After: 390.5 million. 0.964x the previous value.
